# IDEA-CCNL/Fengshenbang-LM

Measured on AMD Instinct MI355X. Metric: tokens/sec Ziya-LLaMA-13B ZeRO-3, higher is better.
Workload: dtype bf16; 1 GPU; model=Ziya-LLaMA-13B, global_batch=16, micro_batch=16, seq_len=2048, parallelism=zero3_dp1, activation_checkpointing=True, ckpt_skip_interval=4

## Files before the change

fengshen_amd/models/layers.py:

```python
from __future__ import annotations

import math
from typing import Callable, List, Optional

import torch
import torch.nn as nn
import torch.nn.init as init

from fengshen_amd.ops import functional as F_ops
from fengshen_amd.parallel import groups
from fengshen_amd.parallel.layers import (
    ColumnParallelLinear,
    RowParallelLinear,
    _init_partition,
    divide,
)
from fengshen_amd.parallel.mappings import (
    copy_to_tensor_model_parallel_region,
    gather_from_tensor_model_parallel_region,
)


def init_normal(std: float) -> Callable:
    def fn(tensor):
        return init.normal_(tensor, mean=0.0, std=std)
    return fn


def scaled_init_normal(std: float, num_layers: int) -> Callable:
    return init_normal(std / math.sqrt(2.0 * num_layers))


def small_init(dim: int) -> Callable:
    return init_normal(math.sqrt(2.0 / (5.0 * dim)))


def wang_init(dim: int, num_layers: int) -> Callable:
    return init_normal(2.0 / (num_layers * math.sqrt(dim)))


class MergedColumnParallelLinear(ColumnParallelLinear):

    def __init__(self, input_size: int, segment_sizes: List[int], bias: bool = True,
                 init_method: Callable = init.xavier_normal_, dtype=None):
        self.segment_sizes = list(segment_sizes)
        super().__init__(input_size, sum(segment_sizes), bias=bias,
                         gather_output=False, init_method=init_method, dtype=dtype)
        tp = groups.get_tensor_model_parallel_world_size()
        if tp > 1:
            off = 0
            for seg in self.segment_sizes:
                seg_per = divide(seg, tp)
                shard = self.weight[off:off + seg_per]
                _init_partition(shard, init_method,
                                full_shape=(seg, input_size), partition_dim=0)
                off += seg_per


class RMSNorm(nn.Module):

    def __init__(self, dim: int, eps: float = 1e-6, dtype=None):
        super().__init__()
        self.weight = nn.Parameter(torch.ones(dim, dtype=dtype))
        self.eps = eps

    def forward(self, x):
        return F_ops.rms_norm(x, self.weight, self.eps)


class LayerNorm(nn.Module):

    def __init__(self, dim: int, eps: float = 1e-5, dtype=None):
        super().__init__()
        self.weight = nn.Parameter(torch.ones(dim, dtype=dtype))
        self.bias = nn.Parameter(torch.zeros(dim, dtype=dtype))
        self.eps = eps

    def forward(self, x):
        return F_ops.layer_norm(x, self.weight, self.bias, self.eps)


class ScaleNorm(nn.Module):

    def __init__(self, dim: int, eps: float = 1e-8, dtype=None):
        super().__init__()
        self.g = nn.Parameter(torch.ones(1, dtype=dtype))
        self.dim = dim
        self.eps = eps

    def forward(self, x):
        n = x.float().norm(dim=-1, keepdim=True) * self.dim ** -0.5
        return (x.float() / n.clamp(min=self.eps)).to(x.dtype) * self.g


def get_norm(kind: str, dim: int, eps: float, dtype=None) -> nn.Module:
    if kind == "rmsnorm":
        return RMSNorm(dim, eps, dtype)
    if kind == "layernorm":
        return LayerNorm(dim, eps, dtype)
    if kind == "scalenorm":
        return ScaleNorm(dim, dtype=dtype)
    raise ValueError(kind)


class ParallelAttention(nn.Module):

    def __init__(self, hidden_size: int, num_heads: int, *, causal: bool,
                 rotary: bool = False, rope_base: float = 10000.0,
                 max_positions: int = 4096,
                 attention_dropout: float = 0.0, hidden_dropout: float = 0.0,
                 bias: bool = True, init_method=None, output_init_method=None,
                 dtype=None, num_kv_heads: Optional[int] = None,
                 layer_idx: int = 0, reduce_output: bool = True):
        super().__init__()
        self.layer_idx = layer_idx
        self.reduce_output = reduce_output
        tp = groups.get_tensor_model_parallel_world_size()
        self.hidden_size = hidden_size
        self.num_heads = num_heads
        self.num_kv_heads = num_kv_heads or num_heads
        assert self.num_kv_heads == num_heads, "GQA arrives with kernel pass 2"
        self.head_dim = divide(hidden_size, num_heads)
        self.num_heads_per_partition = divide(num_heads, tp)
        self.causal = causal
        self.rotary = rotary
        self.attention_dropout = attention_dropout
        self.hidden_dropout = hidden_dropout
        self.norm_factor = 1.0 / math.sqrt(self.head_dim)
        init_method = init_method or init.xavier_normal_
        output_init_method = output_init_method or init_method

        self.qkv_proj = MergedColumnParallelLinear(
            hidden_size, [hidden_size, hidden_size, hidden_size], bias=bias,
            init_method=init_method, dtype=dtype)
        self.out_proj = RowParallelLinear(
            hidden_size, hidden_size, bias=bias, input_is_parallel=True,
            init_method=output_init_method, dtype=dtype,
            reduce_output=reduce_output)

        if rotary:
            self.rope_base = rope_base
            self.max_positions = max_positions
            self._rope_cache = None

    def _rope_tables(self, device, seq_needed: int):
        cache = self._rope_cache
        if (cache is None or cache[0].device != device
                or cache[0].shape[0] < seq_needed):
            n = max(self.max_positions, seq_needed)
            cos, sin = F_ops.build_rope_cache(n, self.head_dim,
                                              base=self.rope_base)
            cache = (cos.to(device), sin.to(device))
            self._rope_cache = cache
        return cache

    def forward(self, x: torch.Tensor,
                attention_mask: Optional[torch.Tensor] = None,
                cache=None):
        b, sq, _ = x.shape
        np_ = self.num_heads_per_partition
        hn = self.head_dim

        qkv = self.qkv_proj(x)
        q, k, v = qkv.chunk(3, dim=-1)
        q = q.view(b, sq, np_, hn).transpose(1, 2)
        k = k.view(b, sq, np_, hn).transpose(1, 2)
        v = v.view(b, sq, np_, hn).transpose(1, 2)

        offset = 0
        if cache is not None:
            offset = cache.get_seq_length(self.layer_idx)
        if self.rotary:
            cos, sin = self._rope_tables(q.device, offset + sq)
            q, k = F_ops.apply_rotary(q, k, cos, sin, offset=offset)
        if cache is not None:
            k, v = cache.update(k, v, self.layer_idx)

        causal = self.causal
        if causal and offset > 0 and q.shape[-2] == 1:
            causal = False
        ctx = F_ops.attention(q, k, v, causal=causal, mask=attention_mask,
                              dropout_p=self.attention_dropout,
                              training=self.training, scale=self.norm_factor)
        ctx = ctx.transpose(1, 2).reshape(b, sq, np_ * hn)
        out = self.out_proj(ctx)
        if isinstance(out, tuple) and self.reduce_output:
            out = out[0]
        return out


class ParallelMLP(nn.Module):

    def __init__(self, hidden_size: int, ffn_hidden_size: Optional[int] = None,
                 bias: bool = True, init_method=None, output_init_method=None,
                 dtype=None, reduce_output: bool = True):
        super().__init__()
        ffn = ffn_hidden_size or 4 * hidden_size
        init_method = init_method or init.xavier_normal_
        self.reduce_output = reduce_output
        self.fc_in = ColumnParallelLinear(
            hidden_size, ffn, bias=bias, gather_output=False,
            init_method=init_method, skip_bias_add=bias, dtype=dtype)
        self.fc_out = RowParallelLinear(
            ffn, hidden_size, bias=bias, input_is_parallel=True,
            init_method=output_init_method or init_method, dtype=dtype,
            reduce_output=reduce_output)

    def forward(self, x):
        h = self.fc_in(x)
        if isinstance(h, tuple):
            h, bias = h
            h = F_ops.bias_gelu(h, bias)
        else:
            h = F_ops.eager_gelu(h.float()).to(h.dtype)
        out = self.fc_out(h)
        if isinstance(out, tuple) and self.reduce_output:
            out = out[0]
        return out


class LLaMAParallelMLP(nn.Module):

    def __init__(self, hidden_size: int, intermediate_size: Optional[int] = None,
                 multiple_of: int = 256, init_method=None,
                 output_init_method=None, dtype=None,
                 reduce_output: bool = True):
        super().__init__()
        self.reduce_output = reduce_output
        if intermediate_size is None:
            intermediate_size = int(2 * (4 * hidden_size) / 3)
            intermediate_size = multiple_of * (
                (intermediate_size + multiple_of - 1) // multiple_of)
        self.intermediate_size = intermediate_size
        init_method = init_method or init.xavier_normal_
        self.gate_up_proj = MergedColumnParallelLinear(
            hidden_size, [intermediate_size, intermediate_size], bias=False,
            init_method=init_method, dtype=dtype)
        self.down_proj = RowParallelLinear(
            intermediate_size, hidden_size, bias=False, input_is_parallel=True,
            init_method=output_init_method or init_method, dtype=dtype,
            reduce_output=reduce_output)

    def forward(self, x):
        packed = self.gate_up_proj(x)
        h = F_ops.swiglu(packed)
        return self.down_proj(h)


class ParallelTransformerLayer(nn.Module):

    def __init__(self, hidden_size: int, num_heads: int, *, causal: bool,
                 norm: str = "layernorm", norm_eps: float = 1e-5,
                 mlp_type: str = "gelu", ffn_hidden_size=None,
                 rotary: bool = False, rope_base: float = 10000.0,
                 max_positions: int = 4096,
                 attention_dropout: float = 0.0, hidden_dropout: float = 0.0,
                 bias: bool = True, init_method=None, output_init_method=None,
                 dtype=None, layer_idx: int = 0,
                 parallel_residual: bool = False):
        super().__init__()
        self.parallel_residual = parallel_residual
        self.input_norm = get_norm(norm, hidden_size, norm_eps, dtype)
        self.attention = ParallelAttention(
            hidden_size, num_heads, causal=causal, rotary=rotary,
            rope_base=rope_base, max_positions=max_positions,
            attention_dropout=attention_dropout, hidden_dropout=hidden_dropout,
            bias=bias, init_method=init_method,
            output_init_method=output_init_method, dtype=dtype,
            layer_idx=layer_idx, reduce_output=not parallel_residual)
        self.post_attention_norm = get_norm(norm, hidden_size, norm_eps, dtype)
        if mlp_type == "swiglu":
            self.mlp = LLaMAParallelMLP(
                hidden_size, ffn_hidden_size, init_method=init_method,
                output_init_method=output_init_method, dtype=dtype,
                reduce_output=not parallel_residual)
        else:
            self.mlp = ParallelMLP(
                hidden_size, ffn_hidden_size, bias=bias, init_method=init_method,
                output_init_method=output_init_method, dtype=dtype,
                reduce_output=not parallel_residual)
        self.hidden_dropout = hidden_dropout

    @staticmethod
    def _split_partial(out):
        if isinstance(out, tuple):
            return out[0], out[1]
        return out, None

    def forward(self, x, attention_mask=None, cache=None):
        if self.parallel_residual:
            from fengshen_amd.parallel.mappings import (
                reduce_from_tensor_model_parallel_region)
            ap, ab = self._split_partial(self.attention(
                self.input_norm(x), attention_mask=attention_mask,
                cache=cache))
            mp, mb = self._split_partial(
                self.mlp(self.post_attention_norm(x)))
            total = reduce_from_tensor_model_parallel_region(ap + mp)
            bias = None
            if ab is not None or mb is not None:
                bias = (ab if ab is not None else 0)                     + (mb if mb is not None else 0)
            return F_ops.bias_dropout_add(total, bias, x,
                                          self.hidden_dropout,
                                          self.training)
        residual = x
        h = self.input_norm(x)
        attn_out = self.attention(h, attention_mask=attention_mask, cache=cache)
        x = F_ops.bias_dropout_add(attn_out, None, residual,
                                   self.hidden_dropout, self.training)
        residual = x
        h = self.post_attention_norm(x)
        mlp_out = self.mlp(h)
        x = F_ops.bias_dropout_add(mlp_out, None, residual,
                                   self.hidden_dropout, self.training)
        return x


def parallel_lm_logits(hidden: torch.Tensor, word_embeddings_weight: torch.Tensor,
                       parallel_output: bool = True):
    input_parallel = copy_to_tensor_model_parallel_region(hidden)
    logits_parallel = torch.nn.functional.linear(
        input_parallel, word_embeddings_weight)
    if parallel_output:
        return logits_parallel
    return gather_from_tensor_model_parallel_region(logits_parallel)


class SinusoidalPositionalEmbedding(nn.Module):

    def __init__(self, dim: int, base: float = 10000.0):
        super().__init__()
        self.dim = dim
        self.base = base

    def forward(self, positions: torch.Tensor) -> torch.Tensor:
        half = self.dim // 2
        inv = 1.0 / (self.base ** (torch.arange(
            half, device=positions.device, dtype=torch.float32) / half))
        ang = positions.float()[..., None] * inv
        return torch.cat([ang.sin(), ang.cos()], dim=-1)


class AliBi(nn.Module):

    def __init__(self, num_heads: int, mp_size: int = 1, mp_rank: int = 0):
        super().__init__()
        self.num_heads = num_heads
        slopes = torch.tensor(self._slopes(num_heads))
        per = num_heads // mp_size
        self.register_buffer("slopes", slopes[mp_rank * per:(mp_rank + 1) * per],
                             persistent=False)
        self._cache = None

    @staticmethod
    def _slopes(n: int):
        def pow2(n):
            start = 2.0 ** (-(2.0 ** -(math.log2(n) - 3)))
            return [start * (start ** i) for i in range(n)]
        if math.log2(n).is_integer():
            return pow2(n)
        closest = 2 ** math.floor(math.log2(n))
        return pow2(closest) + AliBi._slopes(2 * closest)[0::2][: n - closest]

    def forward(self, sq: int, sk: int, device, dtype):
        if (self._cache is None or self._cache.shape[-1] < sk
                or self._cache.device != device):
            pos = torch.arange(sk, device=device, dtype=torch.float32)
            self._cache = self.slopes.to(device)[:, None, None] * \
                (pos[None, None, :] - pos[None, :, None])
        bias = self._cache[:, :sq, :sk] if self._cache.shape[1] >= sq else \
            self._cache[:, -sq:, :sk]
        return bias.to(dtype)


class SoftEmbedding(nn.Module):

    def __init__(self, wte: nn.Module, n_tokens: int = 10,
                 init_range: float = 0.5):
        super().__init__()
        self.wte = wte
        self.n_tokens = n_tokens
        dim = wte.weight.shape[1]
        self.soft_prompt = nn.Parameter(
            torch.empty(n_tokens, dim).uniform_(-init_range, init_range))

    def forward(self, input_ids: torch.Tensor) -> torch.Tensor:
        emb = self.wte(input_ids)
        b = emb.shape[0]
        prompt = self.soft_prompt.unsqueeze(0).expand(b, -1, -1).to(emb.dtype)
        return torch.cat([prompt, emb], dim=1)


class SpatialGatingUnit(nn.Module):

    def __init__(self, dim_ff: int, seq_len: int):
        super().__init__()
        self.norm = LayerNorm(dim_ff // 2)
        self.proj = nn.Linear(seq_len, seq_len)
        nn.init.zeros_(self.proj.weight)
        nn.init.ones_(self.proj.bias)

    def forward(self, x):
        res, gate = x.chunk(2, dim=-1)
        gate = self.norm(gate)
        gate = self.proj(gate.transpose(1, 2)).transpose(1, 2)
        return res * gate


class GMLPBlock(nn.Module):
    def __init__(self, dim: int, dim_ff: int, seq_len: int):
        super().__init__()
        self.norm = LayerNorm(dim)
        self.fc_in = nn.Linear(dim, dim_ff)
        self.sgu = SpatialGatingUnit(dim_ff, seq_len)
        self.fc_out = nn.Linear(dim_ff // 2, dim)

    def forward(self, x):
        h = self.norm(x)
        h = F_ops.eager_gelu(self.fc_in(h).float()).to(h.dtype)
        h = self.sgu(h)
        return x + self.fc_out(h)


def expand_attention_types(attention_config, num_layers: int):
    if attention_config is None:
        return ["global"] * num_layers
    out = []
    for types, repeat in attention_config:
        if repeat == "all":
            for i in range(num_layers):
                out.append(types[i % len(types)])
            break
        for i in range(int(repeat)):
            out.append(types[i % len(types)])
    assert len(out) >= num_layers, (
        f"attention_config covers {len(out)} layers, model has {num_layers}")
    return out[:num_layers]


def get_ltor_masks_and_position_ids(data: torch.Tensor, eod_token: int,
                                    reset_position_ids: bool = False,
                                    reset_attention_mask: bool = False,
                                    eod_mask_loss: bool = False):
    b, s = data.shape
    att = torch.tril(torch.ones(s, s, device=data.device)) \
        .unsqueeze(0).repeat(b, 1, 1)
    loss_mask = torch.ones(b, s, dtype=torch.float, device=data.device)
    if eod_mask_loss:
        loss_mask[data == eod_token] = 0.0
    position_ids = torch.arange(s, device=data.device) \
        .unsqueeze(0).repeat(b, 1)
    if reset_position_ids or reset_attention_mask:
        position_ids = position_ids.clone()
        for bi in range(b):
            eod_idx = position_ids[bi, data[bi] == eod_token]
            prev = 0
            for j in eod_idx.tolist():
                if reset_attention_mask:
                    att[bi, j + 1:, : j + 1] = 0
                if reset_position_ids:
                    position_ids[bi, j + 1:] -= j + 1 - prev
                    prev = j + 1
    return (att < 0.5).unsqueeze(1), loss_mask, position_ids
```

fengshen_amd/ops/csrc/bindings.cpp:

```cpp
#include <torch/extension.h>

#include <hip/hip_runtime.h>
#include <c10/hip/HIPStream.h>

#include <vector>

enum FsDtype { FS_F32 = 0, FS_BF16 = 1, FS_F16 = 2 };

static int fs_dtype(const at::Tensor& t) {
  switch (t.scalar_type()) {
    case at::kFloat: return FS_F32;
    case at::kBFloat16: return FS_BF16;
    case at::kHalf: return FS_F16;
    default: TORCH_CHECK(false, "unsupported dtype ", t.scalar_type());
  }
}

static hipStream_t cur_stream() {
  return c10::hip::getCurrentHIPStream().stream();
}

extern "C" {
void fs_rms_norm_fwd(const void*, const void*, void*, float*, int, int, float,
                     int, hipStream_t);
void fs_rms_norm_bwd(const void*, const void*, const void*, const float*,
                     void*, float*, int, int, int, hipStream_t);
void fs_layer_norm_fwd(const void*, const void*, const void*, void*, float*,
                       float*, int, int, float, int, hipStream_t);
void fs_layer_norm_bwd(const void*, const void*, const void*, const float*,
                       const float*, void*, float*, float*, int, int, int,
                       hipStream_t);
void fs_scaled_softmax_fwd(const void*, const unsigned char*, void*, float,
                           int, int, int, int, int, int, int, int,
                           hipStream_t);
void fs_scaled_softmax_bwd(const void*, const void*, void*, float, int, int,
                           int, hipStream_t);
void fs_rope(const void*, void*, const float*, const float*, long, int, int,
             int, int, int, hipStream_t);
void fs_swiglu_fwd(const void*, void*, long, int, int, hipStream_t);
void fs_swiglu_bwd(const void*, const void*, void*, long, int, int,
                   hipStream_t);
void fs_bias_gelu(const void*, const void*, const void*, void*, long, int, int,
                  int, hipStream_t);
void fs_fused_adamw(float*, const void*, float*, float*, void*, long, float,
                    float, float, float, float, int, int, int, hipStream_t);
void fs_flash_attn_fwd(const void*, const void*, const void*, void*, float*,
                       const int*, int, int, int, int, int, int, float,
                       float, unsigned long long, hipStream_t);
void fs_flash_attn_bwd(const void*, const void*, const void*, const void*,
                       const void*, const float*, void*, void*, void*, float*,
                       const int*, int, int, int, int, int, int, float,
                       float, unsigned long long, hipStream_t);
void fs_bf16_gemv(const void*, const void*, void*, int, int, int,
                  hipStream_t);
void fs_add_rms_norm(const void*, const void*, const void*, void*, void*,
                     int, int, float, hipStream_t);
void fs_decode_attn(const void*, void*, void*, const float*, const float*,
                    const void*, void*, int, int, int, int, float, int,
                    hipStream_t);
void fs_w8_gemv(const void*, const float*, const void*, void*, int, int, int,
                hipStream_t);
void fs_vocab_ce_fwd(const void*, const long*, float*, float*, float*,
                     long, int, int, int, hipStream_t);
void fs_vocab_ce_bwd(const void*, const long*, const float*, const float*,
                     const float*, void*, long, int, int, int, hipStream_t);
void fs_flash_attn_fwd_v3(const void*, const void*, const void*, void*,
                          float*, const int*, int, int, int, int, int, float,
                          float, unsigned long long, hipStream_t);
void fs_flash_attn_bwd_v3(const void*, const void*, const void*, const void*,
                          const void*, const float*, void*, void*, void*,
                          float*, const int*, int, int, int, int, int, float,
                          float, unsigned long long, hipStream_t);
}

static std::vector<at::Tensor> rms_norm_fwd(at::Tensor x, at::Tensor w,
                                            double eps) {
  TORCH_CHECK(x.is_contiguous() && w.is_contiguous());
  const int H = x.size(-1);
  TORCH_CHECK(H % 8 == 0, "hidden must be divisible by 8");
  const long rows = x.numel() / H;
  auto out = at::empty_like(x);
  auto invrms = at::empty({rows}, x.options().dtype(at::kFloat));
  fs_rms_norm_fwd(x.data_ptr(), w.data_ptr(), out.data_ptr(),
                  invrms.data_ptr<float>(), (int)rows, H, (float)eps,
                  fs_dtype(x), cur_stream());
  return {out, invrms};
}

static std::vector<at::Tensor> rms_norm_bwd(at::Tensor gy, at::Tensor x,
                                            at::Tensor w, at::Tensor invrms) {
  const int H = x.size(-1);
  const long rows = x.numel() / H;
  auto gx = at::empty_like(x);
  auto gw32 = at::zeros({H}, x.options().dtype(at::kFloat));
  fs_rms_norm_bwd(gy.data_ptr(), x.data_ptr(), w.data_ptr(),
                  invrms.data_ptr<float>(), gx.data_ptr(),
                  gw32.data_ptr<float>(), (int)rows, H, fs_dtype(x),
                  cur_stream());
  return {gx, gw32.to(w.scalar_type())};
}

static std::vector<at::Tensor> layer_norm_fwd(at::Tensor x, at::Tensor w,
                                              c10::optional<at::Tensor> b,
                                              double eps) {
  TORCH_CHECK(x.is_contiguous());
  const int H = x.size(-1);
  TORCH_CHECK(H % 8 == 0, "hidden must be divisible by 8");
  const long rows = x.numel() / H;
  auto out = at::empty_like(x);
  auto mean = at::empty({rows}, x.options().dtype(at::kFloat));
  auto invstd = at::empty({rows}, x.options().dtype(at::kFloat));
  fs_layer_norm_fwd(x.data_ptr(), w.data_ptr(),
                    b.has_value() ? b->data_ptr() : nullptr, out.data_ptr(),
                    mean.data_ptr<float>(), invstd.data_ptr<float>(),
                    (int)rows, H, (float)eps, fs_dtype(x), cur_stream());
  return {out, mean, invstd};
}

static std::vector<at::Tensor> layer_norm_bwd(at::Tensor gy, at::Tensor x,
                                              at::Tensor w, at::Tensor mean,
                                              at::Tensor invstd) {
  const int H = x.size(-1);
  const long rows = x.numel() / H;
  auto gx = at::empty_like(x);
  auto gw32 = at::zeros({H}, x.options().dtype(at::kFloat));
  auto gb32 = at::zeros({H}, x.options().dtype(at::kFloat));
  fs_layer_norm_bwd(gy.data_ptr(), x.data_ptr(), w.data_ptr(),
                    mean.data_ptr<float>(), invstd.data_ptr<float>(),
                    gx.data_ptr(), gw32.data_ptr<float>(),
                    gb32.data_ptr<float>(), (int)rows, H, fs_dtype(x),
                    cur_stream());
  return {gx, gw32.to(w.scalar_type()), gb32.to(w.scalar_type())};
}

static at::Tensor scaled_masked_softmax_fwd(at::Tensor x,
                                            c10::optional<at::Tensor> mask,
                                            double scale) {
  TORCH_CHECK(x.dim() == 4 && x.is_contiguous());
  const int sk = x.size(3), sq = x.size(2), np = x.size(1), b = x.size(0);
  auto out = at::empty_like(x);
  const unsigned char* mp = nullptr;
  at::Tensor m8;
  int mb = 1, mode = 0, mask_sq = 1;
  if (mask.has_value()) {
    m8 = mask->to(at::kByte).contiguous();
    TORCH_CHECK(m8.dim() == 4 && m8.size(3) == sk &&
                    (m8.size(2) == sq || m8.size(2) == 1),
                "mask must be [mb,1,sq|1,sk]");
    mb = m8.size(0);
    mask_sq = m8.size(2);
    TORCH_CHECK(mb == 1 || mb == b, "mask batch must be 1 or b");
    mp = m8.data_ptr<unsigned char>();
    mode = 1;
  }
  fs_scaled_softmax_fwd(x.data_ptr(), mp, out.data_ptr(), (float)scale,
                        b * np * sq, sk, sq, np, mb, mask_sq, mode,
                        fs_dtype(x), cur_stream());
  return out;
}

static at::Tensor scaled_causal_softmax_fwd(at::Tensor x, double scale) {
  TORCH_CHECK(x.dim() == 3 && x.is_contiguous());
  const int sk = x.size(2), sq = x.size(1), ab = x.size(0);
  TORCH_CHECK(sq == sk, "causal softmax needs sq == sk");
  auto out = at::empty_like(x);
  fs_scaled_softmax_fwd(x.data_ptr(), nullptr, out.data_ptr(), (float)scale,
                        ab * sq, sk, sq, 1, 1, sq, 2, fs_dtype(x),
                        cur_stream());
  return out;
}

static at::Tensor scaled_softmax_bwd(at::Tensor gy, at::Tensor y,
                                     double scale) {
  TORCH_CHECK(gy.is_contiguous() && y.is_contiguous());
  const int sk = y.size(-1);
  const long rows = y.numel() / sk;
  auto gx = at::empty_like(y);
  fs_scaled_softmax_bwd(gy.data_ptr(), y.data_ptr(), gx.data_ptr(),
                        (float)scale, (int)rows, sk, fs_dtype(y),
                        cur_stream());
  return gx;
}

static std::vector<at::Tensor> rope_fwd(at::Tensor q, at::Tensor k,
                                        at::Tensor cos, at::Tensor sin,
                                        int64_t offset) {
  TORCH_CHECK(q.is_contiguous() && k.is_contiguous());
  TORCH_CHECK(cos.scalar_type() == at::kFloat && cos.is_contiguous());
  const int hn = q.size(-1), s = q.size(-2);
  TORCH_CHECK((hn / 2) % 8 == 0, "head_dim/2 must be divisible by 8");
  auto qo = at::empty_like(q);
  auto ko = at::empty_like(k);
  const long bnq = q.numel() / ((long)s * hn);
  const long bnk = k.numel() / ((long)s * hn);
  fs_rope(q.data_ptr(), qo.data_ptr(), cos.data_ptr<float>(),
          sin.data_ptr<float>(), bnq, s, hn, (int)offset, 0, fs_dtype(q),
          cur_stream());
  fs_rope(k.data_ptr(), ko.data_ptr(), cos.data_ptr<float>(),
          sin.data_ptr<float>(), bnk, s, hn, (int)offset, 0, fs_dtype(k),
          cur_stream());
  return {qo, ko};
}

static std::vector<at::Tensor> rope_bwd(at::Tensor gq, at::Tensor gk,
                                        at::Tensor cos, at::Tensor sin,
                                        int64_t offset) {
  const int hn = gq.size(-1), s = gq.size(-2);
  auto qo = at::empty_like(gq);
  auto ko = at::empty_like(gk);
  const long bnq = gq.numel() / ((long)s * hn);
  const long bnk = gk.numel() / ((long)s * hn);
  fs_rope(gq.data_ptr(), qo.data_ptr(), cos.data_ptr<float>(),
          sin.data_ptr<float>(), bnq, s, hn, (int)offset, 1, fs_dtype(gq),
          cur_stream());
  fs_rope(gk.data_ptr(), ko.data_ptr(), cos.data_ptr<float>(),
          sin.data_ptr<float>(), bnk, s, hn, (int)offset, 1, fs_dtype(gk),
          cur_stream());
  return {qo, ko};
}

static at::Tensor swiglu_fwd(at::Tensor packed) {
  TORCH_CHECK(packed.is_contiguous());
  const int h2 = packed.size(-1);
  TORCH_CHECK(h2 % 16 == 0, "packed dim must be divisible by 16");
  const int h = h2 / 2;
  const long rows = packed.numel() / h2;
  auto sizes = packed.sizes().vec();
  sizes.back() = h;
  auto out = at::empty(sizes, packed.options());
  fs_swiglu_fwd(packed.data_ptr(), out.data_ptr(), rows, h, fs_dtype(packed),
                cur_stream());
  return out;
}

static at::Tensor swiglu_bwd(at::Tensor gy, at::Tensor packed) {
  const int h2 = packed.size(-1);
  const int h = h2 / 2;
  const long rows = packed.numel() / h2;
  auto gpacked = at::empty_like(packed);
  fs_swiglu_bwd(gy.contiguous().data_ptr(), packed.data_ptr(),
                gpacked.data_ptr(), rows, h, fs_dtype(packed), cur_stream());
  return gpacked;
}

static at::Tensor bias_gelu_fwd(at::Tensor x, at::Tensor bias) {
  TORCH_CHECK(x.is_contiguous() && bias.is_contiguous());
  const int h = x.size(-1);
  TORCH_CHECK(h % 8 == 0);
  const long rows = x.numel() / h;
  auto out = at::empty_like(x);
  fs_bias_gelu(x.data_ptr(), bias.data_ptr(), nullptr, out.data_ptr(), rows, h,
               0, fs_dtype(x), cur_stream());
  return out;
}

static at::Tensor bias_gelu_bwd(at::Tensor gy, at::Tensor x, at::Tensor bias) {
  const int h = x.size(-1);
  const long rows = x.numel() / h;
  auto gx = at::empty_like(x);
  fs_bias_gelu(x.data_ptr(), bias.data_ptr(), gy.data_ptr(), gx.data_ptr(),
               rows, h, 1, fs_dtype(x), cur_stream());
  return gx;
}

static void fused_adamw(at::Tensor master, at::Tensor grad, at::Tensor m,
                        at::Tensor v, at::Tensor out_param, double lr,
                        double beta1, double beta2, double eps, double wd,
                        int64_t step) {
  TORCH_CHECK(master.scalar_type() == at::kFloat);
  TORCH_CHECK(master.is_contiguous() && grad.is_contiguous());
  void* outp = out_param.data_ptr() == master.data_ptr()
                   ? nullptr : out_param.data_ptr();
  fs_fused_adamw(master.data_ptr<float>(), grad.data_ptr(),
                 m.data_ptr<float>(), v.data_ptr<float>(), outp,
                 master.numel(), (float)lr, (float)beta1, (float)beta2,
                 (float)eps, (float)wd, (int)step, fs_dtype(grad),
                 outp ? fs_dtype(out_param) : FS_F32, cur_stream());
}

static const int kFlashDims[] = {40, 64, 80, 96, 128, 160};

static bool flash_dim_ok(int d) {
  for (int x : kFlashDims)
    if (x == d) return true;
  return false;
}

static std::vector<at::Tensor> flash_attn_fwd(
    at::Tensor q, at::Tensor k, at::Tensor v, double scale, bool causal,
    c10::optional<at::Tensor> klens, double drop_p, int64_t seed) {
  TORCH_CHECK(q.is_contiguous() && k.is_contiguous() && v.is_contiguous());
  TORCH_CHECK(q.scalar_type() == at::kBFloat16, "flash_attn: bf16 only");
  TORCH_CHECK(q.dim() == 4 && flash_dim_ok(q.size(3)),
              "flash_attn: head_dim must be one of 40/64/80/96/128/160");
  const int b = q.size(0), h = q.size(1), sq = q.size(2), d = q.size(3);
  const int sk = k.size(2);
  if (causal) {
    TORCH_CHECK(sq == sk && sq % 64 == 0 && !klens.has_value(),
                "flash_attn causal: sq==sk, sq%64==0, no klens");
  } else {
    TORCH_CHECK(sq % 16 == 0 && sq >= 16,
                "flash_attn: sq must be a multiple of 16");
  }
  const int* klp = nullptr;
  if (klens.has_value()) {
    TORCH_CHECK(klens->scalar_type() == at::kInt && klens->numel() == b
                && klens->is_contiguous());
    klp = klens->data_ptr<int>();
  }
  auto o = at::empty_like(q);
  auto lse = at::empty({b, h, sq}, q.options().dtype(at::kFloat));
  fs_flash_attn_fwd(q.data_ptr(), k.data_ptr(), v.data_ptr(), o.data_ptr(),
                    lse.data_ptr<float>(), klp, b, h, sq, sk, d,
                    causal ? 1 : 0, (float)scale, (float)drop_p,
                    (unsigned long long)seed, cur_stream());
  return {o, lse};
}

static std::vector<at::Tensor> flash_attn_bwd(
    at::Tensor q, at::Tensor k, at::Tensor v, at::Tensor o, at::Tensor dout,
    at::Tensor lse, double scale, bool causal,
    c10::optional<at::Tensor> klens, double drop_p, int64_t seed) {
  const int b = q.size(0), h = q.size(1), sq = q.size(2), d = q.size(3);
  const int sk = k.size(2);
  const int* klp = nullptr;
  if (klens.has_value()) klp = klens->data_ptr<int>();
  auto dq = at::empty_like(q);
  auto dk = at::empty_like(k);
  auto dv = at::empty_like(v);
  auto delta = at::empty({b, h, sq}, q.options().dtype(at::kFloat));
  fs_flash_attn_bwd(q.data_ptr(), k.data_ptr(), v.data_ptr(), o.data_ptr(),
                    dout.contiguous().data_ptr(), lse.data_ptr<float>(),
                    dq.data_ptr(), dk.data_ptr(), dv.data_ptr(),
                    delta.data_ptr<float>(), klp, b, h, sq, sk, d,
                    causal ? 1 : 0, (float)scale, (float)drop_p,
                    (unsigned long long)seed, cur_stream());
  return {dq, dk, dv};
}

static at::Tensor w8_gemv(at::Tensor q8, at::Tensor scale, at::Tensor x) {
  TORCH_CHECK(q8.scalar_type() == at::kChar && x.scalar_type() == at::kBFloat16);
  TORCH_CHECK(q8.is_contiguous() && x.is_contiguous());
  const int out = q8.size(0), in = q8.size(1);
  TORCH_CHECK(in % 16 == 0, "in_features must be divisible by 16");
  const int b = x.numel() / in;
  auto y = at::empty({b, out}, x.options());
  fs_w8_gemv(q8.data_ptr(), scale.data_ptr<float>(), x.data_ptr(),
             y.data_ptr(), b, in, out, cur_stream());
  return y;
}

static at::Tensor bf16_gemv(at::Tensor w, at::Tensor x) {
  TORCH_CHECK(w.scalar_type() == at::kBFloat16 &&
              x.scalar_type() == at::kBFloat16);
  TORCH_CHECK(w.is_contiguous() && x.is_contiguous());
  const int out = w.size(0), in = w.size(1);
  TORCH_CHECK(in % 16 == 0, "in_features must be divisible by 16");
  const int b = x.numel() / in;
  TORCH_CHECK(b >= 1 && b <= 8, "bf16_gemv: batch must be 1..8");
  auto y = at::empty({b, out}, x.options());
  fs_bf16_gemv(w.data_ptr(), x.data_ptr(), y.data_ptr(), b, in, out,
               cur_stream());
  return y;
}

static at::Tensor decode_attn(at::Tensor qkv, at::Tensor kc, at::Tensor vc,
                              at::Tensor cos_t, at::Tensor sin_t,
                              at::Tensor pos, double scale, bool rope) {
  TORCH_CHECK(qkv.scalar_type() == at::kBFloat16 && qkv.is_contiguous());
  TORCH_CHECK(kc.is_contiguous() && vc.is_contiguous());
  TORCH_CHECK(cos_t.scalar_type() == at::kFloat &&
              sin_t.scalar_type() == at::kFloat);
  TORCH_CHECK(pos.scalar_type() == at::kLong);
  const int b = kc.size(0), nh = kc.size(1), L = kc.size(2), d = kc.size(3);
  TORCH_CHECK(d == 64 || d == 128, "decode_attn: head dim must be 64/128");
  TORCH_CHECK(qkv.numel() == (long)b * 3 * nh * d, "qkv shape mismatch");
  auto ctx = at::empty({b, nh * d}, qkv.options());
  fs_decode_attn(qkv.data_ptr(), kc.data_ptr(), vc.data_ptr(),
                 cos_t.data_ptr<float>(), sin_t.data_ptr<float>(),
                 pos.data_ptr(), ctx.data_ptr(), b, nh, d, L, (float)scale,
                 rope ? 1 : 0, cur_stream());
  return ctx;
}

static std::vector<at::Tensor> add_rms_norm(at::Tensor a, at::Tensor b,
                                            at::Tensor w, double eps) {
  TORCH_CHECK(a.scalar_type() == at::kBFloat16 && a.is_contiguous() &&
              b.is_contiguous() && w.is_contiguous());
  const int H = a.size(-1);
  TORCH_CHECK(H % 8 == 0 && w.numel() == H && b.sizes() == a.sizes());
  const int rows = a.numel() / H;
  auto sum_out = at::empty_like(a);
  auto y = at::empty_like(a);
  fs_add_rms_norm(a.data_ptr(), b.data_ptr(), w.data_ptr(),
                  sum_out.data_ptr(), y.data_ptr(), rows, H, (float)eps,
                  cur_stream());
  return {sum_out, y};
}

PYBIND11_MODULE(TORCH_EXTENSION_NAME, mod) {
  mod.def("w8_gemv", &w8_gemv);
  mod.def("bf16_gemv", &bf16_gemv);
  mod.def("decode_attn", &decode_attn);
  mod.def("add_rms_norm", &add_rms_norm);
  mod.def("flash_attn_fwd", &flash_attn_fwd);
  mod.def("vocab_ce_fwd", [](at::Tensor logits2d, at::Tensor targets,
                             int64_t vstart, int64_t vend) {
    TORCH_CHECK(logits2d.is_contiguous() && logits2d.dim() == 2
                && logits2d.scalar_type() == at::kBFloat16);
    TORCH_CHECK(targets.scalar_type() == at::kLong
                && targets.is_contiguous());
    const long n = logits2d.size(0);
    const int w = logits2d.size(1);
    TORCH_CHECK(w % 8 == 0, "vocab shard must be divisible by 8");
    auto opts = logits2d.options().dtype(at::kFloat);
    auto m = at::empty({n}, opts);
    auto z = at::empty({n}, opts);
    auto pred = at::empty({n}, opts);
    fs_vocab_ce_fwd(logits2d.data_ptr(), targets.data_ptr<long>(),
                    m.data_ptr<float>(), z.data_ptr<float>(),
                    pred.data_ptr<float>(), n, w, (int)vstart, (int)vend,
                    cur_stream());
    return std::vector<at::Tensor>{m, z, pred};
  });
  mod.def("vocab_ce_bwd", [](at::Tensor logits2d, at::Tensor targets,
                             at::Tensor m, at::Tensor z, at::Tensor gout,
                             int64_t vstart, int64_t vend) {
    const long n = logits2d.size(0);
    const int w = logits2d.size(1);
    auto dl = at::empty_like(logits2d);
    fs_vocab_ce_bwd(logits2d.data_ptr(), targets.data_ptr<long>(),
                    m.data_ptr<float>(), z.data_ptr<float>(),
                    gout.contiguous().data_ptr<float>(), dl.data_ptr(), n, w,
                    (int)vstart, (int)vend, cur_stream());
    return dl;
  });
  mod.def("flash_attn_bwd_v3", [](at::Tensor q, at::Tensor k, at::Tensor v,
                                  at::Tensor o, at::Tensor dout,
                                  at::Tensor lse, double scale, bool causal,
                                  c10::optional<at::Tensor> klens,
                                  double drop_p, int64_t seed) {
    const int b = q.size(0), h = q.size(1), s = q.size(2), d = q.size(3);
    TORCH_CHECK((d == 128 || d == 96 || d == 64) && s % 64 == 0);
    const int* klp = nullptr;
    if (klens.has_value()) klp = klens->data_ptr<int>();
    auto dq = at::empty_like(q);
    auto dk = at::empty_like(k);
    auto dv = at::empty_like(v);
    auto delta = at::empty({b, h, s}, q.options().dtype(at::kFloat));
    fs_flash_attn_bwd_v3(q.data_ptr(), k.data_ptr(), v.data_ptr(),
                         o.data_ptr(), dout.contiguous().data_ptr(),
                         lse.data_ptr<float>(), dq.data_ptr(), dk.data_ptr(),
                         dv.data_ptr(), delta.data_ptr<float>(), klp, b, h,
                         s, d, causal ? 1 : 0, (float)scale, (float)drop_p,
                         (unsigned long long)seed, cur_stream());
    return std::vector<at::Tensor>{dq, dk, dv};
  });
  mod.def("flash_attn_fwd_v3", [](at::Tensor q, at::Tensor k, at::Tensor v,
                                  double scale, bool causal,
                                  c10::optional<at::Tensor> klens,
                                  double drop_p, int64_t seed) {
    TORCH_CHECK(q.is_contiguous() && k.is_contiguous() && v.is_contiguous());
    TORCH_CHECK(q.scalar_type() == at::kBFloat16);
    const int b = q.size(0), h = q.size(1), s = q.size(2), d = q.size(3);
    TORCH_CHECK((d == 128 || d == 96 || d == 64) && s % 64 == 0 && s >= 64);
    TORCH_CHECK(k.size(2) == s, "v3 is self-attention (sq == sk)");
    const int* klp = nullptr;
    if (klens.has_value()) {
      TORCH_CHECK(klens->scalar_type() == at::kInt
                  && klens->numel() == b && klens->is_contiguous());
      klp = klens->data_ptr<int>();
    }
    auto o = at::empty_like(q);
    auto lse = at::empty({b, h, s}, q.options().dtype(at::kFloat));
    fs_flash_attn_fwd_v3(q.data_ptr(), k.data_ptr(), v.data_ptr(),
                         o.data_ptr(), lse.data_ptr<float>(), klp, b, h, s,
                         d, causal ? 1 : 0, (float)scale, (float)drop_p,
                         (unsigned long long)seed, cur_stream());
    return std::vector<at::Tensor>{o, lse};
  });
  mod.def("flash_attn_bwd", &flash_attn_bwd);
  mod.def("rms_norm_fwd", &rms_norm_fwd);
  mod.def("rms_norm_bwd", &rms_norm_bwd);
  mod.def("layer_norm_fwd", &layer_norm_fwd);
  mod.def("layer_norm_bwd", &layer_norm_bwd);
  mod.def("scaled_masked_softmax_fwd", &scaled_masked_softmax_fwd);
  mod.def("scaled_causal_softmax_fwd", &scaled_causal_softmax_fwd);
  mod.def("scaled_softmax_bwd", &scaled_softmax_bwd);
  mod.def("rope_fwd", &rope_fwd);
  mod.def("rope_bwd", &rope_bwd);
  mod.def("swiglu_fwd", &swiglu_fwd);
  mod.def("swiglu_bwd", &swiglu_bwd);
  mod.def("bias_gelu_fwd", &bias_gelu_fwd);
  mod.def("bias_gelu_bwd", &bias_gelu_bwd);
  mod.def("fused_adamw", &fused_adamw);
}
```

fengshen_amd/ops/csrc/flash_attn.hip:

```cpp

#include "common.h"

typedef __attribute__((ext_vector_type(8))) short bf16x8;
typedef __attribute__((ext_vector_type(4))) float f32x4;

#define FA_QBLK 128
#define FA_KVBLK 64
#define FA_WAVES 8
#define FA_VPAD 8
#define FB_T 32

constexpr int fa_dpad(int d) { return (d + 31) / 32 * 32; }
constexpr int fa_swb(int dp) {
  int need = 2 * dp, p = 128;
  while (p < need) p <<= 1;
  return p;
}

__device__ __forceinline__ int kswz(int row, int byte_in_row) {
  return byte_in_row ^ ((row & 7) << 4);
}

__device__ __forceinline__ unsigned int fa_hash(unsigned long long seed,
                                                unsigned long long idx) {
  unsigned long long z = seed + idx * 0x9E3779B97F4A7C15ull;
  z = (z ^ (z >> 30)) * 0xBF58476D1CE4E5B9ull;
  z = (z ^ (z >> 27)) * 0x94D049BB133111EBull;
  return (unsigned int)(z >> 32);
}

__device__ __forceinline__ short fa_bf16bits(float f) {
  return (short)__hip_bfloat16_raw(__float2bfloat16(f)).x;
}

template <int D>
__device__ __forceinline__ bf16x8 fa_load8(const bf16_t* rowp, int d0) {
  if (d0 < D) return *reinterpret_cast<const bf16x8*>(rowp + d0);
  bf16x8 z;
#pragma unroll
  for (int j = 0; j < 8; ++j) z[j] = 0;
  return z;
}

template <int D, bool CAUSAL>
__global__ __launch_bounds__(FA_WAVES * 64)
void flash_attn_fwd_kernel(const bf16_t* __restrict__ Q,
                           const bf16_t* __restrict__ K,
                           const bf16_t* __restrict__ V,
                           bf16_t* __restrict__ O,
                           float* __restrict__ LSE,
                           const int* __restrict__ klens,
                           int b, int h, int sq, int sk, float scale,
                           unsigned int drop_thresh, float keep_scale,
                           unsigned long long drop_seed) {
  constexpr int DP = fa_dpad(D);
  constexpr int NC = DP / 32;
  constexpr int NTO = DP / 16;
  constexpr int SWB = fa_swb(DP);

  __shared__ char k_raw[FA_KVBLK * SWB];
  __shared__ short vt_lds[DP][FA_KVBLK + FA_VPAD];
  __shared__ short p_lds[FA_WAVES][16][FA_KVBLK + FA_VPAD];

  const int lane = threadIdx.x & 63;
  const int wave = threadIdx.x >> 6;
  const int qb = blockIdx.x;
  const int head = blockIdx.y;
  const int batch = blockIdx.z;

  const bf16_t* Qp = Q + ((long)batch * h + head) * sq * D;
  const bf16_t* Kp = K + ((long)batch * h + head) * sk * D;
  const bf16_t* Vp = V + ((long)batch * h + head) * sk * D;
  bf16_t* Op = O + ((long)batch * h + head) * sq * D;

  const int klen = CAUSAL ? sk
                          : min(klens ? klens[batch] : sk, sk);

  const int q0 = qb * FA_QBLK + wave * 16;
  const bool q_active = q0 < sq;
  const int q0c = q_active ? q0 : (sq > 16 ? sq - 16 : 0);

  bf16x8 q_frag[NC];
  {
    const int row = lane & 15;
    const int k0 = (lane >> 4) * 8;
    const int qrow = min(q0c + row, sq - 1);
#pragma unroll
    for (int c = 0; c < NC; ++c) {
      bf16x8 raw = fa_load8<D>(Qp + (long)qrow * D, c * 32 + k0);
#pragma unroll
      for (int j = 0; j < 8; ++j) {
        unsigned short u = (unsigned short)raw[j];
        float f = __uint_as_float(((unsigned int)u) << 16) * scale;
        raw[j] = fa_bf16bits(f);
      }
      q_frag[c] = raw;
    }
  }

  float m_run[4], l_run[4];
  f32x4 o_acc[NTO];
#pragma unroll
  for (int r = 0; r < 4; ++r) {
    m_run[r] = -INFINITY;
    l_run[r] = 0.f;
  }
#pragma unroll
  for (int t = 0; t < NTO; ++t) o_acc[t] = f32x4{0, 0, 0, 0};

  int n_kv_tiles;
  if (CAUSAL) {
    const int q_hi = min(qb * FA_QBLK + FA_QBLK, sq) - 1;
    n_kv_tiles = (q_hi / FA_KVBLK) + 1;
  } else {
    n_kv_tiles = (klen + FA_KVBLK - 1) / FA_KVBLK;
    if (n_kv_tiles < 1) n_kv_tiles = 1;
  }

  const int tid = threadIdx.x;
  constexpr int ELEMS = FA_KVBLK * DP;
  constexpr int SWEEPS = (ELEMS + FA_WAVES * 64 * 8 - 1) / (FA_WAVES * 64 * 8);
  bf16x8 k_reg[SWEEPS], v_reg[SWEEPS];
#pragma unroll
  for (int sweep = 0; sweep < SWEEPS; ++sweep) {
    const int i = tid * 8 + sweep * (FA_WAVES * 64 * 8);
    if (i < ELEMS) {
      const int kr = i / DP;
      const int kc = i % DP;
      const long krg = min(kr, sk - 1);
      k_reg[sweep] = fa_load8<D>(Kp + krg * D, kc);
      v_reg[sweep] = fa_load8<D>(Vp + krg * D, kc);
    }
  }

  for (int kt = 0; kt < n_kv_tiles; ++kt) {
    const int k_base = kt * FA_KVBLK;
    __syncthreads();
#pragma unroll
    for (int sweep = 0; sweep < SWEEPS; ++sweep) {
      const int i = tid * 8 + sweep * (FA_WAVES * 64 * 8);
      if (i < ELEMS) {
        const int kr = i / DP;
        const int kc = i % DP;
        *reinterpret_cast<bf16x8*>(k_raw + kr * SWB + kswz(kr, kc * 2)) =
            k_reg[sweep];
        bf16x8 vv = v_reg[sweep];
#pragma unroll
        for (int j = 0; j < 8; ++j)
          vt_lds[kc + j][kr ^ ((kc + j) & 0x38)] = vv[j];
      }
    }
    __syncthreads();
    if (kt + 1 < n_kv_tiles) {
      const int nb = (kt + 1) * FA_KVBLK;
#pragma unroll
      for (int sweep = 0; sweep < SWEEPS; ++sweep) {
        const int i = tid * 8 + sweep * (FA_WAVES * 64 * 8);
        if (i < ELEMS) {
          const int kr = i / DP;
          const int kc = i % DP;
          const long krg = min(nb + kr, sk - 1);
          k_reg[sweep] = fa_load8<D>(Kp + krg * D, kc);
          v_reg[sweep] = fa_load8<D>(Vp + krg * D, kc);
        }
      }
    }

    f32x4 s_acc[4];
#pragma unroll
    for (int nt = 0; nt < 4; ++nt) s_acc[nt] = f32x4{0, 0, 0, 0};
    {
      const int col = lane & 15;
#pragma unroll
      for (int nt = 0; nt < 4; ++nt) {
        const int krow = nt * 16 + col;
#pragma unroll
        for (int c = 0; c < NC; ++c) {
          const int d0 = c * 32 + (lane >> 4) * 8;
          bf16x8 bfrag = *reinterpret_cast<const bf16x8*>(
              k_raw + krow * SWB + kswz(krow, d0 * 2));
          s_acc[nt] = __builtin_amdgcn_mfma_f32_16x16x32_bf16(
              q_frag[c], bfrag, s_acc[nt], 0, 0, 0);
        }
      }
    }

    const int col = lane & 15;
    float p[4][4];
    float tile_max[4];
#pragma unroll
    for (int r = 0; r < 4; ++r) {
      const int qrow = q0c + (lane >> 4) * 4 + r;
      float tm = -INFINITY;
#pragma unroll
      for (int nt = 0; nt < 4; ++nt) {
        const int kcol = k_base + nt * 16 + col;
        float v = s_acc[nt][r];
        if (CAUSAL ? (kcol > qrow) : (kcol >= klen)) v = -INFINITY;
        p[nt][r] = v;
        tm = fmaxf(tm, v);
      }
      tile_max[r] = tm;
    }
#pragma unroll
    for (int off = 8; off > 0; off >>= 1) {
#pragma unroll
      for (int r = 0; r < 4; ++r)
        tile_max[r] = fmaxf(tile_max[r], __shfl_xor(tile_max[r], off, 64));
    }
    float alpha[4], rowsum[4];
    bool need_rescale = false;
#pragma unroll
    for (int r = 0; r < 4; ++r) {
      const float m_new = fmaxf(m_run[r], tile_max[r]);
      alpha[r] = (m_run[r] == -INFINITY) ? 0.f : __expf(m_run[r] - m_new);
      if (m_new != m_run[r]) need_rescale = true;
      m_run[r] = m_new;
      float ps = 0.f;
#pragma unroll
      for (int nt = 0; nt < 4; ++nt) {
        float e = (p[nt][r] == -INFINITY) ? 0.f : __expf(p[nt][r] - m_new);
        p[nt][r] = e;
        ps += e;
      }
      rowsum[r] = ps;
    }
#pragma unroll
    for (int off = 8; off > 0; off >>= 1) {
#pragma unroll
      for (int r = 0; r < 4; ++r)
        rowsum[r] += __shfl_xor(rowsum[r], off, 64);
    }
#pragma unroll
    for (int r = 0; r < 4; ++r)
      l_run[r] = l_run[r] * alpha[r] + rowsum[r];
    if (drop_thresh) {
      const unsigned long long bh_base =
          ((unsigned long long)batch * h + head) * sq;
#pragma unroll
      for (int r = 0; r < 4; ++r) {
        const unsigned long long qi =
            (bh_base + (unsigned long long)(q0c + (lane >> 4) * 4 + r)) *
            (unsigned long long)sk;
#pragma unroll
        for (int nt = 0; nt < 4; ++nt) {
          const int kcol = k_base + nt * 16 + col;
          p[nt][r] = (fa_hash(drop_seed, qi + kcol) < drop_thresh)
                         ? 0.f : p[nt][r] * keep_scale;
        }
      }
    }
    if (__any(need_rescale)) {
#pragma unroll
      for (int t = 0; t < NTO; ++t) {
#pragma unroll
        for (int r = 0; r < 4; ++r) o_acc[t][r] *= alpha[r];
      }
    }

#pragma unroll
    for (int r = 0; r < 4; ++r) {
      const int row = (lane >> 4) * 4 + r;
#pragma unroll
      for (int nt = 0; nt < 4; ++nt) {
        p_lds[wave][row][nt * 16 + col] = fa_bf16bits(p[nt][r]);
      }
    }
    __builtin_amdgcn_s_waitcnt(0);

#pragma unroll
    for (int kc = 0; kc < 2; ++kc) {
      const int row = lane & 15;
      const int kv0 = kc * 32 + (lane >> 4) * 8;
      bf16x8 pa = *reinterpret_cast<const bf16x8*>(&p_lds[wave][row][kv0]);
#pragma unroll
      for (int t = 0; t < NTO; ++t) {
        const int dcol = t * 16 + (lane & 15);
        bf16x8 bfrag = *reinterpret_cast<const bf16x8*>(
            &vt_lds[dcol][kv0 ^ (dcol & 0x38)]);
        o_acc[t] = __builtin_amdgcn_mfma_f32_16x16x32_bf16(pa, bfrag, o_acc[t],
                                                           0, 0, 0);
      }
    }
  }

  if (!q_active) return;
  const int col = lane & 15;
#pragma unroll
  for (int r = 0; r < 4; ++r) {
    const int qrow = q0 + (lane >> 4) * 4 + r;
    if (qrow >= sq) continue;
    const float inv_l = (l_run[r] > 0.f) ? 1.f / l_run[r] : 0.f;
#pragma unroll
    for (int t = 0; t < NTO; ++t) {
      const int d = t * 16 + col;
      if (d < D) Op[(long)qrow * D + d] = __float2bfloat16(o_acc[t][r] * inv_l);
    }
    if (col == 0 && LSE) {
      LSE[((long)batch * h + head) * sq + qrow] =
          m_run[r] + logf(fmaxf(l_run[r], 1e-30f));
    }
  }
}


template <int D>
__global__ __launch_bounds__(256)
void flash_delta_kernel(const bf16_t* __restrict__ dO,
                        const bf16_t* __restrict__ O,
                        float* __restrict__ delta, long rows) {
  const int lane = threadIdx.x & 63;
  const int wid = threadIdx.x >> 6;
  const long row0 = (long)blockIdx.x * 4 + wid;
  const long stride = (long)gridDim.x * 4;
  for (long row = row0; row < rows; row += stride) {
    const bf16_t* dop = dO + row * D;
    const bf16_t* op = O + row * D;
    float sacc = 0.f;
    for (int i = lane * 2; i < D; i += 128) {
#pragma unroll
      for (int j = 0; j < 2; ++j)
        sacc += __bfloat162float(dop[i + j]) * __bfloat162float(op[i + j]);
    }
    sacc = wave_reduce_sum(sacc);
    if (lane == 0) delta[row] = sacc;
  }
}

template <int D, bool CAUSAL>
__global__ __launch_bounds__(FA_WAVES * 64)
void flash_attn_bwd_dq_kernel(const bf16_t* __restrict__ Q,
                              const bf16_t* __restrict__ K,
                              const bf16_t* __restrict__ V,
                              const bf16_t* __restrict__ dO,
                              const float* __restrict__ LSE,
                              const float* __restrict__ Delta,
                              bf16_t* __restrict__ dQ,
                              const int* __restrict__ klens,
                              int b, int h, int sq, int sk, float scale,
                              unsigned int drop_thresh, float keep_scale,
                              unsigned long long drop_seed) {
  constexpr int DP = fa_dpad(D);
  constexpr int NC = DP / 32;
  constexpr int NTO = DP / 16;
  constexpr int SWB = fa_swb(DP);

  __shared__ char k_raw[FB_T * SWB];
  __shared__ char v_raw[FB_T * SWB];
  __shared__ short kt_lds[DP][FB_T + FA_VPAD];
  __shared__ short p_lds[FA_WAVES][16][FB_T + FA_VPAD];

  const int lane = threadIdx.x & 63;
  const int wave = threadIdx.x >> 6;
  const long bh = (long)blockIdx.z * h + blockIdx.y;
  const bf16_t* Qp = Q + bh * sq * D;
  const bf16_t* Kp = K + bh * sk * D;
  const bf16_t* Vp = V + bh * sk * D;
  const bf16_t* dOp = dO + bh * sq * D;
  bf16_t* dQp = dQ + bh * sq * D;
  const float* lse = LSE + bh * sq;
  const float* dlt = Delta + bh * sq;

  const int klen = CAUSAL ? sk
                          : min(klens ? klens[blockIdx.z] : sk, sk);

  const int q0 = blockIdx.x * FA_QBLK + wave * 16;
  const bool q_active = q0 < sq;
  const int q0c = q_active ? q0 : (sq > 16 ? sq - 16 : 0);

  bf16x8 q_frag[NC], do_frag[NC];
  {
    const int row = lane & 15;
    const int k0 = (lane >> 4) * 8;
    const int qrow = min(q0c + row, sq - 1);
#pragma unroll
    for (int c = 0; c < NC; ++c) {
      bf16x8 raw = fa_load8<D>(Qp + (long)qrow * D, c * 32 + k0);
#pragma unroll
      for (int j = 0; j < 8; ++j) {
        unsigned short u = (unsigned short)raw[j];
        float f = __uint_as_float(((unsigned int)u) << 16) * scale;
        raw[j] = fa_bf16bits(f);
      }
      q_frag[c] = raw;
      do_frag[c] = fa_load8<D>(dOp + (long)qrow * D, c * 32 + k0);
    }
  }
  float lse_r[4], dlt_r[4];
#pragma unroll
  for (int r = 0; r < 4; ++r) {
    const int qrow = min(q0c + (lane >> 4) * 4 + r, sq - 1);
    lse_r[r] = lse[qrow];
    dlt_r[r] = dlt[qrow];
  }

  f32x4 dq_acc[NTO];
#pragma unroll
  for (int t = 0; t < NTO; ++t) dq_acc[t] = f32x4{0, 0, 0, 0};

  int n_kv_tiles;
  if (CAUSAL) {
    const int q_hi = min(blockIdx.x * FA_QBLK + FA_QBLK, sq) - 1;
    n_kv_tiles = (q_hi / FB_T) + 1;
  } else {
    n_kv_tiles = (klen + FB_T - 1) / FB_T;
  }

  constexpr int BELEMS = FB_T * DP;
  constexpr int BSWEEPS = (BELEMS + FA_WAVES * 64 * 8 - 1)
                          / (FA_WAVES * 64 * 8);
  bf16x8 kst[BSWEEPS], vst[BSWEEPS];
  {
    const int tid = threadIdx.x;
    const int kt0_base = (CAUSAL ? 0 : 0) * FB_T;
#pragma unroll
    for (int sw = 0; sw < BSWEEPS; ++sw) {
      const int i = tid * 8 + sw * (FA_WAVES * 64 * 8);
      if (i < BELEMS) {
        const int kr = i / DP;
        const int kc = i % DP;
        const long krg = min(kt0_base + kr, sk - 1);
        kst[sw] = fa_load8<D>(Kp + krg * D, kc);
        vst[sw] = fa_load8<D>(Vp + krg * D, kc);
      }
    }
  }
  for (int kt = 0; kt < n_kv_tiles; ++kt) {
    __syncthreads();
    {
      const int tid = threadIdx.x;
#pragma unroll
      for (int sw = 0; sw < BSWEEPS; ++sw) {
        const int i = tid * 8 + sw * (FA_WAVES * 64 * 8);
        if (i < BELEMS) {
          const int kr = i / DP;
          const int kc = i % DP;
          bf16x8 kk = kst[sw];
          *reinterpret_cast<bf16x8*>(
              k_raw + kr * SWB + kswz(kr, kc * 2)) = kk;
          *reinterpret_cast<bf16x8*>(
              v_raw + kr * SWB + kswz(kr, kc * 2)) = vst[sw];
#pragma unroll
          for (int j = 0; j < 8; ++j)
            kt_lds[kc + j][kr ^ ((kc + j) & 0x18)] = kk[j];
        }
      }
    }
    __syncthreads();
    const int k_base = kt * FB_T;
    if (kt + 1 < n_kv_tiles) {
      const int nb = (kt + 1) * FB_T;
      const int tid = threadIdx.x;
#pragma unroll
      for (int sw = 0; sw < BSWEEPS; ++sw) {
        const int i = tid * 8 + sw * (FA_WAVES * 64 * 8);
        if (i < BELEMS) {
          const int kr = i / DP;
          const int kc = i % DP;
          const long krg = min(nb + kr, sk - 1);
          kst[sw] = fa_load8<D>(Kp + krg * D, kc);
          vst[sw] = fa_load8<D>(Vp + krg * D, kc);
        }
      }
    }

    f32x4 s_acc[2], dp_acc[2];
#pragma unroll
    for (int nt = 0; nt < 2; ++nt) {
      s_acc[nt] = f32x4{0, 0, 0, 0};
      dp_acc[nt] = f32x4{0, 0, 0, 0};
    }
    {
      const int col = lane & 15;
#pragma unroll
      for (int nt = 0; nt < 2; ++nt) {
        const int krow = nt * 16 + col;
#pragma unroll
        for (int c = 0; c < NC; ++c) {
          const int d0 = c * 32 + (lane >> 4) * 8;
          bf16x8 kb = *reinterpret_cast<const bf16x8*>(
              k_raw + krow * SWB + kswz(krow, d0 * 2));
          s_acc[nt] = __builtin_amdgcn_mfma_f32_16x16x32_bf16(
              q_frag[c], kb, s_acc[nt], 0, 0, 0);
          bf16x8 vb = *reinterpret_cast<const bf16x8*>(
              v_raw + krow * SWB + kswz(krow, d0 * 2));
          dp_acc[nt] = __builtin_amdgcn_mfma_f32_16x16x32_bf16(
              do_frag[c], vb, dp_acc[nt], 0, 0, 0);
        }
      }
    }

    const int col = lane & 15;
#pragma unroll
    for (int r = 0; r < 4; ++r) {
      const int qrow = q0c + (lane >> 4) * 4 + r;
      const int row = (lane >> 4) * 4 + r;
#pragma unroll
      for (int nt = 0; nt < 2; ++nt) {
        const int kcol = k_base + nt * 16 + col;
        const bool masked = CAUSAL ? (kcol > qrow) : (kcol >= klen);
        float pv = masked ? 0.f : __expf(s_acc[nt][r] - lse_r[r]);
        float dpv = dp_acc[nt][r];
        if (drop_thresh) {
          const unsigned long long idx =
              (bh * (unsigned long long)sq + qrow) *
                  (unsigned long long)sk + kcol;
          dpv = (fa_hash(drop_seed, idx) < drop_thresh)
                    ? 0.f : dpv * keep_scale;
        }
        float ds = pv * (dpv - dlt_r[r]) * scale;
        p_lds[wave][row][nt * 16 + col] = fa_bf16bits(ds);
      }
    }
    __builtin_amdgcn_s_waitcnt(0);

    {
      const int row = lane & 15;
      const int kv0 = (lane >> 4) * 8;
      bf16x8 pa = *reinterpret_cast<const bf16x8*>(&p_lds[wave][row][kv0]);
#pragma unroll
      for (int t = 0; t < NTO; ++t) {
        const int dcol = t * 16 + (lane & 15);
        bf16x8 bfrag = *reinterpret_cast<const bf16x8*>(
            &kt_lds[dcol][kv0 ^ (dcol & 0x18)]);
        dq_acc[t] = __builtin_amdgcn_mfma_f32_16x16x32_bf16(
            pa, bfrag, dq_acc[t], 0, 0, 0);
      }
    }
  }

  if (!q_active) return;
  const int col = lane & 15;
#pragma unroll
  for (int r = 0; r < 4; ++r) {
    const int qrow = q0 + (lane >> 4) * 4 + r;
    if (qrow >= sq) continue;
#pragma unroll
    for (int t = 0; t < NTO; ++t) {
      const int d = t * 16 + col;
      if (d < D) dQp[(long)qrow * D + d] = __float2bfloat16(dq_acc[t][r]);
    }
  }
}

template <int D, bool CAUSAL>
__global__ __launch_bounds__(FA_WAVES * 64)
void flash_attn_bwd_dkv_kernel(const bf16_t* __restrict__ Q,
                               const bf16_t* __restrict__ K,
                               const bf16_t* __restrict__ V,
                               const bf16_t* __restrict__ dO,
                               const float* __restrict__ LSE,
                               const float* __restrict__ Delta,
                               bf16_t* __restrict__ dK,
                               bf16_t* __restrict__ dV,
                               const int* __restrict__ klens,
                               int b, int h, int sq, int sk, float scale,
                               unsigned int drop_thresh, float keep_scale,
                               unsigned long long drop_seed) {
  constexpr int DP = fa_dpad(D);
  constexpr int NC = DP / 32;
  constexpr int NTO = DP / 16;
  constexpr int SWB = fa_swb(DP);

  __shared__ char q_raw[FB_T * SWB];
  __shared__ char do_raw[FB_T * SWB];
  __shared__ short qt_lds[DP][FB_T + FA_VPAD];
  __shared__ short dot_lds[DP][FB_T + FA_VPAD];
  __shared__ short p_lds[FA_WAVES][16][FB_T + FA_VPAD];

  const int lane = threadIdx.x & 63;
  const int wave = threadIdx.x >> 6;
  const long bh = (long)blockIdx.z * h + blockIdx.y;
  const bf16_t* Qp = Q + bh * sq * D;
  const bf16_t* Kp = K + bh * sk * D;
  const bf16_t* Vp = V + bh * sk * D;
  const bf16_t* dOp = dO + bh * sq * D;
  bf16_t* dKp = dK + bh * sk * D;
  bf16_t* dVp = dV + bh * sk * D;
  const float* lse = LSE + bh * sq;
  const float* dlt = Delta + bh * sq;

  const int klen = CAUSAL ? sk
                          : min(klens ? klens[blockIdx.z] : sk, sk);

  const int kv0_blk = blockIdx.x * (FA_WAVES * 16);
  const int kv0_wave = kv0_blk + wave * 16;
  const bool kv_active = kv0_wave < sk;
  const int kv0c = kv_active ? kv0_wave : (sk > 16 ? sk - 16 : 0);

  bf16x8 k_frag[NC], v_frag[NC];
  {
    const int row = lane & 15;
    const int c0 = (lane >> 4) * 8;
    const int kvrow = min(kv0c + row, sk - 1);
#pragma unroll
    for (int c = 0; c < NC; ++c) {
      bf16x8 raw = fa_load8<D>(Kp + (long)kvrow * D, c * 32 + c0);
#pragma unroll
      for (int j = 0; j < 8; ++j) {
        unsigned short u = (unsigned short)raw[j];
        float f = __uint_as_float(((unsigned int)u) << 16) * scale;
        raw[j] = fa_bf16bits(f);
      }
      k_frag[c] = raw;
      v_frag[c] = fa_load8<D>(Vp + (long)kvrow * D, c * 32 + c0);
    }
  }

  f32x4 dv_acc[NTO], dk_acc[NTO];
#pragma unroll
  for (int t = 0; t < NTO; ++t) {
    dv_acc[t] = f32x4{0, 0, 0, 0};
    dk_acc[t] = f32x4{0, 0, 0, 0};
  }

  const int first_qt = CAUSAL ? kv0_blk / FB_T : 0;
  const int n_q_tiles = (sq + FB_T - 1) / FB_T;

  constexpr int BELEMS = FB_T * DP;
  constexpr int BSWEEPS = (BELEMS + FA_WAVES * 64 * 8 - 1)
                          / (FA_WAVES * 64 * 8);
  bf16x8 qst[BSWEEPS], dst[BSWEEPS];
  {
    const int tid = threadIdx.x;
    const int q0_base = first_qt * FB_T;
#pragma unroll
    for (int sw = 0; sw < BSWEEPS; ++sw) {
      const int i = tid * 8 + sw * (FA_WAVES * 64 * 8);
      if (i < BELEMS) {
        const int qr = i / DP;
        const int qc = i % DP;
        const long qrg = min(q0_base + qr, sq - 1);
        qst[sw] = fa_load8<D>(Qp + qrg * D, qc);
        dst[sw] = fa_load8<D>(dOp + qrg * D, qc);
      }
    }
  }
  for (int qt = first_qt; qt < n_q_tiles; ++qt) {
    const int q_base = qt * FB_T;
    __syncthreads();
    {
      const int tid = threadIdx.x;
#pragma unroll
      for (int sw = 0; sw < BSWEEPS; ++sw) {
        const int i = tid * 8 + sw * (FA_WAVES * 64 * 8);
        if (i < BELEMS) {
          const int qr = i / DP;
          const int qc = i % DP;
          bf16x8 qq = qst[sw];
          bf16x8 dd = dst[sw];
          *reinterpret_cast<bf16x8*>(
              q_raw + qr * SWB + kswz(qr, qc * 2)) = qq;
          *reinterpret_cast<bf16x8*>(
              do_raw + qr * SWB + kswz(qr, qc * 2)) = dd;
#pragma unroll
          for (int j = 0; j < 8; ++j) {
            qt_lds[qc + j][qr ^ ((qc + j) & 0x18)] = qq[j];
            dot_lds[qc + j][qr ^ ((qc + j) & 0x18)] = dd[j];
          }
        }
      }
    }
    __syncthreads();
    if (qt + 1 < n_q_tiles) {
      const int nb = (qt + 1) * FB_T;
      const int tid = threadIdx.x;
#pragma unroll
      for (int sw = 0; sw < BSWEEPS; ++sw) {
        const int i = tid * 8 + sw * (FA_WAVES * 64 * 8);
        if (i < BELEMS) {
          const int qr = i / DP;
          const int qc = i % DP;
          const long qrg = min(nb + qr, sq - 1);
          qst[sw] = fa_load8<D>(Qp + qrg * D, qc);
          dst[sw] = fa_load8<D>(dOp + qrg * D, qc);
        }
      }
    }

    f32x4 st_acc[2], dpt_acc[2];
#pragma unroll
    for (int nt = 0; nt < 2; ++nt) {
      st_acc[nt] = f32x4{0, 0, 0, 0};
      dpt_acc[nt] = f32x4{0, 0, 0, 0};
    }
    {
      const int col = lane & 15;
#pragma unroll
      for (int nt = 0; nt < 2; ++nt) {
        const int qrow = nt * 16 + col;
#pragma unroll
        for (int c = 0; c < NC; ++c) {
          const int d0 = c * 32 + (lane >> 4) * 8;
          bf16x8 qb = *reinterpret_cast<const bf16x8*>(
              q_raw + qrow * SWB + kswz(qrow, d0 * 2));
          st_acc[nt] = __builtin_amdgcn_mfma_f32_16x16x32_bf16(
              k_frag[c], qb, st_acc[nt], 0, 0, 0);
          bf16x8 db = *reinterpret_cast<const bf16x8*>(
              do_raw + qrow * SWB + kswz(qrow, d0 * 2));
          dpt_acc[nt] = __builtin_amdgcn_mfma_f32_16x16x32_bf16(
              v_frag[c], db, dpt_acc[nt], 0, 0, 0);
        }
      }
    }

    const int col = lane & 15;
    float pt[2][4];
#pragma unroll
    for (int nt = 0; nt < 2; ++nt) {
      const int qcol = q_base + nt * 16 + col;
      const int qcolc = min(qcol, sq - 1);
      const float lse_c = lse[qcolc];
      const float dlt_c = dlt[qcolc];
#pragma unroll
      for (int r = 0; r < 4; ++r) {
        const int kvrow = kv0c + (lane >> 4) * 4 + r;
        bool masked = CAUSAL ? (qcol < kvrow)
                             : (kvrow >= klen || qcol >= sq);
        float pv = masked ? 0.f : __expf(st_acc[nt][r] - lse_c);
        float dm = 1.f;
        if (drop_thresh) {
          const unsigned long long idx =
              (bh * (unsigned long long)sq + qcol) *
                  (unsigned long long)sk + kvrow;
          dm = (fa_hash(drop_seed, idx) < drop_thresh) ? 0.f : keep_scale;
        }
        pt[nt][r] = pv * dm;
        dpt_acc[nt][r] = pv * (dm * dpt_acc[nt][r] - dlt_c) * scale;
      }
    }

#pragma unroll
    for (int r = 0; r < 4; ++r) {
      const int row = (lane >> 4) * 4 + r;
#pragma unroll
      for (int nt = 0; nt < 2; ++nt)
        p_lds[wave][row][nt * 16 + col] = fa_bf16bits(pt[nt][r]);
    }
    __builtin_amdgcn_s_waitcnt(0);
    {
      const int row = lane & 15;
      const int q0f = (lane >> 4) * 8;
      bf16x8 pa = *reinterpret_cast<const bf16x8*>(&p_lds[wave][row][q0f]);
#pragma unroll
      for (int t = 0; t < NTO; ++t) {
        const int dcol = t * 16 + (lane & 15);
        bf16x8 bfrag = *reinterpret_cast<const bf16x8*>(
            &dot_lds[dcol][q0f ^ (dcol & 0x18)]);
        dv_acc[t] = __builtin_amdgcn_mfma_f32_16x16x32_bf16(
            pa, bfrag, dv_acc[t], 0, 0, 0);
      }
    }

    __builtin_amdgcn_s_waitcnt(0);
#pragma unroll
    for (int r = 0; r < 4; ++r) {
      const int row = (lane >> 4) * 4 + r;
#pragma unroll
      for (int nt = 0; nt < 2; ++nt)
        p_lds[wave][row][nt * 16 + col] = fa_bf16bits(dpt_acc[nt][r]);
    }
    __builtin_amdgcn_s_waitcnt(0);
    {
      const int row = lane & 15;
      const int q0f = (lane >> 4) * 8;
      bf16x8 pa = *reinterpret_cast<const bf16x8*>(&p_lds[wave][row][q0f]);
#pragma unroll
      for (int t = 0; t < NTO; ++t) {
        const int dcol = t * 16 + (lane & 15);
        bf16x8 bfrag = *reinterpret_cast<const bf16x8*>(
            &qt_lds[dcol][q0f ^ (dcol & 0x18)]);
        dk_acc[t] = __builtin_amdgcn_mfma_f32_16x16x32_bf16(
            pa, bfrag, dk_acc[t], 0, 0, 0);
      }
    }
  }

  if (!kv_active) return;
  const int col = lane & 15;
#pragma unroll
  for (int r = 0; r < 4; ++r) {
    const int kvrow = kv0_wave + (lane >> 4) * 4 + r;
    if (kvrow >= sk) continue;
#pragma unroll
    for (int t = 0; t < NTO; ++t) {
      const int d = t * 16 + col;
      if (d < D) {
        dKp[(long)kvrow * D + d] = __float2bfloat16(dk_acc[t][r]);
        dVp[(long)kvrow * D + d] = __float2bfloat16(dv_acc[t][r]);
      }
    }
  }
}

template <int D>
static void launch_fwd(bool causal, const void* q, const void* k,
                       const void* v, void* o, float* lse, const int* klens,
                       int b, int h, int sq, int sk, float scale,
                       unsigned int dth, float ksc, unsigned long long seed,
                       hipStream_t stream) {
  dim3 grid((sq + FA_QBLK - 1) / FA_QBLK, h, b);
  dim3 block(FA_WAVES * 64);
  if (causal)
    hipLaunchKernelGGL((flash_attn_fwd_kernel<D, true>), grid, block, 0,
                       stream, (const bf16_t*)q, (const bf16_t*)k,
                       (const bf16_t*)v, (bf16_t*)o, lse, klens, b, h, sq, sk,
                       scale, dth, ksc, seed);
  else
    hipLaunchKernelGGL((flash_attn_fwd_kernel<D, false>), grid, block, 0,
                       stream, (const bf16_t*)q, (const bf16_t*)k,
                       (const bf16_t*)v, (bf16_t*)o, lse, klens, b, h, sq, sk,
                       scale, dth, ksc, seed);
}

extern "C" void fs_flash_attn_fwd(const void* q, const void* k, const void* v,
                                  void* o, float* lse, const int* klens,
                                  int b, int h, int sq, int sk, int d,
                                  int causal, float scale, float drop_p,
                                  unsigned long long seed,
                                  hipStream_t stream) {
  const unsigned int dth =
      (drop_p > 0.f) ? (unsigned int)(drop_p * 4294967296.0) : 0u;
  const float ksc = (drop_p > 0.f) ? 1.f / (1.f - drop_p) : 1.f;
#define FWD_CASE(DD) case DD: launch_fwd<DD>(causal, q, k, v, o, lse, klens, \
    b, h, sq, sk, scale, dth, ksc, seed, stream); break;
  switch (d) {
    FWD_CASE(40) FWD_CASE(64) FWD_CASE(80)
    FWD_CASE(96) FWD_CASE(128) FWD_CASE(160)
  }
#undef FWD_CASE
}

template <int D>
static void launch_bwd(bool causal, const void* q, const void* k,
                       const void* v, const void* o, const void* dout,
                       const float* lse, void* dq, void* dk, void* dv,
                       float* delta_ws, const int* klens, int b, int h,
                       int sq, int sk, float scale, unsigned int dth,
                       float ksc, unsigned long long seed,
                       hipStream_t stream) {
  const long rows = (long)b * h * sq;
  {
    long blocks = (rows + 3) / 4;
    if (blocks > 4096) blocks = 4096;
    hipLaunchKernelGGL((flash_delta_kernel<D>), dim3((unsigned)blocks),
                       dim3(256), 0, stream, (const bf16_t*)dout,
                       (const bf16_t*)o, delta_ws, rows);
  }
  dim3 gq((sq + FA_QBLK - 1) / FA_QBLK, h, b);
  dim3 gkv((sk + FA_WAVES * 16 - 1) / (FA_WAVES * 16), h, b);
  dim3 block(FA_WAVES * 64);
  if (causal) {
    hipLaunchKernelGGL((flash_attn_bwd_dq_kernel<D, true>), gq, block, 0,
                       stream, (const bf16_t*)q, (const bf16_t*)k,
                       (const bf16_t*)v, (const bf16_t*)dout, lse, delta_ws,
                       (bf16_t*)dq, klens, b, h, sq, sk, scale, dth, ksc,
                       seed);
    hipLaunchKernelGGL((flash_attn_bwd_dkv_kernel<D, true>), gkv, block, 0,
                       stream, (const bf16_t*)q, (const bf16_t*)k,
                       (const bf16_t*)v, (const bf16_t*)dout, lse, delta_ws,
                       (bf16_t*)dk, (bf16_t*)dv, klens, b, h, sq, sk, scale,
                       dth, ksc, seed);
  } else {
    hipLaunchKernelGGL((flash_attn_bwd_dq_kernel<D, false>), gq, block, 0,
                       stream, (const bf16_t*)q, (const bf16_t*)k,
                       (const bf16_t*)v, (const bf16_t*)dout, lse, delta_ws,
                       (bf16_t*)dq, klens, b, h, sq, sk, scale, dth, ksc,
                       seed);
    hipLaunchKernelGGL((flash_attn_bwd_dkv_kernel<D, false>), gkv, block, 0,
                       stream, (const bf16_t*)q, (const bf16_t*)k,
                       (const bf16_t*)v, (const bf16_t*)dout, lse, delta_ws,
                       (bf16_t*)dk, (bf16_t*)dv, klens, b, h, sq, sk, scale,
                       dth, ksc, seed);
  }
}

extern "C" void fs_flash_attn_bwd(const void* q, const void* k, const void* v,
                                  const void* o, const void* dout,
                                  const float* lse, void* dq, void* dk,
                                  void* dv, float* delta_ws, const int* klens,
                                  int b, int h, int sq, int sk, int d,
                                  int causal, float scale, float drop_p,
                                  unsigned long long seed,
                                  hipStream_t stream) {
  const unsigned int dth =
      (drop_p > 0.f) ? (unsigned int)(drop_p * 4294967296.0) : 0u;
  const float ksc = (drop_p > 0.f) ? 1.f / (1.f - drop_p) : 1.f;
#define BWD_CASE(DD) case DD: launch_bwd<DD>(causal, q, k, v, o, dout, lse, \
    dq, dk, dv, delta_ws, klens, b, h, sq, sk, scale, dth, ksc, seed, \
    stream); break;
  switch (d) {
    BWD_CASE(40) BWD_CASE(64) BWD_CASE(80)
    BWD_CASE(96) BWD_CASE(128) BWD_CASE(160)
  }
#undef BWD_CASE
}


#define V3_QBLK 256
#define V3_KVBLK 64

typedef __attribute__((ext_vector_type(16))) float f32x16;

template <int D, bool CAUSAL, bool HAS_DROP>
__global__ __launch_bounds__(FA_WAVES * 64)
void flash_attn_fwd_v3_kernel(const bf16_t* __restrict__ Q,
                              const bf16_t* __restrict__ K,
                              const bf16_t* __restrict__ V,
                              bf16_t* __restrict__ O,
                              float* __restrict__ LSE,
                              const int* __restrict__ klens,
                              int b, int h, int s, float scale,
                              unsigned int drop_thresh, float keep_scale,
                              unsigned long long drop_seed) {
  constexpr int NC = D / 16;
  constexpr int NTO = D / 32;
  constexpr int SWB = fa_swb(D);

  __shared__ char k_raw[2][V3_KVBLK * SWB];
  __shared__ short vt_lds[2][D][V3_KVBLK + FA_VPAD];

  const int lane = threadIdx.x & 63;
  const int wave = threadIdx.x >> 6;
  const int hi = lane >> 5;
  const int ln = lane & 31;
  const long bh = (long)blockIdx.z * h + blockIdx.y;
  const bf16_t* Qp = Q + bh * s * D;
  const bf16_t* Kp = K + bh * s * D;
  const bf16_t* Vp = V + bh * s * D;
  bf16_t* Op = O + bh * s * D;

  const int klen = CAUSAL ? s : min(klens ? klens[blockIdx.z] : s, s);

  const int q0w = blockIdx.x * V3_QBLK + wave * 32;
  const bool q_active = q0w < s;
  const int q0c = q_active ? q0w : s - 32;
  const int my_q = q0c + ln;

  bf16x8 q_frag[NC];
#pragma unroll
  for (int c = 0; c < NC; ++c) {
    bf16x8 raw = *reinterpret_cast<const bf16x8*>(
        Qp + (long)my_q * D + c * 16 + hi * 8);
#pragma unroll
    for (int j = 0; j < 8; ++j) {
      unsigned short u = (unsigned short)raw[j];
      float f = __uint_as_float(((unsigned int)u) << 16) * scale;
      raw[j] = fa_bf16bits(f);
    }
    q_frag[c] = raw;
  }

  float m_run = -INFINITY, l_run = 0.f;
  f32x16 o_acc[NTO];
#pragma unroll
  for (int t = 0; t < NTO; ++t) {
#pragma unroll
    for (int r = 0; r < 16; ++r) o_acc[t][r] = 0.f;
  }

  int n_kv_tiles;
  if (CAUSAL) {
    const int q_hi_row = min(blockIdx.x * V3_QBLK + V3_QBLK, s) - 1;
    n_kv_tiles = (q_hi_row / V3_KVBLK) + 1;
  } else {
    n_kv_tiles = (klen + V3_KVBLK - 1) / V3_KVBLK;
    if (n_kv_tiles < 1) n_kv_tiles = 1;
  }

  const int tid = threadIdx.x;
  constexpr int ELEMS = V3_KVBLK * D;
  constexpr int SWEEPS = (ELEMS + FA_WAVES * 64 * 8 - 1) / (FA_WAVES * 64 * 8);
  bf16x8 k_reg[SWEEPS], v_reg[SWEEPS];
#pragma unroll
  for (int sweep = 0; sweep < SWEEPS; ++sweep) {
    const int i = tid * 8 + sweep * (FA_WAVES * 64 * 8);
    if (i < ELEMS) {
      const long kr = min(i / D, s - 1);
      const int kc = i % D;
      k_reg[sweep] = *reinterpret_cast<const bf16x8*>(Kp + kr * D + kc);
      v_reg[sweep] = *reinterpret_cast<const bf16x8*>(Vp + kr * D + kc);
    }
  }

  {
#pragma unroll
    for (int sweep = 0; sweep < SWEEPS; ++sweep) {
      const int i = tid * 8 + sweep * (FA_WAVES * 64 * 8);
      if (i < ELEMS) {
        const int kr = i / D;
        const int kc = i % D;
        *reinterpret_cast<bf16x8*>(
            k_raw[0] + kr * SWB + kswz(kr, kc * 2)) = k_reg[sweep];
        bf16x8 vv = v_reg[sweep];
#pragma unroll
        for (int j = 0; j < 8; ++j)
          vt_lds[0][kc + j][kr ^ ((kc + j) & 0x38)] = vv[j];
      }
    }
  }
  int cur = 0;
  for (int kt = 0; kt < n_kv_tiles; ++kt) {
    const int k_base = kt * V3_KVBLK;
    __syncthreads();
    if (kt + 1 < n_kv_tiles) {
      const int nb = (kt + 1) * V3_KVBLK;
#pragma unroll
      for (int sweep = 0; sweep < SWEEPS; ++sweep) {
        const int i = tid * 8 + sweep * (FA_WAVES * 64 * 8);
        if (i < ELEMS) {
          const long kr = min((long)(nb + i / D), (long)s - 1);
          const int kc = i % D;
          k_reg[sweep] = *reinterpret_cast<const bf16x8*>(Kp + kr * D + kc);
          v_reg[sweep] = *reinterpret_cast<const bf16x8*>(Vp + kr * D + kc);
        }
      }
    }

    f32x16 st[2];
#pragma unroll
    for (int nt = 0; nt < 2; ++nt) {
#pragma unroll
      for (int r = 0; r < 16; ++r) st[nt][r] = 0.f;
    }
#pragma unroll
    for (int nt = 0; nt < 2; ++nt) {
      const int krow = nt * 32 + ln;
#pragma unroll
      for (int c = 0; c < NC; ++c) {
        bf16x8 a = *reinterpret_cast<const bf16x8*>(
            k_raw[cur] + krow * SWB + kswz(krow, (c * 16 + hi * 8) * 2));
        st[nt] = __builtin_amdgcn_mfma_f32_32x32x16_bf16(a, q_frag[c],
                                                         st[nt], 0, 0, 0);
      }
    }

    float p[32];
    float tmax = -INFINITY;
#pragma unroll
    for (int nt = 0; nt < 2; ++nt) {
#pragma unroll
      for (int r = 0; r < 16; ++r) {
        const int kcol = k_base + nt * 32 + (r & 3) + 8 * (r >> 2) + 4 * hi;
        float v = st[nt][r];
        if (CAUSAL ? (kcol > my_q) : (kcol >= klen)) v = -INFINITY;
        p[nt * 16 + r] = v;
        tmax = fmaxf(tmax, v);
      }
    }
    tmax = fmaxf(tmax, __shfl_xor(tmax, 32, 64));
    const float m_new = fmaxf(m_run, tmax);
    const float alpha = (m_run == -INFINITY) ? 0.f : __expf(m_run - m_new);
    const bool rescale = (m_new != m_run);
    m_run = m_new;
    float rs = 0.f;
#pragma unroll
    for (int i = 0; i < 32; ++i) {
      float e = (p[i] == -INFINITY) ? 0.f : __expf(p[i] - m_new);
      p[i] = e;
      rs += e;
    }
    rs += __shfl_xor(rs, 32, 64);
    l_run = l_run * alpha + rs;

    if (HAS_DROP && drop_thresh) {
      const unsigned long long qi =
          (bh * (unsigned long long)s + my_q) * (unsigned long long)s;
#pragma unroll
      for (int nt = 0; nt < 2; ++nt) {
#pragma unroll
        for (int r = 0; r < 16; ++r) {
          const int kcol =
              k_base + nt * 32 + (r & 3) + 8 * (r >> 2) + 4 * hi;
          float& pv = p[nt * 16 + r];
          pv = (fa_hash(drop_seed, qi + kcol) < drop_thresh)
                   ? 0.f : pv * keep_scale;
        }
      }
    }

    if (__any(rescale)) {
#pragma unroll
      for (int r = 0; r < 16; ++r) {
        const float al = __shfl(alpha, (r & 3) + 8 * (r >> 2) + 4 * hi, 64);
#pragma unroll
        for (int t = 0; t < NTO; ++t) o_acc[t][r] *= al;
      }
    }

    unsigned int pw[8][2];
#pragma unroll
    for (int G = 0; G < 8; ++G) {
      const int base = (G >> 2) * 16 + (G & 3) * 4;
#pragma unroll
      for (int k = 0; k < 2; ++k) {
        const unsigned int lo =
            (unsigned short)fa_bf16bits(p[base + 2 * k]);
        const unsigned int hi_b =
            (unsigned short)fa_bf16bits(p[base + 2 * k + 1]);
        pw[G][k] = (hi_b << 16) | lo;
      }
    }

#pragma unroll
    for (int c2 = 0; c2 < 4; ++c2) {
      unsigned int paw[4];
#pragma unroll
      for (int k = 0; k < 2; ++k) {
        auto pr = __builtin_amdgcn_permlane32_swap(
            (int)pw[2 * c2][k], (int)pw[2 * c2 + 1][k], false, false);
        paw[k] = (unsigned int)pr[0];
        paw[k + 2] = (unsigned int)pr[1];
      }
      bf16x8 pa;
#pragma unroll
      for (int k = 0; k < 4; ++k) {
        pa[2 * k] = (short)(paw[k] & 0xFFFF);
        pa[2 * k + 1] = (short)(paw[k] >> 16);
      }
#pragma unroll
      for (int t = 0; t < NTO; ++t) {
        const int dcol = t * 32 + ln;
        bf16x8 vb = *reinterpret_cast<const bf16x8*>(
            &vt_lds[cur][dcol][(c2 * 16 + hi * 8) ^ (dcol & 0x38)]);
        o_acc[t] = __builtin_amdgcn_mfma_f32_32x32x16_bf16(pa, vb, o_acc[t],
                                                           0, 0, 0);
      }
    }

    if (kt + 1 < n_kv_tiles) {
      const int nxt = cur ^ 1;
#pragma unroll
      for (int sweep = 0; sweep < SWEEPS; ++sweep) {
        const int i = tid * 8 + sweep * (FA_WAVES * 64 * 8);
        if (i < ELEMS) {
          const int kr = i / D;
          const int kc = i % D;
          *reinterpret_cast<bf16x8*>(
              k_raw[nxt] + kr * SWB + kswz(kr, kc * 2)) = k_reg[sweep];
          bf16x8 vv = v_reg[sweep];
#pragma unroll
          for (int j = 0; j < 8; ++j)
            vt_lds[nxt][kc + j][kr ^ ((kc + j) & 0x38)] = vv[j];
        }
      }
      cur = nxt;
    }
  }

  if (!q_active) return;
  const float my_inv_l = (l_run > 0.f) ? 1.f / l_run : 0.f;
#pragma unroll
  for (int r = 0; r < 16; ++r) {
    const int qrow = q0w + (r & 3) + 8 * (r >> 2) + 4 * hi;
    const float inv_l =
        __shfl(my_inv_l, (r & 3) + 8 * (r >> 2) + 4 * hi, 64);
#pragma unroll
    for (int t = 0; t < NTO; ++t) {
      Op[(long)qrow * D + t * 32 + ln] =
          __float2bfloat16(o_acc[t][r] * inv_l);
    }
  }
  if (hi == 0 && LSE) {
    LSE[bh * s + q0w + ln] = m_run + logf(fmaxf(l_run, 1e-30f));
  }
}

extern "C" void fs_flash_attn_fwd_v3(const void* q, const void* k,
                                     const void* v, void* o, float* lse,
                                     const int* klens, int b, int h, int s,
                                     int d, int causal, float scale,
                                     float drop_p, unsigned long long seed,
                                     hipStream_t stream) {
  dim3 grid((s + V3_QBLK - 1) / V3_QBLK, h, b);
  dim3 block(FA_WAVES * 64);
  const unsigned int dth =
      (drop_p > 0.f) ? (unsigned int)(drop_p * 4294967296.0) : 0u;
  const float ksc = (drop_p > 0.f) ? 1.f / (1.f - drop_p) : 1.f;
#define V3F(DD, CC, DR) hipLaunchKernelGGL( \
    (flash_attn_fwd_v3_kernel<DD, CC, DR>), \
    grid, block, 0, stream, (const bf16_t*)q, (const bf16_t*)k, \
    (const bf16_t*)v, (bf16_t*)o, lse, klens, b, h, s, scale, dth, ksc, seed)
  if (dth) {
    if (d == 128 && causal) V3F(128, true, true);
    else if (d == 128) V3F(128, false, true);
    else if (d == 96 && causal) V3F(96, true, true);
    else if (d == 96) V3F(96, false, true);
    else if (d == 64 && causal) V3F(64, true, true);
    else V3F(64, false, true);
  } else {
    if (d == 128 && causal) V3F(128, true, false);
    else if (d == 128) V3F(128, false, false);
    else if (d == 96 && causal) V3F(96, true, false);
    else if (d == 96) V3F(96, false, false);
    else if (d == 64 && causal) V3F(64, true, false);
    else V3F(64, false, false);
  }
#undef V3F
}


#define B3_FB 32

template <int D, bool CAUSAL, bool HAS_DROP>
__global__ __launch_bounds__(FA_WAVES * 64)
void flash_attn_bwd_dq_v3_kernel(const bf16_t* __restrict__ Q,
                                 const bf16_t* __restrict__ K,
                                 const bf16_t* __restrict__ V,
                                 const bf16_t* __restrict__ dO,
                                 const float* __restrict__ LSE,
                                 const float* __restrict__ Delta,
                                 bf16_t* __restrict__ dQ,
                                 const int* __restrict__ klens,
                                 int b, int h, int s, float scale,
                                 unsigned int drop_thresh, float keep_scale,
                                 unsigned long long drop_seed) {
  constexpr int NC = D / 16;
  constexpr int NTO = D / 32;
  constexpr int SWB = fa_swb(D);

  __shared__ char k_raw[B3_FB * SWB];
  __shared__ char v_raw[B3_FB * SWB];
  __shared__ short kt_lds[D][B3_FB + FA_VPAD];
  __shared__ short p_x[FA_WAVES][32][B3_FB + FA_VPAD];

  const int lane = threadIdx.x & 63;
  const int wave = threadIdx.x >> 6;
  const int hi = lane >> 5;
  const int ln = lane & 31;
  const long bh = (long)blockIdx.z * h + blockIdx.y;
  const bf16_t* Qp = Q + bh * s * D;
  const bf16_t* Kp = K + bh * s * D;
  const bf16_t* Vp = V + bh * s * D;
  const bf16_t* dOp = dO + bh * s * D;
  bf16_t* dQp = dQ + bh * s * D;
  const float* lse = LSE + bh * s;
  const float* dlt = Delta + bh * s;

  const int klen = CAUSAL ? s : min(klens ? klens[blockIdx.z] : s, s);
  const int q0w = blockIdx.x * V3_QBLK + wave * 32;
  const bool q_active = q0w < s;
  const int q0c = q_active ? q0w : s - 32;
  const int my_q = q0c + ln;

  bf16x8 q_frag[NC], do_frag[NC];
#pragma unroll
  for (int c = 0; c < NC; ++c) {
    bf16x8 raw = *reinterpret_cast<const bf16x8*>(
        Qp + (long)my_q * D + c * 16 + hi * 8);
#pragma unroll
    for (int j = 0; j < 8; ++j) {
      unsigned short u = (unsigned short)raw[j];
      raw[j] = fa_bf16bits(
          __uint_as_float(((unsigned int)u) << 16) * scale);
    }
    q_frag[c] = raw;
    do_frag[c] = *reinterpret_cast<const bf16x8*>(
        dOp + (long)my_q * D + c * 16 + hi * 8);
  }
  const float lse_r = lse[my_q];
  const float dlt_r = dlt[my_q];

  f32x16 dq_acc[NTO];
#pragma unroll
  for (int t = 0; t < NTO; ++t) {
#pragma unroll
    for (int r = 0; r < 16; ++r) dq_acc[t][r] = 0.f;
  }

  int n_kv_tiles;
  if (CAUSAL) {
    const int q_hi_row = min(blockIdx.x * V3_QBLK + V3_QBLK, s) - 1;
    n_kv_tiles = (q_hi_row / B3_FB) + 1;
  } else {
    n_kv_tiles = (klen + B3_FB - 1) / B3_FB;
  }

  for (int kt = 0; kt < n_kv_tiles; ++kt) {
    const int k_base = kt * B3_FB;
    __syncthreads();
    {
      const int tid = threadIdx.x;
      for (int i = tid * 8; i < B3_FB * D; i += FA_WAVES * 64 * 8) {
        const int kr = i / D;
        const int kc = i % D;
        const long krg = min(k_base + kr, s - 1);
        bf16x8 kk = *reinterpret_cast<const bf16x8*>(Kp + krg * D + kc);
        *reinterpret_cast<bf16x8*>(k_raw + kr * SWB + kswz(kr, kc * 2)) = kk;
        bf16x8 vv = *reinterpret_cast<const bf16x8*>(Vp + krg * D + kc);
        *reinterpret_cast<bf16x8*>(v_raw + kr * SWB + kswz(kr, kc * 2)) = vv;
#pragma unroll
        for (int j = 0; j < 8; ++j)
          kt_lds[kc + j][kr ^ ((kc + j) & 0x18)] = kk[j];
      }
    }
    __syncthreads();

    f32x16 st, dpt;
#pragma unroll
    for (int r = 0; r < 16; ++r) {
      st[r] = 0.f;
      dpt[r] = 0.f;
    }
    {
      const int krow = ln;
#pragma unroll
      for (int c = 0; c < NC; ++c) {
        bf16x8 ka = *reinterpret_cast<const bf16x8*>(
            k_raw + krow * SWB + kswz(krow, (c * 16 + hi * 8) * 2));
        st = __builtin_amdgcn_mfma_f32_32x32x16_bf16(ka, q_frag[c], st,
                                                     0, 0, 0);
        bf16x8 va = *reinterpret_cast<const bf16x8*>(
            v_raw + krow * SWB + kswz(krow, (c * 16 + hi * 8) * 2));
        dpt = __builtin_amdgcn_mfma_f32_32x32x16_bf16(va, do_frag[c], dpt,
                                                      0, 0, 0);
      }
    }

#pragma unroll
    for (int g = 0; g < 4; ++g) {
      short pk[4] __attribute__((aligned(8)));
#pragma unroll
      for (int j = 0; j < 4; ++j) {
        const int r = g * 4 + j;
        const int kcol = k_base + (r & 3) + 8 * (r >> 2) + 4 * hi;
        const bool masked = CAUSAL ? (kcol > my_q) : (kcol >= klen);
        float pv = masked ? 0.f : __expf(st[r] - lse_r);
        float dpv = dpt[r];
        if (HAS_DROP && drop_thresh) {
          const unsigned long long idx =
              (bh * (unsigned long long)s + my_q) *
                  (unsigned long long)s + kcol;
          dpv = (fa_hash(drop_seed, idx) < drop_thresh)
                    ? 0.f : dpv * keep_scale;
        }
        pk[j] = fa_bf16bits(pv * (dpv - dlt_r) * scale);
      }
      *reinterpret_cast<long*>(&p_x[wave][ln][8 * g + 4 * hi]) =
          *reinterpret_cast<const long*>(pk);
    }
    __builtin_amdgcn_s_waitcnt(0);

#pragma unroll
    for (int c2 = 0; c2 < 2; ++c2) {
      bf16x8 pa = *reinterpret_cast<const bf16x8*>(
          &p_x[wave][ln][c2 * 16 + hi * 8]);
#pragma unroll
      for (int t = 0; t < NTO; ++t) {
        const int dcol = t * 32 + ln;
        bf16x8 kb = *reinterpret_cast<const bf16x8*>(
            &kt_lds[dcol][(c2 * 16 + hi * 8) ^ (dcol & 0x18)]);
        dq_acc[t] = __builtin_amdgcn_mfma_f32_32x32x16_bf16(pa, kb,
                                                            dq_acc[t],
                                                            0, 0, 0);
      }
    }
  }

  if (!q_active) return;
#pragma unroll
  for (int r = 0; r < 16; ++r) {
    const int qrow = q0w + (r & 3) + 8 * (r >> 2) + 4 * hi;
#pragma unroll
    for (int t = 0; t < NTO; ++t)
      dQp[(long)qrow * D + t * 32 + ln] = __float2bfloat16(dq_acc[t][r]);
  }
}

template <int D, bool CAUSAL, bool HAS_DROP>
__global__ __launch_bounds__(FA_WAVES * 64)
void flash_attn_bwd_dkv_v3_kernel(const bf16_t* __restrict__ Q,
                                  const bf16_t* __restrict__ K,
                                  const bf16_t* __restrict__ V,
                                  const bf16_t* __restrict__ dO,
                                  const float* __restrict__ LSE,
                                  const float* __restrict__ Delta,
                                  bf16_t* __restrict__ dK,
                                  bf16_t* __restrict__ dV,
                                  const int* __restrict__ klens,
                                  int b, int h, int s, float scale,
                                  unsigned int drop_thresh, float keep_scale,
                                  unsigned long long drop_seed) {
  constexpr int NC = D / 16;
  constexpr int NTO = D / 32;
  constexpr int SWB = fa_swb(D);

  __shared__ char q_raw[B3_FB * SWB];
  __shared__ char do_raw[B3_FB * SWB];
  __shared__ short qt_lds[D][B3_FB + FA_VPAD];
  __shared__ short dot_lds[D][B3_FB + FA_VPAD];
  __shared__ short p_x[FA_WAVES][32][B3_FB + FA_VPAD];
  __shared__ short ds_x[FA_WAVES][32][B3_FB + FA_VPAD];

  const int lane = threadIdx.x & 63;
  const int wave = threadIdx.x >> 6;
  const int hi = lane >> 5;
  const int ln = lane & 31;
  const long bh = (long)blockIdx.z * h + blockIdx.y;
  const bf16_t* Qp = Q + bh * s * D;
  const bf16_t* Kp = K + bh * s * D;
  const bf16_t* Vp = V + bh * s * D;
  const bf16_t* dOp = dO + bh * s * D;
  bf16_t* dKp = dK + bh * s * D;
  bf16_t* dVp = dV + bh * s * D;
  const float* lse = LSE + bh * s;
  const float* dlt = Delta + bh * s;

  const int klen = CAUSAL ? s : min(klens ? klens[blockIdx.z] : s, s);
  const int kv0_blk = blockIdx.x * V3_QBLK;
  const int kv0w = kv0_blk + wave * 32;
  const bool kv_active = kv0w < s;
  const int kv0c = kv_active ? kv0w : s - 32;
  const int my_kv = kv0c + ln;

  f32x16 dv_acc[NTO], dk_acc[NTO];
#pragma unroll
  for (int t = 0; t < NTO; ++t) {
#pragma unroll
    for (int r = 0; r < 16; ++r) {
      dv_acc[t][r] = 0.f;
      dk_acc[t][r] = 0.f;
    }
  }

  const int first_qt = CAUSAL ? kv0_blk / B3_FB : 0;
  const int n_q_tiles = s / B3_FB;

  for (int qt = first_qt; qt < n_q_tiles; ++qt) {
    const int q_base = qt * B3_FB;
    __syncthreads();
    {
      const int tid = threadIdx.x;
      for (int i = tid * 8; i < B3_FB * D; i += FA_WAVES * 64 * 8) {
        const int qr = i / D;
        const int qc = i % D;
        bf16x8 qq = *reinterpret_cast<const bf16x8*>(
            Qp + (long)(q_base + qr) * D + qc);
        *reinterpret_cast<bf16x8*>(q_raw + qr * SWB + kswz(qr, qc * 2)) = qq;
        bf16x8 dd = *reinterpret_cast<const bf16x8*>(
            dOp + (long)(q_base + qr) * D + qc);
        *reinterpret_cast<bf16x8*>(do_raw + qr * SWB + kswz(qr, qc * 2)) =
            dd;
#pragma unroll
        for (int j = 0; j < 8; ++j) {
          qt_lds[qc + j][qr ^ ((qc + j) & 0x18)] = qq[j];
          dot_lds[qc + j][qr ^ ((qc + j) & 0x18)] = dd[j];
        }
      }
    }
    __syncthreads();

    f32x16 st;
#pragma unroll
    for (int r = 0; r < 16; ++r) st[r] = 0.f;
#pragma unroll
    for (int c = 0; c < NC; ++c) {
      bf16x8 ka = *reinterpret_cast<const bf16x8*>(
          Kp + (long)my_kv * D + c * 16 + hi * 8);
      bf16x8 qb = *reinterpret_cast<const bf16x8*>(
          q_raw + ln * SWB + kswz(ln, (c * 16 + hi * 8) * 2));
      st = __builtin_amdgcn_mfma_f32_32x32x16_bf16(ka, qb, st, 0, 0, 0);
    }
    f32x16 dpt;
#pragma unroll
    for (int r = 0; r < 16; ++r) dpt[r] = 0.f;
#pragma unroll
    for (int c = 0; c < NC; ++c) {
      bf16x8 va = *reinterpret_cast<const bf16x8*>(
          Vp + (long)my_kv * D + c * 16 + hi * 8);
      bf16x8 db = *reinterpret_cast<const bf16x8*>(
          do_raw + ln * SWB + kswz(ln, (c * 16 + hi * 8) * 2));
      dpt = __builtin_amdgcn_mfma_f32_32x32x16_bf16(va, db, dpt, 0, 0, 0);
    }

    const int qcol = q_base + ln;
    const float lse_c = lse[qcol];
    const float dlt_c = dlt[qcol];

#pragma unroll
    for (int r = 0; r < 16; ++r) {
      const int kvrow_loc = (r & 3) + 8 * (r >> 2) + 4 * hi;
      const int kvrow = kv0c + kvrow_loc;
      const bool masked = CAUSAL ? (qcol < kvrow) : (kvrow >= klen);
      float pv = masked ? 0.f : __expf(st[r] * scale - lse_c);
      float dm = 1.f;
      if (HAS_DROP && drop_thresh) {
        const unsigned long long idx =
            (bh * (unsigned long long)s + qcol) *
                (unsigned long long)s + kvrow;
        dm = (fa_hash(drop_seed, idx) < drop_thresh) ? 0.f : keep_scale;
      }
      p_x[wave][kvrow_loc][ln] = fa_bf16bits(pv * dm);
      ds_x[wave][kvrow_loc][ln] =
          fa_bf16bits(pv * (dm * dpt[r] - dlt_c) * scale);
    }
    __builtin_amdgcn_s_waitcnt(0);

#pragma unroll
    for (int c2 = 0; c2 < 2; ++c2) {
      bf16x8 pa = *reinterpret_cast<const bf16x8*>(
          &p_x[wave][ln][c2 * 16 + hi * 8]);
#pragma unroll
      for (int t = 0; t < NTO; ++t) {
        const int dcol = t * 32 + ln;
        bf16x8 bfrag = *reinterpret_cast<const bf16x8*>(
            &dot_lds[dcol][(c2 * 16 + hi * 8) ^ (dcol & 0x18)]);
        dv_acc[t] = __builtin_amdgcn_mfma_f32_32x32x16_bf16(
            pa, bfrag, dv_acc[t], 0, 0, 0);
      }
    }

#pragma unroll
    for (int c2 = 0; c2 < 2; ++c2) {
      bf16x8 pa = *reinterpret_cast<const bf16x8*>(
          &ds_x[wave][ln][c2 * 16 + hi * 8]);
#pragma unroll
      for (int t = 0; t < NTO; ++t) {
        const int dcol = t * 32 + ln;
        bf16x8 bfrag = *reinterpret_cast<const bf16x8*>(
            &qt_lds[dcol][(c2 * 16 + hi * 8) ^ (dcol & 0x18)]);
        dk_acc[t] = __builtin_amdgcn_mfma_f32_32x32x16_bf16(
            pa, bfrag, dk_acc[t], 0, 0, 0);
      }
    }
  }

  if (!kv_active) return;
#pragma unroll
  for (int r = 0; r < 16; ++r) {
    const int kvrow = kv0w + (r & 3) + 8 * (r >> 2) + 4 * hi;
#pragma unroll
    for (int t = 0; t < NTO; ++t) {
      dKp[(long)kvrow * D + t * 32 + ln] = __float2bfloat16(dk_acc[t][r]);
      dVp[(long)kvrow * D + t * 32 + ln] = __float2bfloat16(dv_acc[t][r]);
    }
  }
}

template <int D, bool CAUSAL, bool HAS_DROP>
static void launch_bwd_v3(const void* q, const void* k, const void* v,
                          const void* o, const void* dout, const float* lse,
                          void* dq, void* dk, void* dv, float* delta_ws,
                          const int* klens, int b, int h, int s, float scale,
                          unsigned int dth, float ksc,
                          unsigned long long seed, hipStream_t stream) {
  const long rows = (long)b * h * s;
  {
    long blocks = (rows + 3) / 4;
    if (blocks > 4096) blocks = 4096;
    hipLaunchKernelGGL((flash_delta_kernel<D>), dim3((unsigned)blocks),
                       dim3(256), 0, stream, (const bf16_t*)dout,
                       (const bf16_t*)o, delta_ws, rows);
  }
  dim3 grid((s + V3_QBLK - 1) / V3_QBLK, h, b);
  dim3 block(FA_WAVES * 64);
  hipLaunchKernelGGL((flash_attn_bwd_dq_v3_kernel<D, CAUSAL, HAS_DROP>),
                     grid, block, 0, stream, (const bf16_t*)q,
                     (const bf16_t*)k, (const bf16_t*)v, (const bf16_t*)dout,
                     lse, delta_ws, (bf16_t*)dq, klens, b, h, s, scale, dth,
                     ksc, seed);
  hipLaunchKernelGGL((flash_attn_bwd_dkv_v3_kernel<D, CAUSAL, HAS_DROP>),
                     grid, block, 0, stream, (const bf16_t*)q,
                     (const bf16_t*)k, (const bf16_t*)v, (const bf16_t*)dout,
                     lse, delta_ws, (bf16_t*)dk, (bf16_t*)dv, klens, b, h, s,
                     scale, dth, ksc, seed);
}

extern "C" void fs_flash_attn_bwd_v3(const void* q, const void* k,
                                     const void* v, const void* o,
                                     const void* dout, const float* lse,
                                     void* dq, void* dk, void* dv,
                                     float* delta_ws, const int* klens,
                                     int b, int h, int s, int d, int causal,
                                     float scale, float drop_p,
                                     unsigned long long seed,
                                     hipStream_t stream) {
  const unsigned int dth =
      (drop_p > 0.f) ? (unsigned int)(drop_p * 4294967296.0) : 0u;
  const float ksc = (drop_p > 0.f) ? 1.f / (1.f - drop_p) : 1.f;
#define BWD3(DD, CC, DR) launch_bwd_v3<DD, CC, DR>( \
      q, k, v, o, dout, lse, dq, dk, dv, delta_ws, klens, b, h, s, scale, \
      dth, ksc, seed, stream)
  if (dth) {
    if (d == 128 && causal) BWD3(128, true, true);
    else if (d == 128) BWD3(128, false, true);
    else if (d == 96 && causal) BWD3(96, true, true);
    else if (d == 96) BWD3(96, false, true);
    else if (d == 64 && causal) BWD3(64, true, true);
    else BWD3(64, false, true);
  } else {
    if (d == 128 && causal) BWD3(128, true, false);
    else if (d == 128) BWD3(128, false, false);
    else if (d == 96 && causal) BWD3(96, true, false);
    else if (d == 96) BWD3(96, false, false);
    else if (d == 64 && causal) BWD3(64, true, false);
    else BWD3(64, false, false);
  }
#undef BWD3
}
```

fengshen_amd/ops/csrc/kernels.hip:

```cpp

#include "common.h"

enum FsDtype { FS_F32 = 0, FS_BF16 = 1, FS_F16 = 2 };

template <typename T>
__global__ void rms_norm_fwd_kernel(const T* __restrict__ x,
                                    const T* __restrict__ w,
                                    T* __restrict__ out,
                                    float* __restrict__ invrms,
                                    int rows, int H, float eps) {
  extern __shared__ float lds[];
  __shared__ float red[32];
  for (int row = blockIdx.x; row < rows; row += gridDim.x) {
    const T* xr = x + (long)row * H;
    T* yr = out + (long)row * H;
    float ss = 0.f;
    for (int c = threadIdx.x * 8; c < H; c += blockDim.x * 8) {
      float v[8];
      load8<T>(xr + c, v);
#pragma unroll
      for (int i = 0; i < 8; ++i) {
        lds[c + i] = v[i];
        ss += v[i] * v[i];
      }
    }
    ss = block_reduce_sum(ss, red);
    float ir = rsqrtf(ss / H + eps);
    if (threadIdx.x == 0 && invrms) invrms[row] = ir;
    for (int c = threadIdx.x * 8; c < H; c += blockDim.x * 8) {
      float wv[8], o[8];
      load8<T>(w + c, wv);
#pragma unroll
      for (int i = 0; i < 8; ++i) o[i] = lds[c + i] * ir * wv[i];
      store8<T>(yr + c, o);
    }
    __syncthreads();
  }
}

template <typename T>
__global__ void rms_norm_bwd_kernel(const T* __restrict__ gy,
                                    const T* __restrict__ x,
                                    const T* __restrict__ w,
                                    const float* __restrict__ invrms,
                                    T* __restrict__ gx,
                                    float* __restrict__ gw_f32,
                                    int rows, int H) {
  extern __shared__ float lds[];
  __shared__ float red[32];
  float* xhat_s = lds;
  float* gyw_s = lds + H;
  float* gw_s = lds + 2 * H;
  for (int c = threadIdx.x; c < H; c += blockDim.x) gw_s[c] = 0.f;
  __syncthreads();
  for (int row = blockIdx.x; row < rows; row += gridDim.x) {
    const T* xr = x + (long)row * H;
    const T* gr = gy + (long)row * H;
    T* gxr = gx + (long)row * H;
    const float ir = invrms[row];
    float dot = 0.f;
    for (int c = threadIdx.x * 8; c < H; c += blockDim.x * 8) {
      float xv[8], gv[8], wv[8];
      load8<T>(xr + c, xv);
      load8<T>(gr + c, gv);
      load8<T>(w + c, wv);
#pragma unroll
      for (int i = 0; i < 8; ++i) {
        float xh = xv[i] * ir;
        float gw_ = gv[i] * wv[i];
        xhat_s[c + i] = xh;
        gyw_s[c + i] = gw_;
        dot += gw_ * xh;
        gw_s[c + i] += gv[i] * xh;
      }
    }
    dot = block_reduce_sum(dot, red) / H;
    for (int c = threadIdx.x * 8; c < H; c += blockDim.x * 8) {
      float o[8];
#pragma unroll
      for (int i = 0; i < 8; ++i)
        o[i] = ir * (gyw_s[c + i] - xhat_s[c + i] * dot);
      store8<T>(gxr + c, o);
    }
    __syncthreads();
  }
  for (int c = threadIdx.x; c < H; c += blockDim.x)
    atomicAdd(&gw_f32[c], gw_s[c]);
}

template <typename T>
__global__ void layer_norm_fwd_kernel(const T* __restrict__ x,
                                      const T* __restrict__ w,
                                      const T* __restrict__ b,
                                      T* __restrict__ out,
                                      float* __restrict__ mean_out,
                                      float* __restrict__ invstd_out,
                                      int rows, int H, float eps) {
  extern __shared__ float lds[];
  __shared__ float red[32];
  for (int row = blockIdx.x; row < rows; row += gridDim.x) {
    const T* xr = x + (long)row * H;
    T* yr = out + (long)row * H;
    float s = 0.f;
    for (int c = threadIdx.x * 8; c < H; c += blockDim.x * 8) {
      float v[8];
      load8<T>(xr + c, v);
#pragma unroll
      for (int i = 0; i < 8; ++i) {
        lds[c + i] = v[i];
        s += v[i];
      }
    }
    float mu = block_reduce_sum(s, red) / H;
    float var = 0.f;
    for (int c = threadIdx.x * 8; c < H; c += blockDim.x * 8) {
#pragma unroll
      for (int i = 0; i < 8; ++i) {
        float d = lds[c + i] - mu;
        var += d * d;
      }
    }
    var = block_reduce_sum(var, red) / H;
    float is = rsqrtf(var + eps);
    if (threadIdx.x == 0) {
      if (mean_out) mean_out[row] = mu;
      if (invstd_out) invstd_out[row] = is;
    }
    for (int c = threadIdx.x * 8; c < H; c += blockDim.x * 8) {
      float wv[8], bv[8], o[8];
      load8<T>(w + c, wv);
      if (b) load8<T>(b + c, bv);
#pragma unroll
      for (int i = 0; i < 8; ++i) {
        o[i] = (lds[c + i] - mu) * is * wv[i] + (b ? bv[i] : 0.f);
      }
      store8<T>(yr + c, o);
    }
    __syncthreads();
  }
}

template <typename T>
__global__ void layer_norm_bwd_kernel(const T* __restrict__ gy,
                                      const T* __restrict__ x,
                                      const T* __restrict__ w,
                                      const float* __restrict__ mean,
                                      const float* __restrict__ invstd,
                                      T* __restrict__ gx,
                                      float* __restrict__ gw_f32,
                                      float* __restrict__ gb_f32,
                                      int rows, int H) {
  extern __shared__ float lds[];
  __shared__ float red[32];
  float* xhat_s = lds;
  float* gyw_s = lds + H;
  float* gw_s = lds + 2 * H;
  float* gb_s = lds + 3 * H;
  for (int c = threadIdx.x; c < H; c += blockDim.x) {
    gw_s[c] = 0.f;
    gb_s[c] = 0.f;
  }
  __syncthreads();
  for (int row = blockIdx.x; row < rows; row += gridDim.x) {
    const T* xr = x + (long)row * H;
    const T* gr = gy + (long)row * H;
    T* gxr = gx + (long)row * H;
    const float mu = mean[row];
    const float is = invstd[row];
    float dot = 0.f, gsum = 0.f;
    for (int c = threadIdx.x * 8; c < H; c += blockDim.x * 8) {
      float xv[8], gv[8], wv[8];
      load8<T>(xr + c, xv);
      load8<T>(gr + c, gv);
      load8<T>(w + c, wv);
#pragma unroll
      for (int i = 0; i < 8; ++i) {
        float xh = (xv[i] - mu) * is;
        float gw_ = gv[i] * wv[i];
        xhat_s[c + i] = xh;
        gyw_s[c + i] = gw_;
        dot += gw_ * xh;
        gsum += gw_;
        gw_s[c + i] += gv[i] * xh;
        gb_s[c + i] += gv[i];
      }
    }
    dot = block_reduce_sum(dot, red) / H;
    gsum = block_reduce_sum(gsum, red) / H;
    for (int c = threadIdx.x * 8; c < H; c += blockDim.x * 8) {
      float o[8];
#pragma unroll
      for (int i = 0; i < 8; ++i)
        o[i] = is * (gyw_s[c + i] - gsum - xhat_s[c + i] * dot);
      store8<T>(gxr + c, o);
    }
    __syncthreads();
  }
  for (int c = threadIdx.x; c < H; c += blockDim.x) {
    atomicAdd(&gw_f32[c], gw_s[c]);
    if (gb_f32) atomicAdd(&gb_f32[c], gb_s[c]);
  }
}

template <typename T, int MODE>
__global__ void scaled_softmax_fwd_kernel(const T* __restrict__ x,
                                          const unsigned char* __restrict__ mask,
                                          T* __restrict__ out, float scale,
                                          int rows, int sk, int sq,
                                          int np, int mask_batches,
                                          int mask_sq) {
  extern __shared__ float lds[];
  __shared__ float red[32];
  for (int row = blockIdx.x; row < rows; row += gridDim.x) {
    const T* xr = x + (long)row * sk;
    T* yr = out + (long)row * sk;
    const int si = row % sq;
    const unsigned char* mr = nullptr;
    if (MODE == 1) {
      const int bi = row / (np * sq);
      const int mb = (mask_batches == 1) ? 0 : bi;
      const int msi = (mask_sq == 1) ? 0 : si;
      mr = mask + ((long)mb * mask_sq + msi) * sk;
    }
    const int limit = (MODE == 2) ? (si + 1) : sk;

    float mx = -INFINITY;
    int c = threadIdx.x * 8;
    for (; c + 7 < limit; c += blockDim.x * 8) {
      float v[8];
      load8<T>(xr + c, v);
#pragma unroll
      for (int i = 0; i < 8; ++i) {
        float val = v[i] * scale;
        if (MODE == 1 && mr[c + i]) val = -10000.f;
        lds[c + i] = val;
        mx = fmaxf(mx, val);
      }
    }
    for (int t = (limit & ~7) + threadIdx.x; t < limit; t += blockDim.x) {
      float val = to_f32<T>(xr[t]) * scale;
      if (MODE == 1 && mr[t]) val = -10000.f;
      lds[t] = val;
      mx = fmaxf(mx, val);
    }
    mx = block_reduce_max(mx, red);
    float sum = 0.f;
    for (int t = threadIdx.x; t < limit; t += blockDim.x) {
      float e = __expf(lds[t] - mx);
      lds[t] = e;
      sum += e;
    }
    sum = block_reduce_sum(sum, red);
    const float inv = 1.f / sum;
    for (int t = threadIdx.x; t < limit; t += blockDim.x)
      lds[t] *= inv;
    __syncthreads();
    for (c = threadIdx.x * 8; c + 7 < sk; c += blockDim.x * 8) {
      float o[8];
#pragma unroll
      for (int i = 0; i < 8; ++i) o[i] = (c + i < limit) ? lds[c + i] : 0.f;
      store8<T>(yr + c, o);
    }
    for (int t = (sk & ~7) + threadIdx.x; t < sk; t += blockDim.x)
      yr[t] = from_f32<T>(t < limit ? lds[t] : 0.f);
    __syncthreads();
  }
}

template <typename T>
__global__ void scaled_softmax_bwd_kernel(const T* __restrict__ gy,
                                          const T* __restrict__ y,
                                          T* __restrict__ gx, float scale,
                                          int rows, int sk) {
  extern __shared__ float lds[];
  __shared__ float red[32];
  float* ys = lds;
  float* gs = lds + sk;
  for (int row = blockIdx.x; row < rows; row += gridDim.x) {
    const T* yr = y + (long)row * sk;
    const T* gr = gy + (long)row * sk;
    T* gxr = gx + (long)row * sk;
    float dot = 0.f;
    int c = threadIdx.x * 8;
    for (; c + 7 < sk; c += blockDim.x * 8) {
      float yv[8], gv[8];
      load8<T>(yr + c, yv);
      load8<T>(gr + c, gv);
#pragma unroll
      for (int i = 0; i < 8; ++i) {
        ys[c + i] = yv[i];
        gs[c + i] = gv[i];
        dot += yv[i] * gv[i];
      }
    }
    for (int t = (sk & ~7) + threadIdx.x; t < sk; t += blockDim.x) {
      float yv = to_f32<T>(yr[t]);
      float gv = to_f32<T>(gr[t]);
      ys[t] = yv;
      gs[t] = gv;
      dot += yv * gv;
    }
    dot = block_reduce_sum(dot, red);
    for (c = threadIdx.x * 8; c + 7 < sk; c += blockDim.x * 8) {
      float o[8];
#pragma unroll
      for (int i = 0; i < 8; ++i)
        o[i] = scale * ys[c + i] * (gs[c + i] - dot);
      store8<T>(gxr + c, o);
    }
    for (int t = (sk & ~7) + threadIdx.x; t < sk; t += blockDim.x)
      gxr[t] = from_f32<T>(scale * ys[t] * (gs[t] - dot));
    __syncthreads();
  }
}

template <typename T, bool BWD>
__global__ void rope_kernel(const T* __restrict__ x, T* __restrict__ out,
                            const float* __restrict__ cos_t,
                            const float* __restrict__ sin_t,
                            long total_pairs, int s, int h2, int offset) {
  const long stride = (long)gridDim.x * blockDim.x * 8;
  for (long i = (long)(blockIdx.x * blockDim.x + threadIdx.x) * 8;
       i < total_pairs; i += stride) {
    const long d = i % h2;
    const long si = (i / h2) % s;
    const long bn = i / ((long)h2 * s);
    const long base = (bn * s + si) * (2 * h2);
    const float* cr = cos_t + (si + offset) * (2 * h2) + d;
    const float* sr = sin_t + (si + offset) * (2 * h2) + d;
    float x1[8], x2[8], o1[8], o2[8];
    load8<T>(x + base + d, x1);
    load8<T>(x + base + d + h2, x2);
#pragma unroll
    for (int j = 0; j < 8; ++j) {
      const float c = cr[j];
      const float sn = sr[j];
      if (!BWD) {
        o1[j] = x1[j] * c - x2[j] * sn;
        o2[j] = x2[j] * c + x1[j] * sn;
      } else {
        o1[j] = x1[j] * c + x2[j] * sn;
        o2[j] = x2[j] * c - x1[j] * sn;
      }
    }
    store8<T>(out + base + d, o1);
    store8<T>(out + base + d + h2, o2);
  }
}

template <typename T>
__global__ void swiglu_fwd_kernel(const T* __restrict__ packed,
                                  T* __restrict__ out, long rows, int h) {
  const long total = rows * (long)h;
  const long stride = (long)gridDim.x * blockDim.x * 8;
  for (long i = (long)(blockIdx.x * blockDim.x + threadIdx.x) * 8; i < total;
       i += stride) {
    const long row = i / h;
    const long col = i % h;
    const T* g = packed + row * 2 * h + col;
    const T* u = g + h;
    float gv[8], uv[8], o[8];
    load8<T>(g, gv);
    load8<T>(u, uv);
#pragma unroll
    for (int j = 0; j < 8; ++j) {
      const float sig = 1.f / (1.f + __expf(-gv[j]));
      o[j] = gv[j] * sig * uv[j];
    }
    store8<T>(out + i, o);
  }
}

template <typename T>
__global__ void swiglu_bwd_kernel(const T* __restrict__ gy,
                                  const T* __restrict__ packed,
                                  T* __restrict__ gpacked, long rows, int h) {
  const long total = rows * (long)h;
  const long stride = (long)gridDim.x * blockDim.x * 8;
  for (long i = (long)(blockIdx.x * blockDim.x + threadIdx.x) * 8; i < total;
       i += stride) {
    const long row = i / h;
    const long col = i % h;
    const T* g = packed + row * 2 * h + col;
    const T* u = g + h;
    float gv[8], uv[8], go[8], dg[8], du[8];
    load8<T>(g, gv);
    load8<T>(u, uv);
    load8<T>(gy + i, go);
#pragma unroll
    for (int j = 0; j < 8; ++j) {
      const float sig = 1.f / (1.f + __expf(-gv[j]));
      const float silu = gv[j] * sig;
      dg[j] = go[j] * uv[j] * sig * (1.f + gv[j] * (1.f - sig));
      du[j] = go[j] * silu;
    }
    store8<T>(gpacked + row * 2 * h + col, dg);
    store8<T>(gpacked + row * 2 * h + col + h, du);
  }
}

__device__ __forceinline__ float gelu_tanh(float y) {
  return y * 0.5f * (1.f + tanhf(0.79788456f * y * (1.f + 0.044715f * y * y)));
}
__device__ __forceinline__ float gelu_tanh_grad(float y) {
  const float t = tanhf(0.79788456f * y * (1.f + 0.044715f * y * y));
  return 0.5f * y * ((1.f - t * t) * (0.79788456f + 0.1070322243f * y * y)) +
         0.5f * (1.f + t);
}

template <typename T, bool BWD>
__global__ void bias_gelu_kernel(const T* __restrict__ x,
                                 const T* __restrict__ bias,
                                 const T* __restrict__ gy,
                                 T* __restrict__ out, long rows, int h) {
  const long total = rows * (long)h;
  const long stride = (long)gridDim.x * blockDim.x * 8;
  for (long i = (long)(blockIdx.x * blockDim.x + threadIdx.x) * 8; i < total;
       i += stride) {
    const long col = i % h;
    float xv[8], bv[8], o[8];
    load8<T>(x + i, xv);
    load8<T>(bias + col, bv);
    if (!BWD) {
#pragma unroll
      for (int j = 0; j < 8; ++j) o[j] = gelu_tanh(xv[j] + bv[j]);
    } else {
      float gv[8];
      load8<T>(gy + i, gv);
#pragma unroll
      for (int j = 0; j < 8; ++j)
        o[j] = gelu_tanh_grad(xv[j] + bv[j]) * gv[j];
    }
    store8<T>(out + i, o);
  }
}

template <typename GT, typename OT>
__global__ void fused_adamw_kernel(float* __restrict__ master,
                                   const GT* __restrict__ grad,
                                   float* __restrict__ m,
                                   float* __restrict__ v,
                                   OT* __restrict__ out_param,
                                   long n, float lr, float beta1, float beta2,
                                   float eps, float wd, float bc1, float bc2) {
  const long n4 = n & ~3L;
  const long stride = (long)gridDim.x * blockDim.x * 4;
  for (long i = (long)(blockIdx.x * blockDim.x + threadIdx.x) * 4; i < n4;
       i += stride) {
    float4_t p = *reinterpret_cast<float4_t*>(master + i);
    float4_t mj = *reinterpret_cast<float4_t*>(m + i);
    float4_t vj = *reinterpret_cast<float4_t*>(v + i);
    float g[4];
#pragma unroll
    for (int j = 0; j < 4; ++j) g[j] = to_f32<GT>(grad[i + j]);
#pragma unroll
    for (int j = 0; j < 4; ++j) {
      float pj = p[j] * (1.f - lr * wd);
      float mm = beta1 * mj[j] + (1.f - beta1) * g[j];
      float vv = beta2 * vj[j] + (1.f - beta2) * g[j] * g[j];
      const float denom = sqrtf(vv / bc2) + eps;
      pj -= lr / bc1 * (mm / denom);
      p[j] = pj;
      mj[j] = mm;
      vj[j] = vv;
    }
    *reinterpret_cast<float4_t*>(master + i) = p;
    *reinterpret_cast<float4_t*>(m + i) = mj;
    *reinterpret_cast<float4_t*>(v + i) = vj;
    if (out_param) {
#pragma unroll
      for (int j = 0; j < 4; ++j) out_param[i + j] = from_f32<OT>(p[j]);
    }
  }
  for (long t = n4 + blockIdx.x * blockDim.x + threadIdx.x; t < n;
       t += (long)gridDim.x * blockDim.x) {
    float g = to_f32<GT>(grad[t]);
    float pj = master[t] * (1.f - lr * wd);
    float mm = m[t] = beta1 * m[t] + (1.f - beta1) * g;
    float vv = v[t] = beta2 * v[t] + (1.f - beta2) * g * g;
    pj -= lr / bc1 * (mm / (sqrtf(vv / bc2) + eps));
    master[t] = pj;
    if (out_param) out_param[t] = from_f32<OT>(pj);
  }
}

template <typename T, int MODE>
__global__ void scaled_softmax_fwd_wave_kernel(
    const T* __restrict__ x, const unsigned char* __restrict__ mask,
    T* __restrict__ out, float scale, long rows, int sk, int sq,
    int np, int mask_batches, int mask_sq) {
  const int lane = threadIdx.x & 63;
  const int wid = threadIdx.x >> 6;
  const int nchunks = (sk + 511) / 512;
  float v[32];
  for (long row = (long)blockIdx.x * 4 + wid; row < rows;
       row += (long)gridDim.x * 4) {
    const T* xr = x + row * sk;
    T* yr = out + row * sk;
    const int si = (int)(row % sq);
    const unsigned char* mr = nullptr;
    if (MODE == 1) {
      const long bi = row / ((long)np * sq);
      const long mb = (mask_batches == 1) ? 0 : bi;
      const int msi = (mask_sq == 1) ? 0 : si;
      mr = mask + ((long)mb * mask_sq + msi) * sk;
    }
    const int limit = (MODE == 2) ? (si + 1) : sk;

    float mx = -INFINITY;
#pragma unroll 4
    for (int c = 0; c < nchunks; ++c) {
      const int base = c * 512 + lane * 8;
      if (base < sk) {
        float t[8];
        load8<T>(xr + base, t);
#pragma unroll
        for (int j = 0; j < 8; ++j) {
          float val = t[j] * scale;
          if (MODE == 1 && mr[base + j]) val = -10000.f;
          if (MODE == 2 && base + j >= limit) val = -INFINITY;
          v[c * 8 + j] = val;
          mx = fmaxf(mx, val);
        }
      }
    }
    mx = wave_reduce_max(mx);
    float sum = 0.f;
#pragma unroll 4
    for (int c = 0; c < nchunks; ++c) {
      const int base = c * 512 + lane * 8;
      if (base < sk) {
#pragma unroll
        for (int j = 0; j < 8; ++j) {
          float e = (v[c * 8 + j] == -INFINITY) ? 0.f
                                                : __expf(v[c * 8 + j] - mx);
          v[c * 8 + j] = e;
          sum += e;
        }
      }
    }
    sum = wave_reduce_sum(sum);
    const float inv = 1.f / sum;
#pragma unroll 4
    for (int c = 0; c < nchunks; ++c) {
      const int base = c * 512 + lane * 8;
      if (base < sk) {
        float o[8];
#pragma unroll
        for (int j = 0; j < 8; ++j) o[j] = v[c * 8 + j] * inv;
        store8<T>(yr + base, o);
      }
    }
  }
}

template <typename T>
__global__ void scaled_softmax_bwd_wave_kernel(
    const T* __restrict__ gy, const T* __restrict__ y, T* __restrict__ gx,
    float scale, long rows, int sk) {
  const int lane = threadIdx.x & 63;
  const int wid = threadIdx.x >> 6;
  const int nchunks = (sk + 511) / 512;
  float yv[32], gv[32];
  for (long row = (long)blockIdx.x * 4 + wid; row < rows;
       row += (long)gridDim.x * 4) {
    const T* yr = y + row * sk;
    const T* gr = gy + row * sk;
    T* gxr = gx + row * sk;
    float dot = 0.f;
#pragma unroll 4
    for (int c = 0; c < nchunks; ++c) {
      const int base = c * 512 + lane * 8;
      if (base < sk) {
        float ty[8], tg[8];
        load8<T>(yr + base, ty);
        load8<T>(gr + base, tg);
#pragma unroll
        for (int j = 0; j < 8; ++j) {
          yv[c * 8 + j] = ty[j];
          gv[c * 8 + j] = tg[j];
          dot += ty[j] * tg[j];
        }
      }
    }
    dot = wave_reduce_sum(dot);
#pragma unroll 4
    for (int c = 0; c < nchunks; ++c) {
      const int base = c * 512 + lane * 8;
      if (base < sk) {
        float o[8];
#pragma unroll
        for (int j = 0; j < 8; ++j)
          o[j] = scale * yv[c * 8 + j] * (gv[c * 8 + j] - dot);
        store8<T>(gxr + base, o);
      }
    }
  }
}

static inline int grid_for(long work_items, int block = 256) {
  long g = (work_items + block - 1) / block;
  if (g > FS_MAX_BLOCKS) g = FS_MAX_BLOCKS;
  if (g < 1) g = 1;
  return (int)g;
}

#define DISPATCH_DTYPE(dtype, T, ...)            \
  switch (dtype) {                               \
    case FS_F32: { using T = float; __VA_ARGS__; break; }   \
    case FS_BF16: { using T = bf16_t; __VA_ARGS__; break; } \
    case FS_F16: { using T = fp16_t; __VA_ARGS__; break; }  \
  }

extern "C" {

void fs_rms_norm_fwd(const void* x, const void* w, void* out, float* invrms,
                     int rows, int H, float eps, int dtype, hipStream_t s) {
  int grid = rows < FS_MAX_BLOCKS ? rows : FS_MAX_BLOCKS;
  size_t lds = (size_t)H * 4;
  DISPATCH_DTYPE(dtype, T,
    hipLaunchKernelGGL((rms_norm_fwd_kernel<T>), dim3(grid), dim3(256), lds, s,
                       (const T*)x, (const T*)w, (T*)out, invrms, rows, H, eps));
}

void fs_rms_norm_bwd(const void* gy, const void* x, const void* w,
                     const float* invrms, void* gx, float* gw_f32, int rows,
                     int H, int dtype, hipStream_t s) {
  int grid = rows < FS_MAX_BLOCKS ? rows : FS_MAX_BLOCKS;
  size_t lds = (size_t)H * 12;
  DISPATCH_DTYPE(dtype, T,
    hipLaunchKernelGGL((rms_norm_bwd_kernel<T>), dim3(grid), dim3(256), lds, s,
                       (const T*)gy, (const T*)x, (const T*)w, invrms, (T*)gx,
                       gw_f32, rows, H));
}

void fs_layer_norm_fwd(const void* x, const void* w, const void* b, void* out,
                       float* mean, float* invstd, int rows, int H, float eps,
                       int dtype, hipStream_t s) {
  int grid = rows < FS_MAX_BLOCKS ? rows : FS_MAX_BLOCKS;
  size_t lds = (size_t)H * 4;
  DISPATCH_DTYPE(dtype, T,
    hipLaunchKernelGGL((layer_norm_fwd_kernel<T>), dim3(grid), dim3(256), lds, s,
                       (const T*)x, (const T*)w, (const T*)b, (T*)out, mean,
                       invstd, rows, H, eps));
}

void fs_layer_norm_bwd(const void* gy, const void* x, const void* w,
                       const float* mean, const float* invstd, void* gx,
                       float* gw_f32, float* gb_f32, int rows, int H, int dtype,
                       hipStream_t s) {
  int grid = rows < FS_MAX_BLOCKS ? rows : FS_MAX_BLOCKS;
  size_t lds = (size_t)H * 16;
  DISPATCH_DTYPE(dtype, T,
    hipLaunchKernelGGL((layer_norm_bwd_kernel<T>), dim3(grid), dim3(256), lds, s,
                       (const T*)gy, (const T*)x, (const T*)w, mean, invstd,
                       (T*)gx, gw_f32, gb_f32, rows, H));
}

void fs_scaled_softmax_fwd(const void* x, const unsigned char* mask, void* out,
                           float scale, int rows, int sk, int sq, int np,
                           int mask_batches, int mask_sq, int mode, int dtype,
                           hipStream_t s) {
  if (sk <= 2048 && sk % 8 == 0) {
    long wgrid = ((long)rows + 3) / 4;
    if (wgrid > 4096) wgrid = 4096;
    DISPATCH_DTYPE(dtype, T, {
      if (mode == 0)
        hipLaunchKernelGGL((scaled_softmax_fwd_wave_kernel<T, 0>),
                           dim3((unsigned)wgrid), dim3(256), 0, s,
                           (const T*)x, mask, (T*)out, scale, (long)rows, sk,
                           sq, np, mask_batches, mask_sq);
      else if (mode == 1)
        hipLaunchKernelGGL((scaled_softmax_fwd_wave_kernel<T, 1>),
                           dim3((unsigned)wgrid), dim3(256), 0, s,
                           (const T*)x, mask, (T*)out, scale, (long)rows, sk,
                           sq, np, mask_batches, mask_sq);
      else
        hipLaunchKernelGGL((scaled_softmax_fwd_wave_kernel<T, 2>),
                           dim3((unsigned)wgrid), dim3(256), 0, s,
                           (const T*)x, mask, (T*)out, scale, (long)rows, sk,
                           sq, np, mask_batches, mask_sq);
    });
    return;
  }
  int grid = rows < FS_MAX_BLOCKS ? rows : FS_MAX_BLOCKS;
  size_t lds = (size_t)sk * 4;
  DISPATCH_DTYPE(dtype, T, {
    if (mode == 0)
      hipLaunchKernelGGL((scaled_softmax_fwd_kernel<T, 0>), dim3(grid),
                         dim3(256), lds, s, (const T*)x, mask, (T*)out, scale,
                         rows, sk, sq, np, mask_batches, mask_sq);
    else if (mode == 1)
      hipLaunchKernelGGL((scaled_softmax_fwd_kernel<T, 1>), dim3(grid),
                         dim3(256), lds, s, (const T*)x, mask, (T*)out, scale,
                         rows, sk, sq, np, mask_batches, mask_sq);
    else
      hipLaunchKernelGGL((scaled_softmax_fwd_kernel<T, 2>), dim3(grid),
                         dim3(256), lds, s, (const T*)x, mask, (T*)out, scale,
                         rows, sk, sq, np, mask_batches, mask_sq);
  });
}

void fs_scaled_softmax_bwd(const void* gy, const void* y, void* gx, float scale,
                           int rows, int sk, int dtype, hipStream_t s) {
  if (sk <= 2048 && sk % 8 == 0) {
    long wgrid = ((long)rows + 3) / 4;
    if (wgrid > 4096) wgrid = 4096;
    DISPATCH_DTYPE(dtype, T,
      hipLaunchKernelGGL((scaled_softmax_bwd_wave_kernel<T>),
                         dim3((unsigned)wgrid), dim3(256), 0, s,
                         (const T*)gy, (const T*)y, (T*)gx, scale, (long)rows,
                         sk));
    return;
  }
  int grid = rows < FS_MAX_BLOCKS ? rows : FS_MAX_BLOCKS;
  size_t lds = (size_t)sk * 8;
  DISPATCH_DTYPE(dtype, T,
    hipLaunchKernelGGL((scaled_softmax_bwd_kernel<T>), dim3(grid), dim3(256),
                       lds, s, (const T*)gy, (const T*)y, (T*)gx, scale, rows,
                       sk));
}

void fs_rope(const void* x, void* out, const float* cos_t, const float* sin_t,
             long bn, int seq, int hn, int offset, int bwd, int dtype,
             hipStream_t s) {
  const int h2 = hn / 2;
  const long total_pairs = bn * (long)seq * h2;
  int grid = grid_for(total_pairs / 8);
  DISPATCH_DTYPE(dtype, T, {
    if (bwd)
      hipLaunchKernelGGL((rope_kernel<T, true>), dim3(grid), dim3(256), 0, s,
                         (const T*)x, (T*)out, cos_t, sin_t, total_pairs, seq,
                         h2, offset);
    else
      hipLaunchKernelGGL((rope_kernel<T, false>), dim3(grid), dim3(256), 0, s,
                         (const T*)x, (T*)out, cos_t, sin_t, total_pairs, seq,
                         h2, offset);
  });
}

void fs_swiglu_fwd(const void* packed, void* out, long rows, int h, int dtype,
                   hipStream_t s) {
  int grid = grid_for(rows * (long)h / 8);
  DISPATCH_DTYPE(dtype, T,
    hipLaunchKernelGGL((swiglu_fwd_kernel<T>), dim3(grid), dim3(256), 0, s,
                       (const T*)packed, (T*)out, rows, h));
}

void fs_swiglu_bwd(const void* gy, const void* packed, void* gpacked, long rows,
                   int h, int dtype, hipStream_t s) {
  int grid = grid_for(rows * (long)h / 8);
  DISPATCH_DTYPE(dtype, T,
    hipLaunchKernelGGL((swiglu_bwd_kernel<T>), dim3(grid), dim3(256), 0, s,
                       (const T*)gy, (const T*)packed, (T*)gpacked, rows, h));
}

void fs_bias_gelu(const void* x, const void* bias, const void* gy, void* out,
                  long rows, int h, int bwd, int dtype, hipStream_t s) {
  int grid = grid_for(rows * (long)h / 8);
  DISPATCH_DTYPE(dtype, T, {
    if (bwd)
      hipLaunchKernelGGL((bias_gelu_kernel<T, true>), dim3(grid), dim3(256), 0,
                         s, (const T*)x, (const T*)bias, (const T*)gy, (T*)out,
                         rows, h);
    else
      hipLaunchKernelGGL((bias_gelu_kernel<T, false>), dim3(grid), dim3(256), 0,
                         s, (const T*)x, (const T*)bias, (const T*)gy, (T*)out,
                         rows, h);
  });
}

void fs_fused_adamw(float* master, const void* grad, float* m, float* v,
                    void* out_param, long n, float lr, float beta1, float beta2,
                    float eps, float wd, int step, int grad_dtype,
                    int out_dtype, hipStream_t s) {
  const float bc1 = 1.f - powf(beta1, (float)step);
  const float bc2 = 1.f - powf(beta2, (float)step);
  int grid = grid_for((n + 3) / 4);
  DISPATCH_DTYPE(grad_dtype, GT, {
    DISPATCH_DTYPE(out_dtype, OT, {
      hipLaunchKernelGGL((fused_adamw_kernel<GT, OT>), dim3(grid), dim3(256), 0,
                         s, master, (const GT*)grad, m, v, (OT*)out_param, n,
                         lr, beta1, beta2, eps, wd, bc1, bc2);
    });
  });
}

}

typedef char char16_t_v __attribute__((ext_vector_type(16)));

__global__ __launch_bounds__(256)
void w8_gemv_kernel(const signed char* __restrict__ q8,
                    const float* __restrict__ scale,
                    const bf16_t* __restrict__ x,
                    bf16_t* __restrict__ y,
                    int batch, int in_features, int out_features) {
  const int lane = threadIdx.x & 63;
  const int wid = threadIdx.x >> 6;
  const int row0 = blockIdx.x * 4 + wid;
  for (int row = row0; row < out_features; row += gridDim.x * 4) {
    const signed char* wr = q8 + (long)row * in_features;
    for (int b = 0; b < batch; ++b) {
      const bf16_t* xb = x + (long)b * in_features;
      float acc = 0.f;
      for (int i = lane * 16; i + 15 < in_features; i += 64 * 16) {
        char16_t_v w = *reinterpret_cast<const char16_t_v*>(wr + i);
        float xv[8], xv2[8];
        load8<bf16_t>(xb + i, xv);
        load8<bf16_t>(xb + i + 8, xv2);
#pragma unroll
        for (int j = 0; j < 8; ++j) {
          acc += (float)w[j] * xv[j];
          acc += (float)w[j + 8] * xv2[j];
        }
      }
      acc = wave_reduce_sum(acc);
      if (lane == 0) y[(long)b * out_features + row] =
          from_f32<bf16_t>(acc * scale[row]);
    }
  }
}

extern "C" void fs_w8_gemv(const void* q8, const float* scale, const void* x,
                           void* y, int batch, int in_features,
                           int out_features, hipStream_t s) {
  int grid = (out_features + 3) / 4;
  if (grid > FS_MAX_BLOCKS) grid = FS_MAX_BLOCKS;
  hipLaunchKernelGGL(w8_gemv_kernel, dim3(grid), dim3(256), 0, s,
                     (const signed char*)q8, scale, (const bf16_t*)x,
                     (bf16_t*)y, batch, in_features, out_features);
}


__global__ void add_rms_norm_kernel(const bf16_t* __restrict__ a,
                                    const bf16_t* __restrict__ b,
                                    const bf16_t* __restrict__ w,
                                    bf16_t* __restrict__ sum_out,
                                    bf16_t* __restrict__ y,
                                    int rows, int H, float eps) {
  extern __shared__ float lds[];
  __shared__ float red[32];
  for (int row = blockIdx.x; row < rows; row += gridDim.x) {
    const bf16_t* ar = a + (long)row * H;
    const bf16_t* br = b + (long)row * H;
    float ss = 0.f;
    for (int c = threadIdx.x * 8; c < H; c += blockDim.x * 8) {
      float va[8], vb[8], o[8];
      load8<bf16_t>(ar + c, va);
      load8<bf16_t>(br + c, vb);
#pragma unroll
      for (int i = 0; i < 8; ++i) {
        o[i] = va[i] + vb[i];
        lds[c + i] = o[i];
        ss += o[i] * o[i];
      }
      store8<bf16_t>(sum_out + (long)row * H + c, o);
    }
    ss = block_reduce_sum(ss, red);
    const float ir = rsqrtf(ss / H + eps);
    for (int c = threadIdx.x * 8; c < H; c += blockDim.x * 8) {
      float wv[8], o[8];
      load8<bf16_t>(w + c, wv);
#pragma unroll
      for (int i = 0; i < 8; ++i) o[i] = lds[c + i] * ir * wv[i];
      store8<bf16_t>(y + (long)row * H + c, o);
    }
    __syncthreads();
  }
}

extern "C" void fs_add_rms_norm(const void* a, const void* b, const void* w,
                                void* sum_out, void* y, int rows, int H,
                                float eps, hipStream_t s) {
  int grid = rows < FS_MAX_BLOCKS ? rows : FS_MAX_BLOCKS;
  size_t lds = (size_t)H * 4;
  hipLaunchKernelGGL(add_rms_norm_kernel, dim3(grid), dim3(256), lds, s,
                     (const bf16_t*)a, (const bf16_t*)b, (const bf16_t*)w,
                     (bf16_t*)sum_out, (bf16_t*)y, rows, H, eps);
}


template <int B>
__global__ __launch_bounds__(256)
void bf16_gemv_kernel(const bf16_t* __restrict__ w,
                      const bf16_t* __restrict__ x,
                      bf16_t* __restrict__ y,
                      int in_features, int out_features) {
  const int lane = threadIdx.x & 63;
  const int wid = threadIdx.x >> 6;
  for (int row = blockIdx.x * 4 + wid; row < out_features;
       row += gridDim.x * 4) {
    const bf16_t* wr = w + (long)row * in_features;
    float acc[B];
#pragma unroll
    for (int b = 0; b < B; ++b) acc[b] = 0.f;
    for (int i = lane * 16; i + 15 < in_features; i += 64 * 16) {
      float wv[8], wv2[8];
      load8<bf16_t>(wr + i, wv);
      load8<bf16_t>(wr + i + 8, wv2);
#pragma unroll
      for (int b = 0; b < B; ++b) {
        const bf16_t* xb = x + (long)b * in_features;
        float xv[8], xv2[8];
        load8<bf16_t>(xb + i, xv);
        load8<bf16_t>(xb + i + 8, xv2);
#pragma unroll
        for (int j = 0; j < 8; ++j)
          acc[b] += wv[j] * xv[j] + wv2[j] * xv2[j];
      }
    }
#pragma unroll
    for (int b = 0; b < B; ++b) {
      float r = wave_reduce_sum(acc[b]);
      if (lane == 0)
        y[(long)b * out_features + row] = from_f32<bf16_t>(r);
    }
  }
}

extern "C" void fs_bf16_gemv(const void* w, const void* x, void* y, int batch,
                             int in_features, int out_features,
                             hipStream_t s) {
  int grid = (out_features + 3) / 4;
  if (grid > FS_MAX_BLOCKS) grid = FS_MAX_BLOCKS;
#define FS_GEMV_CASE(B)                                                      \
  case B:                                                                    \
    hipLaunchKernelGGL((bf16_gemv_kernel<B>), dim3(grid), dim3(256), 0, s,   \
                       (const bf16_t*)w, (const bf16_t*)x, (bf16_t*)y,       \
                       in_features, out_features);                           \
    break;
  switch (batch) {
    FS_GEMV_CASE(1) FS_GEMV_CASE(2) FS_GEMV_CASE(3) FS_GEMV_CASE(4)
    FS_GEMV_CASE(5) FS_GEMV_CASE(6) FS_GEMV_CASE(7) FS_GEMV_CASE(8)
  }
#undef FS_GEMV_CASE
}


#define FS_DEC_BLK 128

template <int D, bool ROPE>
__global__ __launch_bounds__(FS_DEC_BLK)
void decode_attn_kernel(const bf16_t* __restrict__ qkv,
                        bf16_t* __restrict__ kc, bf16_t* __restrict__ vc,
                        const float* __restrict__ cos_t,
                        const float* __restrict__ sin_t,
                        const long* __restrict__ pos_p,
                        bf16_t* __restrict__ ctx,
                        int nh, int cache_len, float scale) {
  const int tid = threadIdx.x;
  const int bh = blockIdx.x;
  const int b = bh / nh, h = bh % nh;
  const int pos = (int)pos_p[0];
  const int H = nh * D;

  __shared__ float qraw[D], kraw[D];
  __shared__ float qs[D], ks_new[D];
  __shared__ float red[16];
  __shared__ float pbuf[FS_DEC_BLK];
  __shared__ float ktile[FS_DEC_BLK][D + 1];

  float v_new = 0.f;
  if (tid < D) {
    qraw[tid] = to_f32<bf16_t>(qkv[(long)b * 3 * H + h * D + tid]);
    kraw[tid] = to_f32<bf16_t>(qkv[(long)b * 3 * H + H + h * D + tid]);
    v_new = to_f32<bf16_t>(qkv[(long)b * 3 * H + 2 * H + h * D + tid]);
  }
  __syncthreads();
  if (tid < D) {
    float q = qraw[tid], k = kraw[tid];
    if (ROPE) {
      float c = cos_t[(long)pos * D + tid];
      float s = sin_t[(long)pos * D + tid];
      float qr = (tid < D / 2) ? -qraw[tid + D / 2] : qraw[tid - D / 2];
      float kr = (tid < D / 2) ? -kraw[tid + D / 2] : kraw[tid - D / 2];
      q = q * c + qr * s;
      k = k * c + kr * s;
    }
    qs[tid] = q * scale;
    ks_new[tid] = k;
    const long coff = (((long)b * nh + h) * cache_len + pos) * D + tid;
    kc[coff] = from_f32<bf16_t>(k);
    vc[coff] = from_f32<bf16_t>(v_new);
  }
  __threadfence();
  __syncthreads();

  const bf16_t* kbase = kc + ((long)b * nh + h) * (long)cache_len * D;
  const bf16_t* vbase = vc + ((long)b * nh + h) * (long)cache_len * D;
  float m_run = -INFINITY, l_run = 0.f, oacc = 0.f;
  for (int p0 = 0; p0 <= pos; p0 += FS_DEC_BLK) {
    const int nrow = min(FS_DEC_BLK, pos + 1 - p0);
    for (int idx = tid * 8; idx < nrow * D; idx += FS_DEC_BLK * 8) {
      const int r = idx / D, c = idx % D;
      float kv[8];
      load8<bf16_t>(kbase + (long)(p0 + r) * D + c, kv);
#pragma unroll
      for (int j = 0; j < 8; ++j) ktile[r][c + j] = kv[j];
    }
    __syncthreads();
    if (pos >= p0 && pos < p0 + FS_DEC_BLK && tid < D)
      ktile[pos - p0][tid] = ks_new[tid];
    __syncthreads();
    float s_t = -INFINITY;
    if (tid < nrow) {
      float acc = 0.f;
#pragma unroll
      for (int j = 0; j < D; j += 8) {
#pragma unroll
        for (int jj = 0; jj < 8; ++jj)
          acc += qs[j + jj] * ktile[tid][j + jj];
      }
      s_t = acc;
    }
    const float m_chunk = block_reduce_max(s_t, red);
    const float m_new = fmaxf(m_run, m_chunk);
    const float alpha = __expf(m_run - m_new);
    const float pr = (tid < nrow) ? __expf(s_t - m_new) : 0.f;
    pbuf[tid] = pr;
    const float psum = block_reduce_sum(pr, red);
    l_run = l_run * alpha + psum;
    m_run = m_new;
    if (tid < D) {
      float acc = oacc * alpha;
      for (int t = 0; t < nrow; ++t)
        acc += pbuf[t] * to_f32<bf16_t>(vbase[(long)(p0 + t) * D + tid]);
      oacc = acc;
    }
    __syncthreads();
  }
  if (tid < D)
    ctx[(long)b * H + h * D + tid] = from_f32<bf16_t>(oacc / l_run);
}

extern "C" void fs_decode_attn(const void* qkv, void* kc, void* vc,
                               const float* cos_t, const float* sin_t,
                               const void* pos, void* ctx, int b, int nh,
                               int d, int cache_len, float scale, int rope,
                               hipStream_t s) {
#define FS_DEC_CASE(D)                                                       \
  if (d == D) {                                                              \
    if (rope)                                                                \
      hipLaunchKernelGGL((decode_attn_kernel<D, true>), dim3(b * nh),        \
                         dim3(FS_DEC_BLK), 0, s, (const bf16_t*)qkv,         \
                         (bf16_t*)kc, (bf16_t*)vc, cos_t, sin_t,             \
                         (const long*)pos, (bf16_t*)ctx, nh, cache_len,      \
                         scale);                                             \
    else                                                                     \
      hipLaunchKernelGGL((decode_attn_kernel<D, false>), dim3(b * nh),       \
                         dim3(FS_DEC_BLK), 0, s, (const bf16_t*)qkv,         \
                         (bf16_t*)kc, (bf16_t*)vc, cos_t, sin_t,             \
                         (const long*)pos, (bf16_t*)ctx, nh, cache_len,      \
                         scale);                                             \
    return;                                                                  \
  }
  FS_DEC_CASE(64)
  FS_DEC_CASE(128)
#undef FS_DEC_CASE
}


__global__ __launch_bounds__(256)
void vocab_ce_fwd_kernel(const bf16_t* __restrict__ logits,
                         const long* __restrict__ targets,
                         float* __restrict__ m_out,
                         float* __restrict__ z_out,
                         float* __restrict__ pred_out,
                         long n, int w, int vstart, int vend) {
  __shared__ float red[8];
  for (long row = blockIdx.x; row < n; row += gridDim.x) {
    const bf16_t* lp = logits + row * w;
    float m = -INFINITY;
    for (int j = threadIdx.x * 8; j < w; j += 256 * 8) {
      short8_t v8 = *reinterpret_cast<const short8_t*>(lp + j);
#pragma unroll
      for (int k = 0; k < 8; ++k) {
        unsigned short u = (unsigned short)v8[k];
        m = fmaxf(m, __uint_as_float(((unsigned int)u) << 16));
      }
    }
    m = block_reduce_max(m, red);
    __syncthreads();
    float z = 0.f;
    for (int j = threadIdx.x * 8; j < w; j += 256 * 8) {
      short8_t v8 = *reinterpret_cast<const short8_t*>(lp + j);
#pragma unroll
      for (int k = 0; k < 8; ++k) {
        unsigned short u = (unsigned short)v8[k];
        z += __expf(__uint_as_float(((unsigned int)u) << 16) - m);
      }
    }
    z = block_reduce_sum(z, red);
    if (threadIdx.x == 0) {
      m_out[row] = m;
      z_out[row] = z;
      const long t = targets[row];
      float pred = 0.f;
      if (t >= vstart && t < vend)
        pred = __bfloat162float(lp[t - vstart]);
      pred_out[row] = pred;
    }
    __syncthreads();
  }
}

__global__ __launch_bounds__(256)
void vocab_ce_bwd_kernel(const bf16_t* __restrict__ logits,
                         const long* __restrict__ targets,
                         const float* __restrict__ m_in,
                         const float* __restrict__ z_in,
                         const float* __restrict__ gout,
                         bf16_t* __restrict__ dlogits,
                         long n, int w, int vstart, int vend) {
  for (long row = blockIdx.x; row < n; row += gridDim.x) {
    const bf16_t* lp = logits + row * w;
    bf16_t* gp = dlogits + row * w;
    const float m = m_in[row];
    const float inv_z = 1.f / z_in[row];
    const float g = gout[row];
    const long t = targets[row] - vstart;
    for (int j = threadIdx.x * 8; j < w; j += 256 * 8) {
      short8_t v8 = *reinterpret_cast<const short8_t*>(lp + j);
      short8_t o8;
#pragma unroll
      for (int k = 0; k < 8; ++k) {
        unsigned short u = (unsigned short)v8[k];
        float d = __expf(__uint_as_float(((unsigned int)u) << 16) - m)
                  * inv_z;
        if (j + k == t) d -= 1.f;
        o8[k] = (short)__hip_bfloat16_raw(__float2bfloat16(d * g)).x;
      }
      *reinterpret_cast<short8_t*>(gp + j) = o8;
    }
  }
}

extern "C" void fs_vocab_ce_fwd(const void* logits, const long* targets,
                                float* m_out, float* z_out, float* pred_out,
                                long n, int w, int vstart, int vend,
                                hipStream_t stream) {
  long blocks = n < FS_MAX_BLOCKS ? n : FS_MAX_BLOCKS;
  hipLaunchKernelGGL(vocab_ce_fwd_kernel, dim3((unsigned)blocks), dim3(256),
                     0, stream, (const bf16_t*)logits, targets, m_out, z_out,
                     pred_out, n, w, vstart, vend);
}

extern "C" void fs_vocab_ce_bwd(const void* logits, const long* targets,
                                const float* m_in, const float* z_in,
                                const float* gout, void* dlogits, long n,
                                int w, int vstart, int vend,
                                hipStream_t stream) {
  long blocks = n < FS_MAX_BLOCKS ? n : FS_MAX_BLOCKS;
  hipLaunchKernelGGL(vocab_ce_bwd_kernel, dim3((unsigned)blocks), dim3(256),
                     0, stream, (const bf16_t*)logits, targets, m_in, z_in,
                     gout, (bf16_t*)dlogits, n, w, vstart, vend);
}
```

fengshen_amd/ops/flash.py:

```python
from __future__ import annotations

from typing import Optional

import torch

from fengshen_amd.ops import get_ext

_FLASH_DIMS = (40, 64, 80, 96, 128, 160)


def _v3_eligible(ext, q, k, causal, klens, dropout_p):
    if not (hasattr(ext, "flash_attn_fwd_v3")
            and q.shape[-1] in (64, 96, 128)
            and q.shape[-2] == k.shape[-2]
            and q.shape[-2] % 64 == 0 and q.shape[-2] >= 64):
        return False
    if dropout_p > 0:
        import os
        return os.environ.get("FENGSHEN_FLASH_V3_DROP") == "1" \
            and q.shape[-1] in (64, 96)
    return True


class _FlashAttention(torch.autograd.Function):
    @staticmethod
    def forward(ctx, q, k, v, scale, causal, klens, dropout_p, seed):
        ext = get_ext()
        if _v3_eligible(ext, q, k, causal, klens, dropout_p):
            o, lse = ext.flash_attn_fwd_v3(q, k, v, scale, causal, klens,
                                           dropout_p, seed)
        else:
            o, lse = ext.flash_attn_fwd(q, k, v, scale, causal, klens,
                                        dropout_p, seed)
        ctx.save_for_backward(q, k, v, o, lse)
        ctx.scale = scale
        ctx.causal = causal
        ctx.klens = klens
        ctx.dropout_p = dropout_p
        ctx.seed = seed
        return o

    @staticmethod
    def backward(ctx, do):
        q, k, v, o, lse = ctx.saved_tensors
        ext = get_ext()
        if _v3_eligible(ext, q, k, ctx.causal, ctx.klens, ctx.dropout_p):
            dq, dk, dv = ext.flash_attn_bwd_v3(
                q, k, v, o, do.contiguous(), lse, ctx.scale, ctx.causal,
                ctx.klens, ctx.dropout_p, ctx.seed)
        else:
            dq, dk, dv = ext.flash_attn_bwd(
                q, k, v, o, do.contiguous(), lse, ctx.scale, ctx.causal,
                ctx.klens, ctx.dropout_p, ctx.seed)
        return dq, dk, dv, None, None, None, None, None


def _draw_seed(device) -> int:
    base = int(torch.randint(0, 2 ** 62, (1,)).item())
    try:
        from fengshen_amd.parallel import groups as pg
        base += pg.get_tensor_model_parallel_rank() * 0x9E3779B9
    except Exception:
        pass
    return base


def flash_attention(q: torch.Tensor, k: torch.Tensor, v: torch.Tensor,
                    scale: float, causal: bool = True,
                    klens: Optional[torch.Tensor] = None,
                    dropout_p: float = 0.0) -> torch.Tensor:
    seed = _draw_seed(q.device) if dropout_p > 0 else 0
    return _FlashAttention.apply(q.contiguous(), k.contiguous(),
                                 v.contiguous(), scale, causal, klens,
                                 float(dropout_p), seed)


def mask_to_klens(mask: torch.Tensor, sk: int) -> Optional[torch.Tensor]:
    if mask.dtype != torch.bool:
        mask = mask != 0
    if mask.dim() == 4:
        if mask.shape[2] != 1 or mask.shape[1] != 1 or mask.shape[3] != sk:
            return None
        m2 = mask[:, 0, 0, :]
    elif mask.dim() == 2 and mask.shape[1] == sk:
        m2 = mask
    else:
        return None
    klens = (~m2).sum(dim=1, dtype=torch.int32)
    ar = torch.arange(sk, device=mask.device, dtype=torch.int32)
    if not torch.equal(m2, ar.unsqueeze(0) >= klens.unsqueeze(1)):
        return None
    return klens.contiguous()


def flash_attn_supported(q, k, v, causal, mask, dropout_p) -> bool:
    if q.dtype != torch.bfloat16:
        return False
    if q.shape[-1] not in _FLASH_DIMS:
        return False
    sq, sk = q.shape[-2], k.shape[-2]
    if causal:
        return mask is None and sq == sk and sq % 64 == 0
    return sq % 16 == 0 and sq >= 16
```

Measured before the change: 9702 tokens/s.

## Run flash attention directly on packed QKV with strided views and in-place RoPE

Adds a packed self-attention path that reads q, k, v as strided views of the fused QKV projection output. It applies rotary embedding in place and writes attention output and gradients straight into [b, s, h] layouts. This removes the chunk/transpose/contiguous copies and the separate RoPE allocations in both forward and backward. The cost is strided kernel variants, the extra cos/sin precomputed tables, and in-place mutation of qkv, which relies on autograd mark_dirty being correct under activation checkpointing.

```diff
diff --git a/fengshen_amd/models/layers.py b/fengshen_amd/models/layers.py
--- a/fengshen_amd/models/layers.py
+++ b/fengshen_amd/models/layers.py
@@ -162,6 +162,28 @@
         hn = self.head_dim
 
         qkv = self.qkv_proj(x)
+
+        if cache is None and F_ops.use_hip(qkv):
+            from fengshen_amd.ops.flash import (
+                mask_to_klens, packed_attn_eligible, packed_self_attention)
+            drop = self.attention_dropout if self.training else 0.0
+            if packed_attn_eligible(qkv, hn, self.causal, attention_mask,
+                                    drop):
+                klens = None
+                if attention_mask is not None:
+                    klens = mask_to_klens(attention_mask, sq)
+                if attention_mask is None or klens is not None:
+                    cos = sin = None
+                    if self.rotary:
+                        cos, sin = self._rope_tables(qkv.device, sq)
+                    ctx = packed_self_attention(
+                        qkv, np_, cos, sin, 0, self.norm_factor,
+                        causal=self.causal, klens=klens)
+                    out = self.out_proj(ctx)
+                    if isinstance(out, tuple) and self.reduce_output:
+                        out = out[0]
+                    return out
+
         q, k, v = qkv.chunk(3, dim=-1)
         q = q.view(b, sq, np_, hn).transpose(1, 2)
         k = k.view(b, sq, np_, hn).transpose(1, 2)
diff --git a/fengshen_amd/ops/csrc/bindings.cpp b/fengshen_amd/ops/csrc/bindings.cpp
--- a/fengshen_amd/ops/csrc/bindings.cpp
+++ b/fengshen_amd/ops/csrc/bindings.cpp
@@ -71,6 +71,18 @@
                           const void*, const float*, void*, void*, void*,
                           float*, const int*, int, int, int, int, int, float,
                           float, unsigned long long, hipStream_t);
+void fs_flash_attn_fwd_v3_strided(const void*, const void*, const void*,
+                                  void*, float*, const int*, const long*,
+                                  const long*, int, int, int, int, int, float,
+                                  float, unsigned long long, hipStream_t);
+void fs_flash_attn_bwd_v3_strided(const void*, const void*, const void*,
+                                  const void*, const void*, const float*,
+                                  void*, void*, void*, float*, const int*,
+                                  const long*, const long*, const long*,
+                                  const long*, int, int, int, int, int, float,
+                                  float, unsigned long long, hipStream_t);
+void fs_rope_inplace(void*, void*, const float*, const float*, int, int, int,
+                     int, long, long, long, int, int, int, hipStream_t);
 }
 
 static std::vector<at::Tensor> rms_norm_fwd(at::Tensor x, at::Tensor w,
@@ -336,6 +348,131 @@
                     causal ? 1 : 0, (float)scale, (float)drop_p,
                     (unsigned long long)seed, cur_stream());
   return {dq, dk, dv};
+}
+
+static void check_strided_view(const at::Tensor& t, const char* name, int b,
+                               int h, int s, int d) {
+  TORCH_CHECK(t.is_cuda() && t.scalar_type() == at::kBFloat16, name,
+              ": must be a bf16 GPU tensor");
+  TORCH_CHECK(t.dim() == 4 && t.size(0) == b && t.size(1) == h &&
+                  t.size(2) == s && t.size(3) == d,
+              name, ": expected shape [", b, ", ", h, ", ", s, ", ", d, "]");
+  TORCH_CHECK(t.stride(3) == 1, name, ": last dim must be unit-stride");
+  for (int i = 0; i < 3; ++i)
+    TORCH_CHECK(t.stride(i) > 0 && t.stride(i) % 8 == 0, name, ": stride ", i,
+                " (", t.stride(i), ") must be a positive multiple of 8");
+  TORCH_CHECK(t.storage_offset() % 8 == 0 &&
+                  reinterpret_cast<uintptr_t>(t.data_ptr()) % 16 == 0,
+              name, ": base offset must be a multiple of 8 elements");
+  const int64_t last = t.storage_offset() + (b - 1) * t.stride(0) +
+                       (h - 1) * t.stride(1) + (s - 1) * t.stride(2) + d;
+  TORCH_CHECK(last * 2 <= (int64_t)t.storage().nbytes(), name,
+              ": view runs past its storage");
+}
+
+static void check_same_strides(const at::Tensor& a, const at::Tensor& b,
+                               const char* what) {
+  TORCH_CHECK(a.strides() == b.strides(), what, " must share strides");
+}
+
+static void strides3(const at::Tensor& t, long out[3]) {
+  out[0] = t.stride(0);
+  out[1] = t.stride(1);
+  out[2] = t.stride(2);
+}
+
+static const int* checked_klens(const c10::optional<at::Tensor>& klens,
+                                bool causal, int b) {
+  if (!klens.has_value()) return nullptr;
+  TORCH_CHECK(!causal, "flash v3: klens only with causal=False");
+  TORCH_CHECK(klens->is_cuda() && klens->scalar_type() == at::kInt &&
+              klens->numel() == b && klens->is_contiguous());
+  return klens->data_ptr<int>();
+}
+
+static at::Tensor flash_attn_fwd_v3_strided(
+    at::Tensor q, at::Tensor k, at::Tensor v, at::Tensor o, double scale,
+    bool causal, c10::optional<at::Tensor> klens) {
+  TORCH_CHECK(q.dim() == 4, "q must be [b, h, s, d]");
+  const int b = q.size(0), h = q.size(1), s = q.size(2), d = q.size(3);
+  TORCH_CHECK((d == 128 || d == 96 || d == 64) && s % 64 == 0 && s >= 64,
+              "flash v3: d in {64, 96, 128}, s a multiple of 64");
+  check_strided_view(q, "q", b, h, s, d);
+  check_strided_view(k, "k", b, h, s, d);
+  check_strided_view(v, "v", b, h, s, d);
+  check_strided_view(o, "o", b, h, s, d);
+  check_same_strides(q, k, "q and k");
+  check_same_strides(q, v, "q and v");
+  const int* klp = checked_klens(klens, causal, b);
+  long qs[3], os[3];
+  strides3(q, qs);
+  strides3(o, os);
+  auto lse = at::empty({b, h, s}, q.options().dtype(at::kFloat));
+  fs_flash_attn_fwd_v3_strided(q.data_ptr(), k.data_ptr(), v.data_ptr(),
+                               o.data_ptr(), lse.data_ptr<float>(), klp, qs,
+                               os, b, h, s, d, causal ? 1 : 0, (float)scale,
+                               0.f, 0ull, cur_stream());
+  return lse;
+}
+
+static void flash_attn_bwd_v3_strided(
+    at::Tensor q, at::Tensor k, at::Tensor v, at::Tensor o, at::Tensor dout,
+    at::Tensor lse, at::Tensor dq, at::Tensor dk, at::Tensor dv, double scale,
+    bool causal, c10::optional<at::Tensor> klens) {
+  TORCH_CHECK(q.dim() == 4, "q must be [b, h, s, d]");
+  const int b = q.size(0), h = q.size(1), s = q.size(2), d = q.size(3);
+  TORCH_CHECK((d == 128 || d == 96 || d == 64) && s % 64 == 0 && s >= 64,
+              "flash v3: d in {64, 96, 128}, s a multiple of 64");
+  check_strided_view(q, "q", b, h, s, d);
+  check_strided_view(k, "k", b, h, s, d);
+  check_strided_view(v, "v", b, h, s, d);
+  check_strided_view(o, "o", b, h, s, d);
+  check_strided_view(dout, "dout", b, h, s, d);
+  check_strided_view(dq, "dq", b, h, s, d);
+  check_strided_view(dk, "dk", b, h, s, d);
+  check_strided_view(dv, "dv", b, h, s, d);
+  check_same_strides(q, k, "q and k");
+  check_same_strides(q, v, "q and v");
+  check_same_strides(dq, dk, "dq and dk");
+  check_same_strides(dq, dv, "dq and dv");
+  TORCH_CHECK(lse.is_cuda() && lse.scalar_type() == at::kFloat &&
+              lse.is_contiguous() && lse.numel() == (int64_t)b * h * s,
+              "lse must be contiguous fp32 [b, h, s]");
+  const int* klp = checked_klens(klens, causal, b);
+  long qs[3], os[3], dos[3], gs[3];
+  strides3(q, qs);
+  strides3(o, os);
+  strides3(dout, dos);
+  strides3(dq, gs);
+  auto delta = at::empty({b, h, s}, q.options().dtype(at::kFloat));
+  fs_flash_attn_bwd_v3_strided(
+      q.data_ptr(), k.data_ptr(), v.data_ptr(), o.data_ptr(), dout.data_ptr(),
+      lse.data_ptr<float>(), dq.data_ptr(), dk.data_ptr(), dv.data_ptr(),
+      delta.data_ptr<float>(), klp, qs, os, dos, gs, b, h, s, d,
+      causal ? 1 : 0, (float)scale, 0.f, 0ull, cur_stream());
+}
+
+static void rope_inplace(at::Tensor q, at::Tensor k, at::Tensor cos,
+                         at::Tensor sin, int64_t offset, bool bwd) {
+  TORCH_CHECK(q.dim() == 4, "q must be [b, np, s, hn]");
+  const int b = q.size(0), np = q.size(1), s = q.size(2), hn = q.size(3);
+  TORCH_CHECK((hn / 2) % 8 == 0 && hn % 2 == 0,
+              "head_dim/2 must be divisible by 8");
+  check_strided_view(q, "q", b, np, s, hn);
+  check_strided_view(k, "k", b, np, s, hn);
+  check_same_strides(q, k, "q and k");
+  TORCH_CHECK(cos.is_cuda() && sin.is_cuda() &&
+              cos.scalar_type() == at::kFloat &&
+              sin.scalar_type() == at::kFloat && cos.is_contiguous() &&
+              sin.is_contiguous() && cos.dim() == 2 && cos.size(1) == hn &&
+              sin.sizes() == cos.sizes(),
+              "cos/sin must be contiguous fp32 [S, hn]");
+  TORCH_CHECK(offset >= 0 && offset + s <= cos.size(0),
+              "rope table too short for offset + s");
+  fs_rope_inplace(q.data_ptr(), k.data_ptr(), cos.data_ptr<float>(),
+                  sin.data_ptr<float>(), b, np, s, hn, q.stride(0),
+                  q.stride(1), q.stride(2), (int)offset, bwd ? 1 : 0,
+                  fs_dtype(q), cur_stream());
 }
 
 static at::Tensor w8_gemv(at::Tensor q8, at::Tensor scale, at::Tensor x) {
@@ -480,6 +617,9 @@
     return std::vector<at::Tensor>{o, lse};
   });
   mod.def("flash_attn_bwd", &flash_attn_bwd);
+  mod.def("flash_attn_fwd_v3_strided", &flash_attn_fwd_v3_strided);
+  mod.def("flash_attn_bwd_v3_strided", &flash_attn_bwd_v3_strided);
+  mod.def("rope_inplace", &rope_inplace);
   mod.def("rms_norm_fwd", &rms_norm_fwd);
   mod.def("rms_norm_bwd", &rms_norm_bwd);
   mod.def("layer_norm_fwd", &layer_norm_fwd);
diff --git a/fengshen_amd/ops/csrc/flash_attn.hip b/fengshen_amd/ops/csrc/flash_attn.hip
--- a/fengshen_amd/ops/csrc/flash_attn.hip
+++ b/fengshen_amd/ops/csrc/flash_attn.hip
@@ -902,6 +902,35 @@
 
 typedef __attribute__((ext_vector_type(16))) float f32x16;
 
+struct FaStrides {
+  long b, h, r;
+};
+
+template <int D>
+__global__ __launch_bounds__(256)
+void flash_delta_v3_kernel(const bf16_t* __restrict__ dO,
+                           const bf16_t* __restrict__ O,
+                           float* __restrict__ delta, FaStrides dos,
+                           FaStrides os, int h, int s) {
+  const int lane = threadIdx.x & 63;
+  const int wid = threadIdx.x >> 6;
+  const bf16_t* dob = dO + blockIdx.z * dos.b + blockIdx.y * dos.h;
+  const bf16_t* ob = O + blockIdx.z * os.b + blockIdx.y * os.h;
+  float* dl = delta + ((long)blockIdx.z * h + blockIdx.y) * s;
+  for (int row = blockIdx.x * 4 + wid; row < s; row += gridDim.x * 4) {
+    const bf16_t* dop = dob + row * dos.r;
+    const bf16_t* op = ob + row * os.r;
+    float sacc = 0.f;
+    for (int i = lane * 2; i < D; i += 128) {
+#pragma unroll
+      for (int j = 0; j < 2; ++j)
+        sacc += __bfloat162float(dop[i + j]) * __bfloat162float(op[i + j]);
+    }
+    sacc = wave_reduce_sum(sacc);
+    if (lane == 0) dl[row] = sacc;
+  }
+}
+
 template <int D, bool CAUSAL, bool HAS_DROP>
 __global__ __launch_bounds__(FA_WAVES * 64)
 void flash_attn_fwd_v3_kernel(const bf16_t* __restrict__ Q,
@@ -910,6 +939,7 @@
                               bf16_t* __restrict__ O,
                               float* __restrict__ LSE,
                               const int* __restrict__ klens,
+                              FaStrides qs, FaStrides os,
                               int b, int h, int s, float scale,
                               unsigned int drop_thresh, float keep_scale,
                               unsigned long long drop_seed) {
@@ -925,10 +955,11 @@
   const int hi = lane >> 5;
   const int ln = lane & 31;
   const long bh = (long)blockIdx.z * h + blockIdx.y;
-  const bf16_t* Qp = Q + bh * s * D;
-  const bf16_t* Kp = K + bh * s * D;
-  const bf16_t* Vp = V + bh * s * D;
-  bf16_t* Op = O + bh * s * D;
+  const long qoff = blockIdx.z * qs.b + blockIdx.y * qs.h;
+  const bf16_t* Qp = Q + qoff;
+  const bf16_t* Kp = K + qoff;
+  const bf16_t* Vp = V + qoff;
+  bf16_t* Op = O + blockIdx.z * os.b + blockIdx.y * os.h;
 
   const int klen = CAUSAL ? s : min(klens ? klens[blockIdx.z] : s, s);
 
@@ -941,7 +972,7 @@
 #pragma unroll
   for (int c = 0; c < NC; ++c) {
     bf16x8 raw = *reinterpret_cast<const bf16x8*>(
-        Qp + (long)my_q * D + c * 16 + hi * 8);
+        Qp + (long)my_q * qs.r + c * 16 + hi * 8);
 #pragma unroll
     for (int j = 0; j < 8; ++j) {
       unsigned short u = (unsigned short)raw[j];
@@ -978,8 +1009,8 @@
     if (i < ELEMS) {
       const long kr = min(i / D, s - 1);
       const int kc = i % D;
-      k_reg[sweep] = *reinterpret_cast<const bf16x8*>(Kp + kr * D + kc);
-      v_reg[sweep] = *reinterpret_cast<const bf16x8*>(Vp + kr * D + kc);
+      k_reg[sweep] = *reinterpret_cast<const bf16x8*>(Kp + kr * qs.r + kc);
+      v_reg[sweep] = *reinterpret_cast<const bf16x8*>(Vp + kr * qs.r + kc);
     }
   }
 
@@ -1011,8 +1042,8 @@
         if (i < ELEMS) {
           const long kr = min((long)(nb + i / D), (long)s - 1);
           const int kc = i % D;
-          k_reg[sweep] = *reinterpret_cast<const bf16x8*>(Kp + kr * D + kc);
-          v_reg[sweep] = *reinterpret_cast<const bf16x8*>(Vp + kr * D + kc);
+          k_reg[sweep] = *reinterpret_cast<const bf16x8*>(Kp + kr * qs.r + kc);
+          v_reg[sweep] = *reinterpret_cast<const bf16x8*>(Vp + kr * qs.r + kc);
         }
       }
     }
@@ -1157,7 +1188,7 @@
         __shfl(my_inv_l, (r & 3) + 8 * (r >> 2) + 4 * hi, 64);
 #pragma unroll
     for (int t = 0; t < NTO; ++t) {
-      Op[(long)qrow * D + t * 32 + ln] =
+      Op[(long)qrow * os.r + t * 32 + ln] =
           __float2bfloat16(o_acc[t][r] * inv_l);
     }
   }
@@ -1166,12 +1197,13 @@
   }
 }
 
-extern "C" void fs_flash_attn_fwd_v3(const void* q, const void* k,
-                                     const void* v, void* o, float* lse,
-                                     const int* klens, int b, int h, int s,
-                                     int d, int causal, float scale,
-                                     float drop_p, unsigned long long seed,
-                                     hipStream_t stream) {
+extern "C" void fs_flash_attn_fwd_v3_strided(
+    const void* q, const void* k, const void* v, void* o, float* lse,
+    const int* klens, const long* qs3, const long* os3, int b, int h, int s,
+    int d, int causal, float scale, float drop_p, unsigned long long seed,
+    hipStream_t stream) {
+  const FaStrides qs{qs3[0], qs3[1], qs3[2]};
+  const FaStrides os{os3[0], os3[1], os3[2]};
   dim3 grid((s + V3_QBLK - 1) / V3_QBLK, h, b);
   dim3 block(FA_WAVES * 64);
   const unsigned int dth =
@@ -1180,7 +1212,8 @@
 #define V3F(DD, CC, DR) hipLaunchKernelGGL( \
     (flash_attn_fwd_v3_kernel<DD, CC, DR>), \
     grid, block, 0, stream, (const bf16_t*)q, (const bf16_t*)k, \
-    (const bf16_t*)v, (bf16_t*)o, lse, klens, b, h, s, scale, dth, ksc, seed)
+    (const bf16_t*)v, (bf16_t*)o, lse, klens, qs, os, b, h, s, scale, dth, \
+    ksc, seed)
   if (dth) {
     if (d == 128 && causal) V3F(128, true, true);
     else if (d == 128) V3F(128, false, true);
@@ -1199,6 +1232,17 @@
 #undef V3F
 }
 
+extern "C" void fs_flash_attn_fwd_v3(const void* q, const void* k,
+                                     const void* v, void* o, float* lse,
+                                     const int* klens, int b, int h, int s,
+                                     int d, int causal, float scale,
+                                     float drop_p, unsigned long long seed,
+                                     hipStream_t stream) {
+  const long c3[3] = {(long)h * s * d, (long)s * d, (long)d};
+  fs_flash_attn_fwd_v3_strided(q, k, v, o, lse, klens, c3, c3, b, h, s, d,
+                               causal, scale, drop_p, seed, stream);
+}
+
 
 #define B3_FB 32
 
@@ -1212,6 +1256,7 @@
                                  const float* __restrict__ Delta,
                                  bf16_t* __restrict__ dQ,
                                  const int* __restrict__ klens,
+                                 FaStrides qs, FaStrides dos, FaStrides gs,
                                  int b, int h, int s, float scale,
                                  unsigned int drop_thresh, float keep_scale,
                                  unsigned long long drop_seed) {
@@ -1229,11 +1274,12 @@
   const int hi = lane >> 5;
   const int ln = lane & 31;
   const long bh = (long)blockIdx.z * h + blockIdx.y;
-  const bf16_t* Qp = Q + bh * s * D;
-  const bf16_t* Kp = K + bh * s * D;
-  const bf16_t* Vp = V + bh * s * D;
-  const bf16_t* dOp = dO + bh * s * D;
-  bf16_t* dQp = dQ + bh * s * D;
+  const long qoff = blockIdx.z * qs.b + blockIdx.y * qs.h;
+  const bf16_t* Qp = Q + qoff;
+  const bf16_t* Kp = K + qoff;
+  const bf16_t* Vp = V + qoff;
+  const bf16_t* dOp = dO + blockIdx.z * dos.b + blockIdx.y * dos.h;
+  bf16_t* dQp = dQ + blockIdx.z * gs.b + blockIdx.y * gs.h;
   const float* lse = LSE + bh * s;
   const float* dlt = Delta + bh * s;
 
@@ -1247,7 +1293,7 @@
 #pragma unroll
   for (int c = 0; c < NC; ++c) {
     bf16x8 raw = *reinterpret_cast<const bf16x8*>(
-        Qp + (long)my_q * D + c * 16 + hi * 8);
+        Qp + (long)my_q * qs.r + c * 16 + hi * 8);
 #pragma unroll
     for (int j = 0; j < 8; ++j) {
       unsigned short u = (unsigned short)raw[j];
@@ -1256,7 +1302,7 @@
     }
     q_frag[c] = raw;
     do_frag[c] = *reinterpret_cast<const bf16x8*>(
-        dOp + (long)my_q * D + c * 16 + hi * 8);
+        dOp + (long)my_q * dos.r + c * 16 + hi * 8);
   }
   const float lse_r = lse[my_q];
   const float dlt_r = dlt[my_q];
@@ -1285,9 +1331,9 @@
         const int kr = i / D;
         const int kc = i % D;
         const long krg = min(k_base + kr, s - 1);
-        bf16x8 kk = *reinterpret_cast<const bf16x8*>(Kp + krg * D + kc);
+        bf16x8 kk = *reinterpret_cast<const bf16x8*>(Kp + krg * qs.r + kc);
         *reinterpret_cast<bf16x8*>(k_raw + kr * SWB + kswz(kr, kc * 2)) = kk;
-        bf16x8 vv = *reinterpret_cast<const bf16x8*>(Vp + krg * D + kc);
+        bf16x8 vv = *reinterpret_cast<const bf16x8*>(Vp + krg * qs.r + kc);
         *reinterpret_cast<bf16x8*>(v_raw + kr * SWB + kswz(kr, kc * 2)) = vv;
 #pragma unroll
         for (int j = 0; j < 8; ++j)
@@ -1363,7 +1409,7 @@
     const int qrow = q0w + (r & 3) + 8 * (r >> 2) + 4 * hi;
 #pragma unroll
     for (int t = 0; t < NTO; ++t)
-      dQp[(long)qrow * D + t * 32 + ln] = __float2bfloat16(dq_acc[t][r]);
+      dQp[(long)qrow * gs.r + t * 32 + ln] = __float2bfloat16(dq_acc[t][r]);
   }
 }
 
@@ -1378,6 +1424,7 @@
                                   bf16_t* __restrict__ dK,
                                   bf16_t* __restrict__ dV,
                                   const int* __restrict__ klens,
+                                  FaStrides qs, FaStrides dos, FaStrides gs,
                                   int b, int h, int s, float scale,
                                   unsigned int drop_thresh, float keep_scale,
                                   unsigned long long drop_seed) {
@@ -1397,12 +1444,14 @@
   const int hi = lane >> 5;
   const int ln = lane & 31;
   const long bh = (long)blockIdx.z * h + blockIdx.y;
-  const bf16_t* Qp = Q + bh * s * D;
-  const bf16_t* Kp = K + bh * s * D;
-  const bf16_t* Vp = V + bh * s * D;
-  const bf16_t* dOp = dO + bh * s * D;
-  bf16_t* dKp = dK + bh * s * D;
-  bf16_t* dVp = dV + bh * s * D;
+  const long qoff = blockIdx.z * qs.b + blockIdx.y * qs.h;
+  const bf16_t* Qp = Q + qoff;
+  const bf16_t* Kp = K + qoff;
+  const bf16_t* Vp = V + qoff;
+  const bf16_t* dOp = dO + blockIdx.z * dos.b + blockIdx.y * dos.h;
+  const long goff = blockIdx.z * gs.b + blockIdx.y * gs.h;
+  bf16_t* dKp = dK + goff;
+  bf16_t* dVp = dV + goff;
   const float* lse = LSE + bh * s;
   const float* dlt = Delta + bh * s;
 
@@ -1435,10 +1484,10 @@
         const int qr = i / D;
         const int qc = i % D;
         bf16x8 qq = *reinterpret_cast<const bf16x8*>(
-            Qp + (long)(q_base + qr) * D + qc);
+            Qp + (long)(q_base + qr) * qs.r + qc);
         *reinterpret_cast<bf16x8*>(q_raw + qr * SWB + kswz(qr, qc * 2)) = qq;
         bf16x8 dd = *reinterpret_cast<const bf16x8*>(
-            dOp + (long)(q_base + qr) * D + qc);
+            dOp + (long)(q_base + qr) * dos.r + qc);
         *reinterpret_cast<bf16x8*>(do_raw + qr * SWB + kswz(qr, qc * 2)) =
             dd;
 #pragma unroll
@@ -1456,7 +1505,7 @@
 #pragma unroll
     for (int c = 0; c < NC; ++c) {
       bf16x8 ka = *reinterpret_cast<const bf16x8*>(
-          Kp + (long)my_kv * D + c * 16 + hi * 8);
+          Kp + (long)my_kv * qs.r + c * 16 + hi * 8);
       bf16x8 qb = *reinterpret_cast<const bf16x8*>(
           q_raw + ln * SWB + kswz(ln, (c * 16 + hi * 8) * 2));
       st = __builtin_amdgcn_mfma_f32_32x32x16_bf16(ka, qb, st, 0, 0, 0);
@@ -1467,7 +1516,7 @@
 #pragma unroll
     for (int c = 0; c < NC; ++c) {
       bf16x8 va = *reinterpret_cast<const bf16x8*>(
-          Vp + (long)my_kv * D + c * 16 + hi * 8);
+          Vp + (long)my_kv * qs.r + c * 16 + hi * 8);
       bf16x8 db = *reinterpret_cast<const bf16x8*>(
           do_raw + ln * SWB + kswz(ln, (c * 16 + hi * 8) * 2));
       dpt = __builtin_amdgcn_mfma_f32_32x32x16_bf16(va, db, dpt, 0, 0, 0);
@@ -1531,8 +1580,8 @@
     const int kvrow = kv0w + (r & 3) + 8 * (r >> 2) + 4 * hi;
 #pragma unroll
     for (int t = 0; t < NTO; ++t) {
-      dKp[(long)kvrow * D + t * 32 + ln] = __float2bfloat16(dk_acc[t][r]);
-      dVp[(long)kvrow * D + t * 32 + ln] = __float2bfloat16(dv_acc[t][r]);
+      dKp[(long)kvrow * gs.r + t * 32 + ln] = __float2bfloat16(dk_acc[t][r]);
+      dVp[(long)kvrow * gs.r + t * 32 + ln] = __float2bfloat16(dv_acc[t][r]);
     }
   }
 }
@@ -1541,46 +1590,48 @@
 static void launch_bwd_v3(const void* q, const void* k, const void* v,
                           const void* o, const void* dout, const float* lse,
                           void* dq, void* dk, void* dv, float* delta_ws,
-                          const int* klens, int b, int h, int s, float scale,
-                          unsigned int dth, float ksc,
+                          const int* klens, FaStrides qs, FaStrides os,
+                          FaStrides dos, FaStrides gs, int b, int h, int s,
+                          float scale, unsigned int dth, float ksc,
                           unsigned long long seed, hipStream_t stream) {
-  const long rows = (long)b * h * s;
   {
-    long blocks = (rows + 3) / 4;
-    if (blocks > 4096) blocks = 4096;
-    hipLaunchKernelGGL((flash_delta_kernel<D>), dim3((unsigned)blocks),
-                       dim3(256), 0, stream, (const bf16_t*)dout,
-                       (const bf16_t*)o, delta_ws, rows);
+    int bx = (s + 31) / 32;
+    if (bx > 16) bx = 16;
+    hipLaunchKernelGGL((flash_delta_v3_kernel<D>), dim3(bx, h, b), dim3(256),
+                       0, stream, (const bf16_t*)dout, (const bf16_t*)o,
+                       delta_ws, dos, os, h, s);
   }
   dim3 grid((s + V3_QBLK - 1) / V3_QBLK, h, b);
   dim3 block(FA_WAVES * 64);
   hipLaunchKernelGGL((flash_attn_bwd_dq_v3_kernel<D, CAUSAL, HAS_DROP>),
                      grid, block, 0, stream, (const bf16_t*)q,
                      (const bf16_t*)k, (const bf16_t*)v, (const bf16_t*)dout,
-                     lse, delta_ws, (bf16_t*)dq, klens, b, h, s, scale, dth,
-                     ksc, seed);
+                     lse, delta_ws, (bf16_t*)dq, klens, qs, dos, gs, b, h, s,
+                     scale, dth, ksc, seed);
   hipLaunchKernelGGL((flash_attn_bwd_dkv_v3_kernel<D, CAUSAL, HAS_DROP>),
                      grid, block, 0, stream, (const bf16_t*)q,
                      (const bf16_t*)k, (const bf16_t*)v, (const bf16_t*)dout,
-                     lse, delta_ws, (bf16_t*)dk, (bf16_t*)dv, klens, b, h, s,
-                     scale, dth, ksc, seed);
-}
-
-extern "C" void fs_flash_attn_bwd_v3(const void* q, const void* k,
-                                     const void* v, const void* o,
-                                     const void* dout, const float* lse,
-                                     void* dq, void* dk, void* dv,
-                                     float* delta_ws, const int* klens,
-                                     int b, int h, int s, int d, int causal,
-                                     float scale, float drop_p,
-                                     unsigned long long seed,
-                                     hipStream_t stream) {
+                     lse, delta_ws, (bf16_t*)dk, (bf16_t*)dv, klens, qs, dos,
+                     gs, b, h, s, scale, dth, ksc, seed);
+}
+
+extern "C" void fs_flash_attn_bwd_v3_strided(
+    const void* q, const void* k, const void* v, const void* o,
+    const void* dout, const float* lse, void* dq, void* dk, void* dv,
+    float* delta_ws, const int* klens, const long* qs3, const long* os3,
+    const long* dos3, const long* gs3, int b, int h, int s, int d,
+    int causal, float scale, float drop_p, unsigned long long seed,
+    hipStream_t stream) {
+  const FaStrides qs{qs3[0], qs3[1], qs3[2]};
+  const FaStrides os{os3[0], os3[1], os3[2]};
+  const FaStrides dos{dos3[0], dos3[1], dos3[2]};
+  const FaStrides gs{gs3[0], gs3[1], gs3[2]};
   const unsigned int dth =
       (drop_p > 0.f) ? (unsigned int)(drop_p * 4294967296.0) : 0u;
   const float ksc = (drop_p > 0.f) ? 1.f / (1.f - drop_p) : 1.f;
 #define BWD3(DD, CC, DR) launch_bwd_v3<DD, CC, DR>( \
-      q, k, v, o, dout, lse, dq, dk, dv, delta_ws, klens, b, h, s, scale, \
-      dth, ksc, seed, stream)
+      q, k, v, o, dout, lse, dq, dk, dv, delta_ws, klens, qs, os, dos, gs, \
+      b, h, s, scale, dth, ksc, seed, stream)
   if (dth) {
     if (d == 128 && causal) BWD3(128, true, true);
     else if (d == 128) BWD3(128, false, true);
@@ -1598,3 +1649,18 @@
   }
 #undef BWD3
 }
+
+extern "C" void fs_flash_attn_bwd_v3(const void* q, const void* k,
+                                     const void* v, const void* o,
+                                     const void* dout, const float* lse,
+                                     void* dq, void* dk, void* dv,
+                                     float* delta_ws, const int* klens,
+                                     int b, int h, int s, int d, int causal,
+                                     float scale, float drop_p,
+                                     unsigned long long seed,
+                                     hipStream_t stream) {
+  const long c3[3] = {(long)h * s * d, (long)s * d, (long)d};
+  fs_flash_attn_bwd_v3_strided(q, k, v, o, dout, lse, dq, dk, dv, delta_ws,
+                               klens, c3, c3, c3, c3, b, h, s, d, causal,
+                               scale, drop_p, seed, stream);
+}
diff --git a/fengshen_amd/ops/csrc/kernels.hip b/fengshen_amd/ops/csrc/kernels.hip
--- a/fengshen_amd/ops/csrc/kernels.hip
+++ b/fengshen_amd/ops/csrc/kernels.hip
@@ -348,6 +348,45 @@
   }
 }
 
+template <typename T, bool BWD>
+__global__ void rope_inplace_kernel(T* __restrict__ xq, T* __restrict__ xk,
+                                    const float* __restrict__ cos_t,
+                                    const float* __restrict__ sin_t,
+                                    long pairs_per_tensor, int np, int s,
+                                    int h2, int offset, long sb, long sh,
+                                    long sr) {
+  const long stride = (long)gridDim.x * blockDim.x * 8;
+  for (long i0 = (long)(blockIdx.x * blockDim.x + threadIdx.x) * 8;
+       i0 < 2 * pairs_per_tensor; i0 += stride) {
+    T* x = i0 < pairs_per_tensor ? xq : xk;
+    const long i = i0 < pairs_per_tensor ? i0 : i0 - pairs_per_tensor;
+    const long d = i % h2;
+    const long hd = (i / h2) % np;
+    const long si = (i / ((long)h2 * np)) % s;
+    const long bi = i / ((long)h2 * np * s);
+    const long base = bi * sb + hd * sh + si * sr;
+    const float* cr = cos_t + (si + offset) * (2 * h2) + d;
+    const float* sn_r = sin_t + (si + offset) * (2 * h2) + d;
+    float x1[8], x2[8], o1[8], o2[8];
+    load8<T>(x + base + d, x1);
+    load8<T>(x + base + d + h2, x2);
+#pragma unroll
+    for (int j = 0; j < 8; ++j) {
+      const float c = cr[j];
+      const float sn = sn_r[j];
+      if (!BWD) {
+        o1[j] = x1[j] * c - x2[j] * sn;
+        o2[j] = x2[j] * c + x1[j] * sn;
+      } else {
+        o1[j] = x1[j] * c + x2[j] * sn;
+        o2[j] = x2[j] * c - x1[j] * sn;
+      }
+    }
+    store8<T>(x + base + d, o1);
+    store8<T>(x + base + d + h2, o2);
+  }
+}
+
 template <typename T>
 __global__ void swiglu_fwd_kernel(const T* __restrict__ packed,
                                   T* __restrict__ out, long rows, int h) {
@@ -739,6 +778,25 @@
   });
 }
 
+void fs_rope_inplace(void* xq, void* xk, const float* cos_t,
+                     const float* sin_t, int b, int np, int seq, int hn,
+                     long sb, long sh, long sr, int offset, int bwd,
+                     int dtype, hipStream_t s) {
+  const int h2 = hn / 2;
+  const long per_tensor = (long)b * np * seq * h2;
+  int grid = grid_for(2 * per_tensor / 8);
+  DISPATCH_DTYPE(dtype, T, {
+    if (bwd)
+      hipLaunchKernelGGL((rope_inplace_kernel<T, true>), dim3(grid),
+                         dim3(256), 0, s, (T*)xq, (T*)xk, cos_t, sin_t,
+                         per_tensor, np, seq, h2, offset, sb, sh, sr);
+    else
+      hipLaunchKernelGGL((rope_inplace_kernel<T, false>), dim3(grid),
+                         dim3(256), 0, s, (T*)xq, (T*)xk, cos_t, sin_t,
+                         per_tensor, np, seq, h2, offset, sb, sh, sr);
+  });
+}
+
 void fs_swiglu_fwd(const void* packed, void* out, long rows, int h, int dtype,
                    hipStream_t s) {
   int grid = grid_for(rows * (long)h / 8);
diff --git a/fengshen_amd/ops/flash.py b/fengshen_amd/ops/flash.py
--- a/fengshen_amd/ops/flash.py
+++ b/fengshen_amd/ops/flash.py
@@ -55,6 +55,96 @@
         return dq, dk, dv, None, None, None, None, None
 
 
+def _thirds(qkv, num_heads):
+    h = qkv.shape[-1] // 3
+    return tuple(qkv.narrow(2, i * h, h).unflatten(2, (num_heads, -1))
+                 .transpose(1, 2) for i in range(3))
+
+
+class _RopePackedInplace(torch.autograd.Function):
+
+    @staticmethod
+    def forward(ctx, qkv, num_heads, cos, sin, offset):
+        q, k, _ = _thirds(qkv, num_heads)
+        get_ext().rope_inplace(q, k, cos, sin, offset, False)
+        ctx.mark_dirty(qkv)
+        ctx.save_for_backward(cos, sin)
+        ctx.num_heads = num_heads
+        ctx.offset = offset
+        return qkv
+
+    @staticmethod
+    def backward(ctx, grad):
+        cos, sin = ctx.saved_tensors
+        if grad.stride(-1) != 1 or any(st % 8 for st in grad.stride()[:-1]) \
+                or grad.storage_offset() % 8:
+            grad = grad.contiguous()
+        dq, dk, _ = _thirds(grad, ctx.num_heads)
+        get_ext().rope_inplace(dq, dk, cos, sin, ctx.offset, True)
+        return grad, None, None, None, None
+
+
+class _PackedFlash(torch.autograd.Function):
+
+    @staticmethod
+    def forward(ctx, qkv, num_heads, scale, causal, klens):
+        b, s, w = qkv.shape
+        q, k, v = _thirds(qkv, num_heads)
+        o = torch.empty(b, s, w // 3, dtype=qkv.dtype, device=qkv.device)
+        lse = get_ext().flash_attn_fwd_v3_strided(
+            q, k, v, o.unflatten(2, (num_heads, -1)).transpose(1, 2), scale,
+            causal, klens)
+        ctx.save_for_backward(qkv, o, lse)
+        ctx.num_heads = num_heads
+        ctx.scale = scale
+        ctx.causal = causal
+        ctx.klens = klens
+        return o
+
+    @staticmethod
+    def backward(ctx, do):
+        qkv, o, lse = ctx.saved_tensors
+        np_ = ctx.num_heads
+        q, k, v = _thirds(qkv, np_)
+        if do.stride(-1) != 1 or any(st % 8 for st in do.stride()[:-1]) \
+                or do.storage_offset() % 8:
+            do = do.contiguous()
+        grad = torch.empty(qkv.shape, dtype=qkv.dtype, device=qkv.device)
+        dq, dk, dv = _thirds(grad, np_)
+        get_ext().flash_attn_bwd_v3_strided(
+            q, k, v, o.unflatten(2, (np_, -1)).transpose(1, 2),
+            do.unflatten(2, (np_, -1)).transpose(1, 2), lse, dq, dk, dv,
+            ctx.scale, ctx.causal, ctx.klens)
+        return grad, None, None, None, None
+
+
+def packed_attn_eligible(qkv, head_dim: int, causal: bool, mask,
+                         dropout_p: float) -> bool:
+    import os
+    if os.environ.get("FENGSHEN_PACKED_ATTN", "1") == "0":
+        return False
+    if qkv.dtype != torch.bfloat16 or qkv.dim() != 3 or dropout_p > 0:
+        return False
+    s = qkv.shape[1]
+    if head_dim not in (64, 96, 128) or s % 64 != 0 or s < 64:
+        return False
+    if causal and mask is not None:
+        return False
+    return (qkv.stride(2) == 1 and qkv.stride(0) % 8 == 0
+            and qkv.stride(1) % 8 == 0 and qkv.storage_offset() % 8 == 0)
+
+
+def packed_self_attention(qkv: torch.Tensor, num_heads: int,
+                          cos: Optional[torch.Tensor],
+                          sin: Optional[torch.Tensor], offset: int,
+                          scale: float, causal: bool = True,
+                          klens: Optional[torch.Tensor] = None
+                          ) -> torch.Tensor:
+    if cos is not None:
+        qkv = _RopePackedInplace.apply(qkv, num_heads, cos, sin, offset)
+    return _PackedFlash.apply(qkv, num_heads, float(scale), causal, klens)
+
+
 def _draw_seed(device) -> int:
     base = int(torch.randint(0, 2 ** 62, (1,)).item())
     try:
```

Measured after the change: 9995 tokens/s, median of 6. 1.03x the previous value.
